# puzzlepaint/surfelmeshing

Hardware: NVIDIA H100
Metric: RGB-D frames/s at 640x480 (depth pre-processing + Integrate()) (higher is better)
Workload: dtype f32

## Files before the change

surfelmeshing_b200/csrc/api.cu:

```cuda

#include <algorithm>
#include <atomic>
#include <chrono>
#include <cstdio>
#include <cstdlib>
#include <cstring>
#include <limits>
#include <mutex>
#include <string>
#include <vector>

#include "sm_handle.cuh"

namespace smb {

namespace {
thread_local std::string g_last_error;
std::atomic<unsigned long long> g_launches{0};
}

int SetError(int code, const char* message) {
  g_last_error = message ? message : "";
  return code;
}

int CheckLaunch(const char* what) {
  const cudaError_t e = cudaGetLastError();
  if (e == cudaSuccess) return SM_OK;
  g_last_error = std::string(what) + ": " + cudaGetErrorString(e);
  return SM_ERR_CUDA;
}

namespace {
struct ProfileRecord { cudaEvent_t start, stop; int id; };
std::mutex g_profile_mutex;
bool g_profile_enabled = false;
std::vector<ProfileRecord> g_profile_records;
std::vector<cudaEvent_t> g_event_pool;

cudaEvent_t TakeEvent() {
  if (!g_event_pool.empty()) { cudaEvent_t e = g_event_pool.back(); g_event_pool.pop_back(); return e; }
  cudaEvent_t e = nullptr;
  cudaEventCreate(&e);
  return e;
}
}

bool ProfilingEnabled() { return g_profile_enabled; }

void CountLaunches(unsigned long long n) { g_launches.fetch_add(n, std::memory_order_relaxed); }
unsigned long long LaunchCount() { return g_launches.load(); }

void LaunchOnStream(cudaStream_t stream, const KernelLaunch& k, bool dependent) {
  LaunchScope scope(stream, static_cast<KernelId>(k.kernel_id));
  cudaLaunchConfig_t cfg = {};
  cfg.gridDim = k.grid;
  cfg.blockDim = k.block;
  cfg.dynamicSmemBytes = k.smem;
  cfg.stream = stream;
  cudaLaunchAttribute attr[1];
  attr[0].id = cudaLaunchAttributeProgrammaticStreamSerialization;
  attr[0].val.programmaticStreamSerializationAllowed = 1;
  cfg.attrs = attr;
  const int mode = PdlMode();
  cfg.numAttrs = (mode == 2 || (mode == 1 && dependent)) ? 1 : 0;
  cudaLaunchKernelExC(&cfg, k.func, const_cast<void**>(k.args));
}

namespace {
u32 ModInverse(u32 x, u32 m) {
  long long t = 0, new_t = 1, r = m, new_r = x % m;
  while (new_r != 0) {
    const long long q = r / new_r;
    long long tmp = t - q * new_t; t = new_t; new_t = tmp;
    tmp = r - q * new_r; r = new_r; new_r = tmp;
  }
  if (t < 0) t += m;
  return static_cast<u32>(t);
}
}

int SetTieBreakWave(TieBreakConfig* cfg, u32 wave, u32 capacity) {
  u32 lane_shift = cfg->lane_request;
  if (wave != 0) {
    const unsigned long long top = (static_cast<unsigned long long>(capacity) / wave + 2) * 2ull * wave;
    if (wave < 2 || top >= 0xFFFFFFFFull) return SetError(SM_ERR_INVALID_ARGUMENT, "tiebreak_wave out of range for this surfel cap");
    if (lane_shift > 10) return SetError(SM_ERR_INVALID_ARGUMENT, "tiebreak_lanes must be a power of two <= 1024");
    if (wave % (1u << lane_shift) != 0 || (wave >> lane_shift) < 2) lane_shift = 0;
    const u32 groups = wave >> lane_shift;
    const unsigned long long prime = 2654435761ull;
    cfg->mul = static_cast<u32>(prime % groups);
    if (cfg->mul == 0) cfg->mul = 1;
    cfg->mul_inv = ModInverse(cfg->mul, groups);
  }
  cfg->wave = wave;
  cfg->lane_shift = lane_shift;
  return SM_OK;
}

TieBreak MakeTieBreak(const TieBreakConfig& cfg, u32 frame_index) {
  TieBreak t{};
  t.wave = cfg.wave;
  if (cfg.wave == 0) return t;
  t.lane_shift = cfg.lane_shift;
  t.wave_offset = cfg.wave_offset;
  t.groups = cfg.wave >> cfg.lane_shift;
  t.mul = cfg.mul;
  t.mul_inv = cfg.mul_inv;
  t.wave_reciprocal = ~0ull / cfg.wave;
  t.group_reciprocal = ~0ull / t.groups;
  t.add = tb_hash(frame_index * 0x9E3779B9u + 0x7F4A7C15u) % t.groups;
  t.salt = tb_hash(frame_index ^ 0x85EBCA6Bu);
  auto threshold = [](double fraction) {
    const double scaled = fraction * 4294967296.0;
    return scaled <= 0 ? 0u : (scaled >= 4294967295.0 ? 0xFFFFFFFFu : static_cast<u32>(scaled));
  };
  t.early_threshold = threshold(cfg.early_fraction);
  t.index_order_threshold = threshold(cfg.index_order_fraction);
  const double later = cfg.early_fraction_later >= 0 ? cfg.early_fraction_later : cfg.early_fraction;
  t.early_threshold_later = threshold(later);
  t.early_threshold_second = threshold(cfg.early_fraction_second >= 0 ? cfg.early_fraction_second : later);
  t.index_order_threshold_later = threshold(cfg.index_order_fraction_later >= 0 ? cfg.index_order_fraction_later : cfg.index_order_fraction);
  return t;
}

int ScaleGrid(int blocks) {
  static const int percent = [] { const char* e = std::getenv("SM_B200_GRID_PERCENT"); return e ? std::atoi(e) : 100; }();
  const int scaled = static_cast<int>(static_cast<long long>(blocks) * percent / 100);
  return scaled > 0 ? scaled : 1;
}

int PdlMode() {
  static const int mode = [] {
    const char* e = std::getenv("SM_B200_PDL");
    return (e && e[0] >= '0' && e[0] <= '2') ? e[0] - '0' : 1;
  }();
  return mode;
}

const char* KernelName(int id) {
  static const char* names[KID_COUNT] = {
      "k_clear", "k_bilateral_outlier", "k_bilateral_generic", "k_outlier", "k_erode_normals_radii", "k_erode",
      "k_normals", "k_radii", "k_project", "k_associate", "k_merge", "k_blend", "k_integrate", "k_update_neighbors",
      "k_new_surfel_scan", "k_create_surfels", "k_reg_accumulate", "k_reg_step", "k_reg_copy_only",
      "k_export_vertices", "k_median_densify", "k_delta_select", "k_viz_buffers", "k_project_tail",
      "k_downscale_depth_median", "k_downscale_color"};
  return (id >= 0 && id < KID_COUNT) ? names[id] : "?";
}

LaunchScope::LaunchScope(cudaStream_t stream, KernelId id) : stream_(stream), slot_(-1) {
  g_launches.fetch_add(1, std::memory_order_relaxed);
  if (g_profile_enabled) {
    std::lock_guard<std::mutex> lock(g_profile_mutex);
    ProfileRecord r{TakeEvent(), TakeEvent(), static_cast<int>(id)};
    cudaEventRecord(r.start, stream_);
    slot_ = static_cast<int>(g_profile_records.size());
    g_profile_records.push_back(r);
  }
}

LaunchScope::~LaunchScope() {
  if (slot_ >= 0) {
    std::lock_guard<std::mutex> lock(g_profile_mutex);
    cudaEventRecord(g_profile_records[slot_].stop, stream_);
  }
}

}

using namespace smb;

#define SM_CUDA(call)                                                                        \
  do {                                                                                       \
    const cudaError_t e_ = (call);                                                           \
    if (e_ != cudaSuccess) {                                                                 \
      g_last_error = std::string(#call) + ": " + cudaGetErrorString(e_);                     \
      return SM_ERR_CUDA;                                                                    \
    }                                                                                        \
  } while (0)

namespace smb {

int FetchCounters(sm_reconstruction* r, cudaStream_t stream) {
  SM_CUDA(cudaMemcpyAsync(r->host_counters, r->d.counters, sizeof(Counters), cudaMemcpyDeviceToHost, stream));
  SM_CUDA(cudaStreamSynchronize(stream));
  if (r->host_counters->capacity_overflow) {
    return SetError(SM_ERR_CAPACITY, "surfel cap exceeded: new surfels of at least one frame were dropped "
                                     "(the reference writes out of bounds here)");
  }
  return SM_OK;
}

FrameParams MakeFrameParams(const sm_reconstruction* r, u32 frame_index, int count_slot, const sm_integrate_params& p,
                            u16* depth, size_t depth_pitch, const u16* depth_pre, size_t depth_pre_pitch,
                            const float* normals, size_t normals_pitch, const float* radius, size_t radius_pitch,
                            const uint8_t* color, size_t color_pitch, const float* global_T_local,
                            const float* local_T_global) {
  FrameParams f;
  f.frame_index = frame_index;
  f.count_slot = count_slot;
  f.skip = 0;
  f.op_epoch = r->op_epoch;
  f.tb = MakeTieBreak(r->tiebreak, frame_index);
  f.active_window = p.surfel_integration_active_window_size;
  f.fx = r->fx; f.fy = r->fy; f.cx = r->cx; f.cy = r->cy;
  f.fx_inv = 1.0f / r->fx;
  f.fy_inv = 1.0f / r->fy;
  const float cx_pixel_center = r->cx - 0.5f;
  const float cy_pixel_center = r->cy - 0.5f;
  f.cx_inv = -cx_pixel_center / r->fx;
  f.cy_inv = -cy_pixel_center / r->fy;
  f.sensor_noise_factor = p.sensor_noise_factor;
  f.cos_normal_compatibility_threshold = cosf(M_PI / 180.0f * p.normal_compatibility_threshold_deg);
  f.max_surfel_confidence = p.max_surfel_confidence;
  f.inv_depth_scaling = 1.0f / p.depth_scaling;
  f.depth_scaling = 1.0f / f.inv_depth_scaling;
  f.radius_factor_squared =
      p.radius_factor_for_regularization_neighbors * p.radius_factor_for_regularization_neighbors;
  f.blend_radius = p.measurement_blending_radius;
  f.local_T_global = MakeMat3x4(local_T_global);
  f.global_T_local = MakeMat3x4(global_T_local);
  f.depth = depth; f.depth_pitch = depth_pitch;
  f.depth_pre = depth_pre; f.depth_pre_pitch = depth_pre_pitch;
  f.normals = reinterpret_cast<const float2*>(normals); f.normals_pitch = normals_pitch;
  f.radius = radius; f.radius_pitch = radius_pitch;
  f.color = reinterpret_cast<const uchar3*>(color); f.color_pitch = color_pitch;
  return f;
}

int IntegrateImpl(sm_reconstruction* r, cudaStream_t stream, u32 frame_index, const sm_integrate_params& p,
                  u16* depth, size_t depth_pitch, const float* normals, size_t normals_pitch, const float* radius,
                  size_t radius_pitch, const uint8_t* color, size_t color_pitch, const float* global_T_local,
                  const float* local_T_global) {
  r->last_stream = stream;
  RecordOperation(r, static_cast<int>(frame_index - static_cast<u32>(p.regularization_frame_window_size)));
  const u16* depth_pre = depth;
  size_t depth_pre_pitch = depth_pitch;
  if (p.do_blending) {
    SM_CUDA(cudaMemcpy2DAsync(r->blend_src, r->blend_src_pitch, depth, depth_pitch, r->d.width * sizeof(u16),
                              r->d.height, cudaMemcpyDeviceToDevice, stream));
    depth_pre = r->blend_src;
    depth_pre_pitch = r->blend_src_pitch;
  }
  const FrameParams f = MakeFrameParams(r, frame_index, r->count_slot, p, depth, depth_pitch, depth_pre, depth_pre_pitch,
                                        normals, normals_pitch, radius, radius_pitch, color, color_pitch,
                                        global_T_local, local_T_global);
  r->last_tiebreak = f.tb;
  int status = IntegrateFrame(stream, r->d, f, p.do_blending != 0, r->rasters_cleared, r->plan, &r->events);
  r->rasters_cleared = false;
  if (status != SM_OK) return status;
  NoteIntegratedFrame(r->d, frame_index);
  const int old_slot = r->count_slot;
  r->count_slot = (r->count_slot + 1) % kCountSlots;
  if (r->events.enabled) cudaEventRecord(r->events.ev[12], stream);
  const int iterations = p.regularization_iterations_per_integration_iteration;
  if (iterations == 0) {
    status = RegularizeSurfels(stream, r->d,  true, frame_index,
                               p.radius_factor_for_regularization_neighbors, p.regularizer_weight,
                               p.regularization_frame_window_size, r->count_slot, old_slot, r->plan);
  } else {
    for (int i = 0; i < iterations && status == SM_OK; ++i) {
      status = RegularizeSurfels(stream, r->d,  false, frame_index,
                                 p.radius_factor_for_regularization_neighbors, p.regularizer_weight,
                                 p.regularization_frame_window_size, r->count_slot, i == 0 ? old_slot : -1, r->plan);
    }
  }
  if (r->events.enabled) cudaEventRecord(r->events.ev[13], stream);
  return status;
}

}

namespace {

int CreateImpl(sm_reconstruction* r, uint64_t max_surfel_count, int32_t width, int32_t height, float fx, float fy,
               float cx, float cy) {
  SM_CUDA(cudaGetDevice(&r->device));
  cudaDeviceProp prop;
  SM_CUDA(cudaGetDeviceProperties(&prop, r->device));
  r->sm_count = prop.multiProcessorCount;
  r->plan.sm_count = r->sm_count;
  {
    const char* e = std::getenv("SM_B200_CARVEOUT");
    const int percent = e ? std::atoi(e) : 47;
    int status = ConfigurePreprocessKernels(percent);
    if (status == SM_OK) status = ConfigureIntegrateKernels(percent, &r->plan);
    if (status == SM_OK) status = ConfigureRegularizeKernels(percent, &r->plan);
    if (status != SM_OK) return status;
  }
  r->fx = fx; r->fy = fy; r->cx = cx; r->cy = cy;
  DeviceState& d = r->d;
  d.width = width; d.height = height;
  d.capacity = static_cast<u32>(max_surfel_count);
  const size_t padded = (max_surfel_count + kSegment - 1) / kSegment * kSegment;
  d.stride = padded;
  const size_t P = static_cast<size_t>(width) * height;
  const size_t scan_tiles = (P + kSegment - 1) / kSegment;
  SM_CUDA(cudaMalloc(&d.surfels, sizeof(float) * SM_ROW_COUNT * d.stride));
  SM_CUDA(cudaMalloc(&d.gradient, sizeof(float4) * d.stride));
  SM_CUDA(cudaMalloc(&r->smooth_alt, sizeof(float) * 3 * d.stride));
  d.smooth = d.surfels + static_cast<size_t>(SM_ROW_SMOOTH_X) * d.stride;
  d.smooth_next = r->smooth_alt;
  SM_CUDA(cudaMemset(d.gradient, 0, sizeof(float4) * d.stride));
  for (int i = 0; i < kSets; ++i) {
    SM_CUDA(cudaMalloc(&r->assoc_set[i], sizeof(PixelAssoc) * P));
    SM_CUDA(cudaMalloc(&r->first_depth_set[i], sizeof(float) * P));
    SM_CUDA(cudaMalloc(&r->supported_set[i], P));
    SM_CUDA(cudaMalloc(&r->vis_set[i], sizeof(VisEntry) * padded));
    SM_CUDA(cudaMalloc(&r->seg_count_set[i], sizeof(u32) * (padded / kSegment)));
    SM_CUDA(cudaMalloc(&r->merge_flag_set[i], padded));
    SM_CUDA(cudaMalloc(&r->upd_list_set[i], sizeof(uint2) * padded));
    SM_CUDA(cudaMalloc(&r->upd_count_set[i], sizeof(u32)));
  }
  d.assoc = r->assoc_set[0]; d.first_depth = r->first_depth_set[0]; d.supported = r->supported_set[0];
  d.vis = r->vis_set[0]; d.seg_count = r->seg_count_set[0]; d.merge_flag = r->merge_flag_set[0];
  d.upd_list = r->upd_list_set[0]; d.upd_count = r->upd_count_set[0];
  d.reg_t_prev = 0;
  d.reg_full_sweep = 1;
  SM_CUDA(cudaMalloc(&d.new_list, sizeof(u32) * P));
  SM_CUDA(cudaMalloc(&d.new_flag, P));
  SM_CUDA(cudaMalloc(&d.new_index, sizeof(u32) * P));
  SM_CUDA(cudaMalloc(&d.scan_state, sizeof(unsigned long long) * scan_tiles));
  SM_CUDA(cudaMalloc(&d.counters, sizeof(Counters)));
  SM_CUDA(cudaMemset(d.counters, 0, sizeof(Counters)));
  d.timeline = nullptr;
  d.timeline_frames = 0;
  SM_CUDA(cudaMemset(d.new_flag, 0, P));
  SM_CUDA(cudaMemset(d.new_index, 0, sizeof(u32) * P));
  SM_CUDA(cudaMemset(d.scan_state, 0, sizeof(unsigned long long) * scan_tiles));
  SM_CUDA(cudaMallocHost(&r->host_counters, sizeof(Counters)));
  std::memset(r->host_counters, 0, sizeof(Counters));
  SM_CUDA(cudaMallocPitch(reinterpret_cast<void**>(&r->scratch_B), &r->scratch_B_pitch, width * sizeof(u16), height));
  SM_CUDA(cudaMallocPitch(reinterpret_cast<void**>(&r->blend_src), &r->blend_src_pitch, width * sizeof(u16), height));
  {
    const char* e = std::getenv("SM_B200_TAIL_FILL");
    const bool want_tma = !(e && std::string(e) == "vector");
    if (want_tma) {
      const int status = MakeDepthTensorMap(&r->scratch_B_map, r->scratch_B, r->scratch_B_pitch, width, height);
      if (status != SM_OK) return status;
      r->scratch_B_map_valid = true;
    }
  }
  for (int i = 0; i < 14; ++i) SM_CUDA(cudaEventCreate(&r->events.ev[i]));
  r->events.enabled = false;
  {
    u32 wave = kDefaultTieBreakWave, lanes = 1u << kDefaultTieBreakLaneShift;
    double early = kDefaultTieBreakEarlyFraction, index_order = kDefaultTieBreakIndexOrderFraction;
    u32 offset = kDefaultTieBreakWaveOffset;
    if (const char* e = std::getenv("SM_B200_TIEBREAK")) {
      unsigned w = 0, l = 0, o = 0; double q = 0, b = 0;
      const int got = std::sscanf(e, "%u,%lf,%lf,%u,%u", &w, &q, &b, &l, &o);
      if (got >= 2) { wave = w; early = q; }
      if (got >= 3) index_order = b;
      if (got >= 4) lanes = l;
      if (got >= 5) offset = o ? 1u : 0u;
    }
    r->tiebreak.wave_offset = offset;
    u32 lane_shift = 0;
    while ((1u << lane_shift) < lanes && lane_shift < 10) ++lane_shift;
    if (wave != 0 && (static_cast<unsigned long long>(d.capacity) / wave + 2) * 2ull * wave >= 0xFFFFFFFFull) wave = 0;
    r->tiebreak.lane_request = lane_shift;
    const int status = SetTieBreakWave(&r->tiebreak, wave, d.capacity);
    if (status != SM_OK) return status;
    r->tiebreak.early_fraction = early;
    r->tiebreak.index_order_fraction = index_order;
    r->tiebreak.early_fraction_later = kDefaultTieBreakEarlyFractionLater;
    r->tiebreak.index_order_fraction_later = kDefaultTieBreakIndexOrderFractionLater;
    r->tiebreak.early_fraction_second = kDefaultTieBreakEarlyFractionSecond;
  }
  const int status = ClearAssociationRasters(nullptr, d);
  if (status != SM_OK) return status;
  SM_CUDA(cudaDeviceSynchronize());
  return SM_OK;
}

}

extern "C" {

void sm_default_integrate_params(sm_integrate_params* p) {
  p->depth_scaling = 5000;
  p->sensor_noise_factor = 0.05f;
  p->max_surfel_confidence = 5.0f;
  p->regularizer_weight = 10.0f;
  p->regularization_frame_window_size = 30;
  p->do_blending = 1;
  p->measurement_blending_radius = 12;
  p->regularization_iterations_per_integration_iteration = 1;
  p->radius_factor_for_regularization_neighbors = 2;
  p->normal_compatibility_threshold_deg = 40;
  p->surfel_integration_active_window_size = std::numeric_limits<int>::max();
}

void sm_default_preprocess_params(sm_preprocess_params* p) {
  p->depth_scaling = 5000;
  p->max_depth = 3.0f;
  p->depth_valid_region_radius = 333;
  p->bilateral_filter_sigma_xy = 3;
  p->bilateral_filter_radius_factor = 2.0f;
  p->bilateral_filter_sigma_depth_factor = 0.05;
  p->outlier_filtering_frame_count = 8;
  p->outlier_filtering_required_inliers = -1;
  p->outlier_filtering_depth_tolerance_factor = 0.02f;
  p->depth_erosion_radius = 2;
  p->observation_angle_threshold_deg = 85;
  p->point_radius_extension_factor = 1.5f;
  p->point_radius_clamp_factor = std::numeric_limits<float>::infinity();
}

const char* sm_last_error(void) { return g_last_error.c_str(); }
const char* sm_version(void) { return "surfel_b200 0.1 (sm_90a)"; }
uint64_t sm_kernel_launch_count(void) { return g_launches.load(); }

int sm_profile_kernels(int32_t enable) {
  std::lock_guard<std::mutex> lock(g_profile_mutex);
  g_profile_enabled = enable != 0;
  return SM_OK;
}

int32_t sm_profile_kernel_count(void) { return KID_COUNT; }
const char* sm_profile_kernel_name(int32_t id) { return KernelName(id); }

int sm_profile_report(double* total_ms, uint64_t* launches, int32_t n) {
  SM_CUDA(cudaDeviceSynchronize());
  std::lock_guard<std::mutex> lock(g_profile_mutex);
  for (int i = 0; i < n; ++i) { total_ms[i] = 0; launches[i] = 0; }
  for (const ProfileRecord& r : g_profile_records) {
    float ms = 0;
    if (cudaEventElapsedTime(&ms, r.start, r.stop) == cudaSuccess && r.id < n) {
      total_ms[r.id] += ms;
      launches[r.id] += 1;
    }
    g_event_pool.push_back(r.start);
    g_event_pool.push_back(r.stop);
  }
  g_profile_records.clear();
  return SM_OK;
}

int sm_create(sm_reconstruction** out, uint64_t max_surfel_count, int32_t width, int32_t height, float fx, float fy,
              float cx, float cy) {
  if (out) *out = nullptr;
  if (!out || width <= 0 || height <= 0 || max_surfel_count == 0 || max_surfel_count > 0x7FFFFFFFull - kSegment) {
    return SetError(SM_ERR_INVALID_ARGUMENT, "sm_create: bad argument");
  }
  sm_reconstruction* r = new sm_reconstruction();
  const int status = CreateImpl(r, max_surfel_count, width, height, fx, fy, cx, cy);
  if (status != SM_OK) {
    const std::string message = g_last_error;
    sm_destroy(r);
    g_last_error = message;
    return status;
  }
  *out = r;
  return SM_OK;
}

int sm_destroy(sm_reconstruction* r) {
  if (!r) return SM_OK;
  cudaDeviceSynchronize();
  cudaGetLastError();
  DestroyFrameGraph(r->graph);
  DeviceState& d = r->d;
  cudaFree(d.surfels); cudaFree(d.gradient); cudaFree(r->smooth_alt); cudaFree(d.new_list);
  for (int i = 0; i < kSets; ++i) {
    cudaFree(r->vis_set[i]); cudaFree(r->seg_count_set[i]); cudaFree(r->merge_flag_set[i]);
    cudaFree(r->upd_list_set[i]); cudaFree(r->upd_count_set[i]);
    cudaFree(r->assoc_set[i]); cudaFree(r->first_depth_set[i]); cudaFree(r->supported_set[i]);
    cudaFree(r->run_depth[i]); cudaFree(r->run_depth_pre[i]); cudaFree(r->run_normals[i]); cudaFree(r->run_radius[i]);
  }
  cudaFree(d.new_flag); cudaFree(d.new_index); cudaFree(d.scan_state); cudaFree(d.counters);
  cudaFree(d.timeline);
  if (r->host_counters) cudaFreeHost(r->host_counters);
  cudaFree(r->scratch_B);
  cudaFree(r->blend_src);
  cudaFree(r->median_stage[0]); cudaFree(r->median_stage[1]);
  cudaFree(r->pyramid_depth_stage); cudaFree(r->pyramid_color_stage);
  FreeTransferBuffers(r);
  for (int i = 0; i < 2; ++i) {
    if (r->pipe.ev_create[i]) cudaEventDestroy(r->pipe.ev_create[i]);
    if (r->pipe.ev_update[i]) cudaEventDestroy(r->pipe.ev_update[i]);
    if (r->pre_done[i]) cudaEventDestroy(r->pre_done[i]);
    if (r->int_done[i]) cudaEventDestroy(r->int_done[i]);
  }
  for (cudaStream_t st : {r->pre_stream, r->pipe.crit, r->pipe.front, r->pipe.side, r->upload_stream, r->graph_stream})
    if (st) cudaStreamDestroy(st);
  for (cudaEvent_t e : {r->pipe.ev_assoc, r->pipe.ev_merge, r->pipe.ev_blend, r->pipe.ev_integrate, r->pipe.ev_reg,
                        r->entry_event, r->upload_done, r->graph_exit})
    if (e) cudaEventDestroy(e);
  for (cudaEvent_t e : r->iteration_done) if (e) cudaEventDestroy(e);
  for (u16* b : r->ring_depth) cudaFree(b);
  for (uchar3* b : r->ring_color) cudaFree(b);
  for (int i = 0; i < 14; ++i) if (r->events.ev[i]) cudaEventDestroy(r->events.ev[i]);
  delete r;
  cudaGetLastError();
  return SM_OK;
}

int sm_reset(sm_reconstruction* r, void* stream) {
  SM_CUDA(cudaMemsetAsync(r->d.counters, 0, sizeof(Counters), static_cast<cudaStream_t>(stream)));
  r->count_slot = 0;
  r->rasters_cleared = false;
  r->last_stream = static_cast<cudaStream_t>(stream);
  ++r->state_generation;
  r->op_history.clear();
  return SM_OK;
}

int sm_preprocess(sm_reconstruction* r, void* stream, const sm_preprocess_params* p, const uint16_t* raw_depth,
                  size_t raw_pitch, const uint16_t* const* other_depths, const size_t* other_pitches,
                  const float* others_TR_reference, uint16_t* out_depth, size_t out_depth_pitch, float* out_normals,
                  size_t out_normals_pitch, float* out_radius, size_t out_radius_pitch) {
  const int status = PreprocessFused(static_cast<cudaStream_t>(stream), *p, r->d.width, r->d.height, r->fx, r->fy,
                                     r->cx, r->cy, raw_depth, raw_pitch, other_depths, other_pitches,
                                     others_TR_reference, r->scratch_B, r->scratch_B_pitch, out_depth,
                                     out_depth_pitch, reinterpret_cast<float2*>(out_normals), out_normals_pitch,
                                     out_radius, out_radius_pitch, r->d.assoc, r->d.first_depth, r->d.supported, nullptr, 0,
                                     nullptr, nullptr, r->ScratchBMap());
  if (status == SM_OK) r->rasters_cleared = true;
  return status;
}

int sm_bilateral_filter_and_depth_cutoff(void* stream, float sigma_xy, float sigma_value_factor,
                                         uint16_t value_to_ignore, float radius_factor, uint16_t max_depth,
                                         float depth_valid_region_radius, int32_t width, int32_t height,
                                         const uint16_t* in_depth, size_t in_pitch, uint16_t* out_depth,
                                         size_t out_pitch) {
  return StageBilateral(static_cast<cudaStream_t>(stream), sigma_xy, sigma_value_factor, value_to_ignore,
                        radius_factor, max_depth, depth_valid_region_radius, width, height, in_depth, in_pitch,
                        out_depth, out_pitch);
}

int sm_outlier_depth_map_fusion(void* stream, int32_t other_count, int32_t required_count, float tolerance, float fx,
                                float fy, float cx, float cy, int32_t width, int32_t height, const uint16_t* in_depth,
                                size_t in_pitch, const uint16_t* const* other_depths, const size_t* other_pitches,
                                const float* others_TR_reference, uint16_t* out_depth, size_t out_pitch) {
  return StageOutlier(static_cast<cudaStream_t>(stream), other_count, required_count, tolerance, fx, fy, cx, cy,
                      width, height, in_depth, in_pitch, other_depths, other_pitches, others_TR_reference, out_depth,
                      out_pitch);
}

int sm_median_filter_and_densify_depth_map(void* stream, int32_t iterations, int32_t width, int32_t height,
                                           const uint16_t* in_depth, size_t in_pitch, uint16_t* out_depth,
                                           size_t out_pitch, uint16_t* scratch, size_t scratch_pitch) {
  return StageMedianDensify(static_cast<cudaStream_t>(stream), iterations, width, height, in_depth, in_pitch, out_depth,
                            out_pitch, scratch, scratch_pitch);
}

int sm_downscale_using_median_while_excluding(void* stream, uint16_t value_to_ignore, int32_t in_width,
                                              int32_t in_height, const uint16_t* in, size_t in_pitch,
                                              int32_t out_width, int32_t out_height, uint16_t* out,
                                              size_t out_pitch) {
  return StageDownscaleMedian(static_cast<cudaStream_t>(stream), value_to_ignore, in_width, in_height, in, in_pitch,
                              out_width, out_height, out, out_pitch);
}

int sm_color_image_pyramid(void* stream, int32_t levels, int32_t width, int32_t height, const uint8_t* in,
                           size_t in_pitch, uint8_t* out, size_t out_pitch) {
  return StageColorPyramid(static_cast<cudaStream_t>(stream), levels, width, height, in, in_pitch, out, out_pitch);
}

int sm_erode_depth_map(void* stream, int32_t radius, int32_t width, int32_t height, const uint16_t* in_depth,
                       size_t in_pitch, uint16_t* out_depth, size_t out_pitch) {
  return StageErode(static_cast<cudaStream_t>(stream), radius, width, height, in_depth, in_pitch, out_depth,
                    out_pitch);
}

int sm_compute_normals_and_drop_bad_pixels(void* stream, float observation_angle_threshold_deg, float depth_scaling,
                                           float fx, float fy, float cx, float cy, int32_t width, int32_t height,
                                           const uint16_t* in_depth, size_t in_pitch, uint16_t* out_depth,
                                           size_t out_pitch, float* out_normals, size_t normals_pitch) {
  return StageNormals(static_cast<cudaStream_t>(stream), observation_angle_threshold_deg, depth_scaling, fx, fy, cx,
                      cy, width, height, in_depth, in_pitch, out_depth, out_pitch,
                      reinterpret_cast<float2*>(out_normals), normals_pitch);
}

int sm_compute_point_radii_and_remove_isolated_pixels(void* stream, float point_radius_extension_factor,
                                                      float point_radius_clamp_factor, float depth_scaling, float fx,
                                                      float fy, float cx, float cy, int32_t width, int32_t height,
                                                      const uint16_t* in_depth, size_t in_pitch, float* out_radius,
                                                      size_t radius_pitch, uint16_t* out_depth, size_t out_pitch) {
  return StageRadii(static_cast<cudaStream_t>(stream), point_radius_extension_factor, point_radius_clamp_factor,
                    depth_scaling, fx, fy, cx, cy, width, height, in_depth, in_pitch, out_radius, radius_pitch,
                    out_depth, out_pitch);
}

int sm_integrate(sm_reconstruction* r, void* stream, uint32_t frame_index, const sm_integrate_params* p,
                 uint16_t* depth, size_t depth_pitch, const float* normals, size_t normals_pitch, const float* radius,
                 size_t radius_pitch, const uint8_t* color, size_t color_pitch, const float global_T_local[12],
                 const float local_T_global[12]) {
  return IntegrateImpl(r, static_cast<cudaStream_t>(stream), frame_index, *p, depth, depth_pitch, normals,
                       normals_pitch, radius, radius_pitch, color, color_pitch, global_T_local, local_T_global);
}

int sm_regularize(sm_reconstruction* r, void* stream, uint32_t frame_index, float regularizer_weight,
                  float radius_factor_for_regularization_neighbors, int32_t regularization_frame_window_size) {
  r->last_stream = static_cast<cudaStream_t>(stream);
  RecordOperation(r, static_cast<int>(frame_index - static_cast<u32>(regularization_frame_window_size)));
  return RegularizeSurfels(static_cast<cudaStream_t>(stream), r->d,  false, frame_index,
                           radius_factor_for_regularization_neighbors, regularizer_weight,
                           regularization_frame_window_size, r->count_slot, -1, r->plan);
}

int sm_surfel_count(sm_reconstruction* r, uint32_t* out) {
  const int status = FetchCounters(r, r->last_stream);
  *out = r->host_counters->surfel_count[r->count_slot] - r->host_counters->merge_count;
  return status;
}

int sm_surfels_size(sm_reconstruction* r, uint32_t* out) {
  const int status = FetchCounters(r, r->last_stream);
  *out = r->host_counters->surfel_count[r->count_slot];
  return status;
}

int sm_transfer_all_to_cpu(sm_reconstruction* r, void* stream_v, uint32_t , float* x, float* y,
                           float* z, float* radius_squared, float* nx, float* ny, float* nz,
                           uint32_t* last_update_stamp, uint64_t* out_count) {
  cudaStream_t stream = static_cast<cudaStream_t>(stream_v);
  const int status = FetchCounters(r, stream);
  const u32 n = r->host_counters->surfel_count[r->count_slot];
  if (out_count) *out_count = n;
  if (n == 0) return status;
  const size_t bytes = sizeof(float) * n;
  const float* s = r->d.surfels;
  const size_t st = r->d.stride;
  SM_CUDA(cudaMemcpyAsync(x, r->d.smooth + 0 * st, bytes, cudaMemcpyDeviceToHost, stream));
  SM_CUDA(cudaMemcpyAsync(y, r->d.smooth + 1 * st, bytes, cudaMemcpyDeviceToHost, stream));
  SM_CUDA(cudaMemcpyAsync(z, r->d.smooth + 2 * st, bytes, cudaMemcpyDeviceToHost, stream));
  SM_CUDA(cudaMemcpyAsync(radius_squared, s + SM_ROW_RADIUS_SQUARED * st, bytes, cudaMemcpyDeviceToHost, stream));
  SM_CUDA(cudaMemcpyAsync(nx, s + SM_ROW_NORMAL_X * st, bytes, cudaMemcpyDeviceToHost, stream));
  SM_CUDA(cudaMemcpyAsync(ny, s + SM_ROW_NORMAL_Y * st, bytes, cudaMemcpyDeviceToHost, stream));
  SM_CUDA(cudaMemcpyAsync(nz, s + SM_ROW_NORMAL_Z * st, bytes, cudaMemcpyDeviceToHost, stream));
  SM_CUDA(cudaMemcpyAsync(last_update_stamp, s + SM_ROW_LAST_UPDATE_STAMP * st, bytes, cudaMemcpyDeviceToHost, stream));
  return status;
}

int sm_transfer_delta_to_cpu(sm_reconstruction* r, void* stream, uint32_t frame_index, sm_transfer_token* token,
                             float* x, float* y, float* z, float* radius_squared, float* nx, float* ny, float* nz,
                             uint32_t* last_update_stamp, sm_transfer_stats* stats) {
  if (!r || !token) return SetError(SM_ERR_INVALID_ARGUMENT, "sm_transfer_delta_to_cpu: null argument");
  return TransferDelta(r, static_cast<cudaStream_t>(stream), frame_index, token, x, y, z, radius_squared, nx, ny, nz,
                       last_update_stamp, stats);
}

int sm_update_visualization_buffers(sm_reconstruction* r, void* stream, const sm_visualization_params* p,
                                    float* vertex_buffer, uint32_t* neighbor_index_buffer, float* normal_vertex_buffer) {
  if (!r || !p) return SetError(SM_ERR_INVALID_ARGUMENT, "sm_update_visualization_buffers: null argument");
  return UpdateVisualizationBuffers(r, static_cast<cudaStream_t>(stream), *p, vertex_buffer, neighbor_index_buffer,
                                    normal_vertex_buffer);
}

int sm_export_vertices(sm_reconstruction* r, void* stream, float* position_buffer, uint8_t* color_buffer) {
  return ExportVertices(static_cast<cudaStream_t>(stream), r->d, r->count_slot, r->sm_count, position_buffer,
                        color_buffer);
}

int sm_get_timings(sm_reconstruction* r, float out_ms[7]) {
  if (!r->events.enabled) return SetError(SM_ERR_INVALID_ARGUMENT, "timings are not enabled (sm_enable_timings)");
  SM_CUDA(cudaEventSynchronize(r->events.ev[13]));
  for (int i = 0; i < 7; ++i) SM_CUDA(cudaEventElapsedTime(&out_ms[i], r->events.ev[2 * i], r->events.ev[2 * i + 1]));
  return SM_OK;
}

int sm_enable_timings(sm_reconstruction* r, int32_t enable) {
  r->events.enabled = enable != 0;
  return SM_OK;
}

int sm_dump_state(sm_reconstruction* r, void* stream_v, float* host_rows, uint64_t host_row_stride_elems,
                  uint32_t* surfels_size, uint32_t* merge_count) {
  cudaStream_t stream = static_cast<cudaStream_t>(stream_v);
  const int status = FetchCounters(r, stream);
  const u32 n = r->host_counters->surfel_count[r->count_slot];
  if (surfels_size) *surfels_size = n;
  if (merge_count) *merge_count = r->host_counters->merge_count;
  if (host_rows && n > host_row_stride_elems) return SetError(SM_ERR_INVALID_ARGUMENT, "sm_dump_state: host rows shorter than surfels_size()");
  if (host_rows && n > 0) {
    SM_CUDA(cudaMemcpy2DAsync(host_rows, host_row_stride_elems * sizeof(float), r->d.surfels,
                              r->d.stride * sizeof(float), n * sizeof(float), SM_ROW_COUNT, cudaMemcpyDeviceToHost,
                              stream));
    SM_CUDA(cudaMemcpy2DAsync(host_rows + SM_ROW_SMOOTH_X * host_row_stride_elems, host_row_stride_elems * sizeof(float),
                              r->d.smooth, r->d.stride * sizeof(float), n * sizeof(float), 3, cudaMemcpyDeviceToHost,
                              stream));
    SM_CUDA(cudaStreamSynchronize(stream));
  }
  return status;
}

int sm_load_state(sm_reconstruction* r, void* stream_v, const float* host_rows, uint64_t host_row_stride_elems,
                  uint32_t surfels_size, uint32_t merge_count) {
  cudaStream_t stream = static_cast<cudaStream_t>(stream_v);
  if (surfels_size > r->d.capacity) return SetError(SM_ERR_CAPACITY, "sm_load_state: state larger than the surfel cap");
  r->d.smooth = r->d.surfels + static_cast<size_t>(SM_ROW_SMOOTH_X) * r->d.stride;
  r->d.smooth_next = r->smooth_alt;
  r->d.reg_full_sweep = 1;
  if (surfels_size > 0) {
    SM_CUDA(cudaMemcpy2DAsync(r->d.surfels, r->d.stride * sizeof(float), host_rows,
                              host_row_stride_elems * sizeof(float), surfels_size * sizeof(float), SM_ROW_COUNT,
                              cudaMemcpyHostToDevice, stream));
    SM_CUDA(cudaMemsetAsync(r->d.gradient, 0, surfels_size * sizeof(float4), stream));
    const int zero_rows[4] = {SM_ROW_GRADIENT_X, SM_ROW_GRADIENT_Y, SM_ROW_GRADIENT_Z, SM_ROW_GRADIENT_COUNT};
    for (int row : zero_rows) {
      SM_CUDA(cudaMemsetAsync(r->d.surfels + row * r->d.stride, 0, surfels_size * sizeof(float), stream));
    }
    SM_CUDA(cudaMemsetAsync(r->d.surfels + kRowMergeEpoch * r->d.stride, 0, surfels_size * sizeof(float), stream));
    const int status = RebuildMetaRow(stream, r->d, surfels_size, r->sm_count);
    if (status != SM_OK) return status;
  }
  Counters c{};
  for (int i = 0; i < kCountSlots; ++i) c.surfel_count[i] = surfels_size;
  c.merge_count = merge_count;
  *r->host_counters = c;
  SM_CUDA(cudaMemcpyAsync(r->d.counters, r->host_counters, sizeof(Counters), cudaMemcpyHostToDevice, stream));
  SM_CUDA(cudaStreamSynchronize(stream));
  r->count_slot = 0;
  r->last_stream = stream;
  ++r->state_generation;
  r->op_history.clear();
  return SM_OK;
}

int sm_download_rasters(sm_reconstruction* r, void* stream_v, uint32_t* supporting_surfels,
                        uint32_t* supporting_surfel_counts, float* supporting_surfel_depth_sums,
                        uint32_t* conflicting_surfels, float* first_surfel_depth, uint8_t* new_surfel_flag_vector,
                        uint32_t* new_surfel_indices) {
  cudaStream_t stream = static_cast<cudaStream_t>(stream_v);
  const size_t P = static_cast<size_t>(r->d.width) * r->d.height;
  std::vector<PixelAssoc> assoc(P);
  SM_CUDA(cudaMemcpyAsync(assoc.data(), r->d.assoc, sizeof(PixelAssoc) * P, cudaMemcpyDeviceToHost, stream));
  if (first_surfel_depth)
    SM_CUDA(cudaMemcpyAsync(first_surfel_depth, r->d.first_depth, sizeof(float) * P, cudaMemcpyDeviceToHost, stream));
  if (new_surfel_flag_vector)
    SM_CUDA(cudaMemcpyAsync(new_surfel_flag_vector, r->d.new_flag, P, cudaMemcpyDeviceToHost, stream));
  if (new_surfel_indices)
    SM_CUDA(cudaMemcpyAsync(new_surfel_indices, r->d.new_index, sizeof(u32) * P, cudaMemcpyDeviceToHost, stream));
  SM_CUDA(cudaStreamSynchronize(stream));
  for (size_t i = 0; i < P; ++i) {
    if (supporting_surfels) supporting_surfels[i] = supporting_index(r->last_tiebreak, assoc[i].x, static_cast<u32>(i));
    if (conflicting_surfels) conflicting_surfels[i] = assoc[i].y;
    if (supporting_surfel_counts) supporting_surfel_counts[i] = assoc[i].z;
    if (supporting_surfel_depth_sums) std::memcpy(&supporting_surfel_depth_sums[i], &assoc[i].w, sizeof(float));
  }
  return SM_OK;
}

int sm_frame_counters(sm_reconstruction* r, void* stream_v, uint64_t out[4]) {
  cudaStream_t stream = static_cast<cudaStream_t>(stream_v);
  const int status = FetchCounters(r, stream);
  const u32 n_after = r->host_counters->surfel_count[r->count_slot];
  const u32 n_swept = n_after - r->host_counters->new_surfel_count;
  const size_t segments = (static_cast<size_t>(n_swept) + kSegment - 1) / kSegment;
  std::vector<u32> seg(segments);
  if (segments) SM_CUDA(cudaMemcpy(seg.data(), r->d.seg_count, sizeof(u32) * segments, cudaMemcpyDeviceToHost));
  uint64_t visible = 0;
  for (u32 c : seg) visible += c;
  const size_t P = static_cast<size_t>(r->d.width) * r->d.height;
  std::vector<PixelAssoc> assoc(P);
  SM_CUDA(cudaMemcpy(assoc.data(), r->d.assoc, sizeof(PixelAssoc) * P, cudaMemcpyDeviceToHost));
  uint64_t support = 0;
  for (const PixelAssoc& a : assoc) support += a.z;
  out[0] = n_swept; out[1] = visible; out[2] = support; out[3] = r->host_counters->new_surfel_count;
  return status;
}

int sm_timeline_enable(sm_reconstruction* r, int32_t frames) {
  if (r == nullptr || frames < 0) return SetError(SM_ERR_INVALID_ARGUMENT, "sm_timeline_enable: bad arguments");
  SM_CUDA(cudaDeviceSynchronize());
  if (r->d.timeline) {
    cudaFree(r->d.timeline);
    r->d.timeline = nullptr;
    r->d.timeline_frames = 0;
  }
  if (frames == 0) return SM_OK;
  const size_t slots = static_cast<size_t>(frames) * KID_COUNT;
  SM_CUDA(cudaMalloc(&r->d.timeline, slots * 2 * sizeof(unsigned long long)));
  std::vector<unsigned long long> init(slots * 2);
  for (size_t i = 0; i < slots; ++i) { init[2 * i] = ~0ull; init[2 * i + 1] = 0ull; }
  SM_CUDA(cudaMemcpy(r->d.timeline, init.data(), init.size() * sizeof(unsigned long long), cudaMemcpyHostToDevice));
  r->d.timeline_frames = static_cast<u32>(frames);
  return SM_OK;
}

int sm_timeline_read(sm_reconstruction* r, uint64_t* out, int32_t frames) {
  if (r == nullptr || out == nullptr) return SetError(SM_ERR_INVALID_ARGUMENT, "sm_timeline_read: bad arguments");
  if (r->d.timeline == nullptr || frames != static_cast<int32_t>(r->d.timeline_frames))
    return SetError(SM_ERR_INVALID_ARGUMENT, "sm_timeline_read: timeline not enabled with this frame count");
  SM_CUDA(cudaDeviceSynchronize());
  SM_CUDA(cudaMemcpy(out, r->d.timeline, static_cast<size_t>(frames) * KID_COUNT * 2 * sizeof(uint64_t), cudaMemcpyDeviceToHost));
  return SM_OK;
}

int sm_stream_run(sm_reconstruction* r, void* stream_v, const sm_stream_desc* s, const sm_preprocess_params* pp,
                  const sm_integrate_params* ip, int32_t first_frame, int32_t last_frame, sm_stream_stats* stats) {
  if (!r || !s || !pp || !ip) return SetError(SM_ERR_INVALID_ARGUMENT, "sm_stream_run: null argument");
  return StreamRun(r, static_cast<cudaStream_t>(stream_v), s, pp, ip, first_frame, last_frame, stats);
}

int sm_configure(sm_reconstruction* r, const char* key, double value) {
  if (!r || !key) return SetError(SM_ERR_INVALID_ARGUMENT, "sm_configure: null argument");
  const std::string k(key);
  if (k == "tiebreak_wave") {
    if (value < 0 || value > 2147483647.0) return SetError(SM_ERR_INVALID_ARGUMENT, "tiebreak_wave out of range");
    return SetTieBreakWave(&r->tiebreak, static_cast<u32>(value), r->d.capacity);
  }
  if (k == "tiebreak_early_fraction_later" || k == "tiebreak_index_order_fraction_later" || k == "tiebreak_early_fraction_second") {
    if (!(value <= 1.0)) return SetError(SM_ERR_INVALID_ARGUMENT, "tiebreak_*_later / _second must be <= 1 (negative: inherit)");
    (k == "tiebreak_early_fraction_later" ? r->tiebreak.early_fraction_later
     : k == "tiebreak_early_fraction_second" ? r->tiebreak.early_fraction_second : r->tiebreak.index_order_fraction_later) = value;
    return SM_OK;
  }
  if (k == "tiebreak_wave_offset") {
    r->tiebreak.wave_offset = value != 0.0 ? 1u : 0u;
    return SM_OK;
  }
  if (k == "tiebreak_lanes") {
    const u32 lanes = static_cast<u32>(value);
    if (value < 1 || value > 1024 || (lanes & (lanes - 1)) != 0) return SetError(SM_ERR_INVALID_ARGUMENT, "tiebreak_lanes must be a power of two in [1, 1024]");
    u32 shift = 0;
    while ((1u << shift) < lanes) ++shift;
    r->tiebreak.lane_request = shift;
    return SetTieBreakWave(&r->tiebreak, r->tiebreak.wave, r->d.capacity);
  }
  if (k == "tiebreak_early_fraction") {
    if (!(value >= 0.0 && value <= 1.0)) return SetError(SM_ERR_INVALID_ARGUMENT, "tiebreak_early_fraction must be in [0, 1]");
    r->tiebreak.early_fraction = value;
    return SM_OK;
  }
  if (k == "tiebreak_index_order_fraction") {
    if (!(value >= 0.0 && value <= 1.0)) return SetError(SM_ERR_INVALID_ARGUMENT, "tiebreak_index_order_fraction must be in [0, 1]");
    r->tiebreak.index_order_fraction = value;
    return SM_OK;
  }
  if (k == "median_filter_and_densify_iterations") {
    if (value < 0 || value > 16 || value != static_cast<int>(value)) return SetError(SM_ERR_INVALID_ARGUMENT, "median_filter_and_densify_iterations must be an integer in [0, 16]");
    r->median_iterations = static_cast<int>(value);
    return SM_OK;
  }
  if (k == "pyramid_level") {
    if (value < 0 || value > 4 || value != static_cast<int>(value)) return SetError(SM_ERR_INVALID_ARGUMENT, "pyramid_level must be an integer in [0, 4]");
    r->pyramid_level = static_cast<int>(value);
    return SM_OK;
  }
  return SetError(SM_ERR_INVALID_ARGUMENT, "sm_configure: unknown key");
}

}
```

surfelmeshing_b200/csrc/integrate.cu:

```cuda

#include <algorithm>
#include <cstdio>
#include <cstdlib>

#include <cooperative_groups.h>

#include "sm_kernels.cuh"

namespace cg = cooperative_groups;

namespace smb {

namespace {

#define SM_S(row, i) d.surfels[static_cast<size_t>(row) * d.stride + (i)]
#define SM_SU(row, i) reinterpret_cast<u32*>(d.surfels)[static_cast<size_t>(row) * d.stride + (i)]
#define SM_SMOOTH(axis, i) d.smooth[static_cast<size_t>(axis) * d.stride + (i)]
#define SM_SMOOTH_NEXT(axis, i) d.smooth_next[static_cast<size_t>(axis) * d.stride + (i)]

constexpr int kBlock = 256;

__device__ __forceinline__ bool is_active(u32 last_update_stamp, u32 frame_index, int window) {
  return static_cast<int>(last_update_stamp) > static_cast<int>(frame_index - static_cast<u32>(window));
}

struct Projection {
  float u, v;
  int px, py;
  bool in_image;
};

__device__ __forceinline__ Projection project(const FrameParams& f, int width, int height, float x, float y, float z) {
  Projection p;
  const float inv_z = frcp(z);
  p.u = ffma(fmul(x, inv_z), f.fx, f.cx);
  p.v = ffma(fmul(y, inv_z), f.fy, f.cy);
  p.px = f2i_trunc(p.u);
  p.py = f2i_trunc(p.v);
  p.in_image = !(p.u < 0.f || p.v < 0.f || p.px < 0 || p.py < 0 || p.px >= width || p.py >= height);
  return p;
}

__device__ __forceinline__ bool secondary_pixel(const Projection& p, int width, int height, int* ox, int* oy) {
  const float x_frac = fsub(p.u, i2f(p.px));
  const float y_frac = fsub(p.v, i2f(p.py));
  if (x_frac < y_frac) {
    if (x_frac < fadd(-y_frac, 1.0f)) {
      if (p.px > 1) { *ox = p.px - 1; *oy = p.py; return true; }
      return false;
    }
    if (p.py < height - 1) { *ox = p.px; *oy = p.py + 1; return true; }
    return false;
  }
  if (x_frac < fadd(-y_frac, 1.0f)) {
    if (p.py > 0) { *ox = p.px; *oy = p.py - 1; return true; }
    return false;
  }
  if (p.px < width - 1) { *ox = p.px + 1; *oy = p.py; return true; }
  return false;
}

__device__ __forceinline__ float normal_z_abs(float nx, float ny) {
  return fsqrt_approx(fmaxf(0.f, ffma(-ny, ny, ffma(-nx, nx, 1.0f))));
}

__device__ __forceinline__ float facing_dot(const FrameParams& f, float x, float y, float z, float nx, float ny,
                                            float nz, float3* local_normal) {
  const float rs = frsqrt_approx(squared_norm(x, y, z));
  *local_normal = rotate_vec(f.local_T_global, nx, ny, nz);
  return fmul(rs, ffma(z, local_normal->z, ffma(x, local_normal->x, fmul(y, local_normal->y))));
}

template <typename Body>
__device__ __forceinline__ void for_each_visible(const DeviceState& d, const u32* surfel_count, Body&& body) {
  constexpr u32 kItemsPerSegment = kSegment / kBlock;
  const u32 max_items = ((d.capacity + kSegment - 1) / kSegment) * kItemsPerSegment;
  const u32 n = *surfel_count;
  u32 item = blockIdx.x;
  u32 cnt = 0;
  VisEntry e = make_uint4(0u, 0u, 0u, 0u);
  if (item < max_items) {
    cnt = d.seg_count[item / kItemsPerSegment];
    e = d.vis[static_cast<size_t>(item) * kBlock + threadIdx.x];
  }
  const u32 items = ((n + kSegment - 1) / kSegment) * kItemsPerSegment;
  while (item < items) {
    const u32 next = item + gridDim.x;
    u32 cnt_next = 0;
    VisEntry e_next = e;
    if (next < items) {
      cnt_next = d.seg_count[next / kItemsPerSegment];
      e_next = d.vis[static_cast<size_t>(next) * kBlock + threadIdx.x];
    }
    const u32 k = (item % kItemsPerSegment) * kBlock + threadIdx.x;
    if (k < cnt) body(static_cast<size_t>(item) * kBlock + threadIdx.x, e);
    item = next;
    cnt = cnt_next;
    e = e_next;
  }
}

__global__ void __launch_bounds__(kBlock) k_clear(DeviceState d) {
  pdl_prologue();
  const int n = d.width * d.height;
  for (int i = blockIdx.x * blockDim.x + threadIdx.x; i < n; i += gridDim.x * blockDim.x) {
    d.assoc[i] = make_uint4(kInvalidIndex, kInvalidIndex, 0u, 0u);
    d.first_depth[i] = __int_as_float(0x7f800000);
    d.supported[i] = 0;
  }
}

constexpr int kProjectBlock = 512;

enum { kProjectAll = 0, kProjectMain = 1, kProjectTail = 2 };

__global__ void __launch_bounds__(kProjectBlock) k_project(DeviceState d, FrameParams f, int part) {
  pdl_prologue();
  if (f.skip) return;
  const TimelineScope timeline_scope(d, f.frame_index, part == kProjectTail ? KID_PROJECT_TAIL : KID_PROJECT);
  __shared__ u32 warp_totals[kProjectBlock / 32];
  const int lane = threadIdx.x & 31, warp = threadIdx.x >> 5;
  const u32 first_seg_if_all = blockIdx.x;

  if (blockIdx.x == 0 && part != kProjectMain) {
    const int tiles = (d.width * d.height + kSegment - 1) / kSegment;
    for (int t = threadIdx.x; t < tiles; t += blockDim.x) d.scan_state[t] = 0ull;
    if (threadIdx.x == 0) { d.counters->scan_ticket = 0; *d.upd_count = 0; }
  }

  struct SlotRows { float2 X, Y, Z; uint2 T; };
  auto fetch = [&](u32 seg) {
    SlotRows r;
    const size_t base = static_cast<size_t>(seg) * kSegment + threadIdx.x * 2;
    r.X = *reinterpret_cast<const float2*>(&SM_S(SM_ROW_X, base));
    r.Y = *reinterpret_cast<const float2*>(&SM_S(SM_ROW_Y, base));
    r.Z = *reinterpret_cast<const float2*>(&SM_S(SM_ROW_Z, base));
    r.T = *reinterpret_cast<const uint2*>(&SM_SU(SM_ROW_LAST_UPDATE_STAMP, base));
    return r;
  };
  SlotRows rows = {};
  if (part != kProjectTail && (static_cast<size_t>(first_seg_if_all) + 1) * kSegment <= d.stride) rows = fetch(first_seg_if_all);
  const u32 n_before = part == kProjectAll ? 0u : d.counters->surfel_count[(f.count_slot + kCountSlots - 1) % kCountSlots];
  const u32 seg_begin = part == kProjectTail ? n_before / kSegment : 0u;
  const u32 n = part == kProjectMain ? (n_before / kSegment) * kSegment
                                     : d.counters->surfel_count[f.count_slot];
  if (part == kProjectTail && static_cast<u64>(seg_begin + blockIdx.x) * kSegment < n) rows = fetch(seg_begin + blockIdx.x);
  for (u32 seg = seg_begin + blockIdx.x; static_cast<u64>(seg) * kSegment < n; seg += gridDim.x) {
    const u32 base = seg * kSegment + threadIdx.x * 2;
    const SlotRows cur = rows;
    if (static_cast<u64>(seg + gridDim.x) * kSegment < n) rows = fetch(seg + gridDim.x);
    VisEntry e[2];
    bool visible[2] = {false, false};
    u32 cnt = 0;
    if (base < n) {
      const float xs[2] = {cur.X.x, cur.X.y}, ys[2] = {cur.Y.x, cur.Y.y}, zs[2] = {cur.Z.x, cur.Z.y};
      const u32 ts[2] = {cur.T.x, cur.T.y};
#pragma unroll
      for (int j = 0; j < 2; ++j) {
        const u32 i = base + j;
        if (i >= n) break;
        const float z = transform_row(f.local_T_global.r2, xs[j], ys[j], zs[j]);
        if (!(z > 0.f)) continue;
        const float x = transform_row(f.local_T_global.r0, xs[j], ys[j], zs[j]);
        const float y = transform_row(f.local_T_global.r1, xs[j], ys[j], zs[j]);
        const Projection p = project(f, d.width, d.height, x, y, z);
        if (!p.in_image) continue;
        const bool active = is_active(ts[j], f.frame_index, f.active_window);
        e[j] = make_uint4(i | (active ? kActiveBit : 0u), __float_as_uint(x), __float_as_uint(y), __float_as_uint(z));
        visible[j] = true;
        ++cnt;
        if (active) {
// ... 510 lines not shown
  }
#endif
}


struct SurfelState {
  float x, y, z, confidence, radius_squared, nx, ny, nz;
  float smooth_x, smooth_y, smooth_z;
  u32 color, creation_stamp, last_update_stamp;
  bool replaced, dirty, stamped;
};

struct PixelMeasurement {
  float measurement_depth, first, radius_squared;
  float2 normal;
  u32 conflicting, count;
  u32 r, g, b;
};

__device__ __forceinline__ PixelMeasurement load_pixel_measurement(const DeviceState& d, const FrameParams& f, int x,
                                                                   int y) {
  PixelMeasurement m;
  const int p = y * d.width + x;
  m.measurement_depth = fmul(u2f(row_ptr(f.depth, f.depth_pitch, y)[x]), f.inv_depth_scaling);
  m.first = d.first_depth[p];
  const PixelAssoc a = d.assoc[p];
  m.conflicting = a.y;
  m.count = a.z;
  m.normal = row_ptr(f.normals, f.normals_pitch, y)[x];
  m.radius_squared = row_ptr(f.radius, f.radius_pitch, y)[x];
  const uchar3 c = row_ptr(f.color, f.color_pitch, y)[x];
  m.r = c.x; m.g = c.y; m.b = c.z;
  return m;
}

__device__ __forceinline__ void integrate_or_conflict(const FrameParams& f, const PixelMeasurement& m, int x, int y,
                                                      u32 idx, float cx_, float cy_, float cz_, SurfelState& s) {
  if (!(m.measurement_depth > 0.f)) return;
  bool integrate = true, conflicting = false;
  if (m.first < fmul(m.measurement_depth, fadd(-f.sensor_noise_factor, 1.0f))) {
    if (m.first == cz_ && m.conflicting == idx) conflicting = true;
    integrate = false;
  }
  if (!integrate && !conflicting) return;
  if (cz_ > fmul(fadd(f.sensor_noise_factor, 1.0f), m.measurement_depth)) integrate = false;
  if (!integrate && !conflicting) return;

  const float lx = fmul(m.measurement_depth, ffma(i2f(x), f.fx_inv, f.cx_inv));
  const float ly = fmul(m.measurement_depth, ffma(i2f(y), f.fy_inv, f.cy_inv));
  const float3 g = transform_point(f.global_T_local, lx, ly, m.measurement_depth);
  const float3 gn = rotate_vec(f.global_T_local, m.normal.x, m.normal.y, -normal_z_abs(m.normal.x, m.normal.y));

  if (conflicting) {
    const float confidence = fadd(s.confidence, -1.0f);
    if (confidence <= 0.f) {
      s.x = g.x; s.y = g.y; s.z = g.z;
      s.smooth_x = g.x; s.smooth_y = g.y; s.smooth_z = g.z;
      s.nx = gn.x; s.ny = gn.y; s.nz = gn.z;
      s.color = m.r | (m.g << 8) | (m.b << 16) | (1u << 24);
      s.radius_squared = m.radius_squared;
      s.confidence = 1.0f;
      s.creation_stamp = f.frame_index;
      s.stamped = true;
      s.replaced = true;
    } else {
      s.confidence = confidence;
    }
    s.dirty = true;
  }
  if (!integrate) return;

  float3 ln;
  if (facing_dot(f, cx_, cy_, cz_, s.nx, s.ny, s.nz, &ln) > 0.f) return;
  if (m.measurement_depth < cz_) {
    if (ffma(gn.z, s.nz, ffma(gn.x, s.nx, fmul(gn.y, s.ny))) < f.cos_normal_compatibility_threshold) return;
  }
  if (s.radius_squared < 0.f) return;

  const float weight = frcp(u2f(max(1u, m.count)));
  if (s.creation_stamp < f.frame_index) {
    const float confidence = s.confidence;
    const float cw = fadd(weight, confidence);
    s.confidence = (cw < f.max_surfel_confidence) ? cw : f.max_surfel_confidence;
    const float normalization_factor = frcp(cw);
    s.x = fmul(normalization_factor, ffma(g.x, weight, fmul(confidence, s.x)));
    s.y = fmul(normalization_factor, ffma(g.y, weight, fmul(confidence, s.y)));
    s.z = fmul(normalization_factor, ffma(g.z, weight, fmul(confidence, s.z)));
    const float nx = ffma(gn.x, weight, fmul(confidence, s.nx));
    const float ny = ffma(gn.y, weight, fmul(confidence, s.ny));
    const float nz = ffma(gn.z, weight, fmul(confidence, s.nz));
    const float normal_normalization = frsqrt_approx(ffma(nz, nz, ffma(nx, nx, fmul(ny, ny))));
    s.nx = fmul(nx, normal_normalization);
    s.ny = fmul(ny, normal_normalization);
    s.nz = fmul(nz, normal_normalization);
    s.radius_squared = fminf(s.radius_squared, m.radius_squared);
    const u32 old_color = s.color;
    const u32 r = f2u_trunc(ffma(normalization_factor, ffma(u2f(m.r), weight, fmul(confidence, u2f(old_color & 0xFFu))), 0.5f));
    const u32 gr = f2u_trunc(ffma(normalization_factor, ffma(u2f(m.g), weight, fmul(confidence, u2f((old_color >> 8) & 0xFFu))), 0.5f));
    const u32 b = f2u_trunc(ffma(normalization_factor, ffma(u2f(m.b), weight, fmul(confidence, u2f((old_color >> 16) & 0xFFu))), 0.5f));
    s.color = (r & 0xFFu) | ((gr & 0xFFu) << 8) | ((b & 0xFFu) << 16);
    s.stamped = true;
    s.dirty = true;
  }
}

#ifndef SM_INTEGRATE_LEVELS
#define SM_INTEGRATE_LEVELS 2
#endif

__device__ __forceinline__ bool pixel_can_touch(const FrameParams& f, float measurement_depth, float first, u32 conflicting,
                                                u32 idx, float cz_) {
  if (!(measurement_depth > 0.f)) return false;
  if (first < fmul(measurement_depth, fadd(-f.sensor_noise_factor, 1.0f))) return first == cz_ && conflicting == idx;
  return !(cz_ > fmul(fadd(f.sensor_noise_factor, 1.0f), measurement_depth));
}

__device__ __forceinline__ bool integrate_entry(const DeviceState& d, const FrameParams& f, size_t pos, const VisEntry& e,
                                                int* ux, int* uy) {
    const u32 idx = e.x & ~kActiveBit;
    const float x = __uint_as_float(e.y), y = __uint_as_float(e.z), z = __uint_as_float(e.w);
    const Projection p = project(f, d.width, d.height, x, y, z);
    int ox = p.px, oy = p.py;
    const bool has2 = secondary_pixel(p, d.width, d.height, &ox, &oy);
    const u8 merged = d.merge_flag[pos];
    SurfelState s;
    PixelMeasurement m0, m1;
#if SM_INTEGRATE_LEVELS == 1
    m0 = load_pixel_measurement(d, f, p.px, p.py);
    m1 = load_pixel_measurement(d, f, ox, oy);
    s.x = SM_S(SM_ROW_X, idx); s.y = SM_S(SM_ROW_Y, idx); s.z = SM_S(SM_ROW_Z, idx);
    s.confidence = SM_S(SM_ROW_CONFIDENCE, idx);
    s.radius_squared = SM_S(SM_ROW_RADIUS_SQUARED, idx);
    s.nx = SM_S(SM_ROW_NORMAL_X, idx); s.ny = SM_S(SM_ROW_NORMAL_Y, idx); s.nz = SM_S(SM_ROW_NORMAL_Z, idx);
    s.color = SM_SU(SM_ROW_COLOR, idx);
    s.creation_stamp = SM_SU(SM_ROW_CREATION_STAMP, idx);
#else
    const int p0 = p.py * d.width + p.px, p1 = oy * d.width + ox;
    m0.measurement_depth = fmul(u2f(row_ptr(f.depth, f.depth_pitch, p.py)[p.px]), f.inv_depth_scaling);
    m1.measurement_depth = fmul(u2f(row_ptr(f.depth, f.depth_pitch, oy)[ox]), f.inv_depth_scaling);
    m0.first = d.first_depth[p0];
    m1.first = d.first_depth[p1];
    const PixelAssoc a0 = d.assoc[p0], a1 = d.assoc[p1];
    m0.conflicting = a0.y; m0.count = a0.z;
    m1.conflicting = a1.y; m1.count = a1.z;
    s.radius_squared = SM_S(SM_ROW_RADIUS_SQUARED, idx);
#endif
    s.last_update_stamp = 0;
    s.smooth_x = s.smooth_y = s.smooth_z = 0.f;
    s.replaced = false; s.dirty = false; s.stamped = false;
    if (merged) {
      SM_SU(SM_ROW_LAST_UPDATE_STAMP, idx) = 0;
      SM_S(SM_ROW_RADIUS_SQUARED, idx) = -1.0f;
      reinterpret_cast<u8*>(&SM_SU(SM_ROW_COLOR, idx))[3] = 1;
      SM_SU(kRowMeta, idx) = kMetaDetachBit;
      SM_SU(kRowMergeEpoch, idx) = f.op_epoch;
      SM_SMOOTH_NEXT(0, idx) = SM_SMOOTH(0, idx); SM_SMOOTH_NEXT(1, idx) = SM_SMOOTH(1, idx);
      SM_SMOOTH_NEXT(2, idx) = SM_SMOOTH(2, idx);
      return false;
    }
    if (!(e.x & kActiveBit)) return false;
    if (s.radius_squared < 0.f) return false;
#if SM_INTEGRATE_LEVELS != 1
    const bool touch0 = pixel_can_touch(f, m0.measurement_depth, m0.first, m0.conflicting, idx, z);
    const bool touch1 = has2 && pixel_can_touch(f, m1.measurement_depth, m1.first, m1.conflicting, idx, z);
    if (touch0 || touch1) {
      const int qx0 = touch0 ? p.px : ox, qy0 = touch0 ? p.py : oy;
      const int qx1 = touch1 ? ox : qx0, qy1 = touch1 ? oy : qy0;
      m0.normal = row_ptr(f.normals, f.normals_pitch, qy0)[qx0];
      m1.normal = row_ptr(f.normals, f.normals_pitch, qy1)[qx1];
      m0.radius_squared = row_ptr(f.radius, f.radius_pitch, qy0)[qx0];
      m1.radius_squared = row_ptr(f.radius, f.radius_pitch, qy1)[qx1];
      const uchar3 c0 = row_ptr(f.color, f.color_pitch, qy0)[qx0];
      const uchar3 c1 = row_ptr(f.color, f.color_pitch, qy1)[qx1];
      m0.r = c0.x; m0.g = c0.y; m0.b = c0.z;
      m1.r = c1.x; m1.g = c1.y; m1.b = c1.z;
      s.x = SM_S(SM_ROW_X, idx); s.y = SM_S(SM_ROW_Y, idx); s.z = SM_S(SM_ROW_Z, idx);
      s.confidence = SM_S(SM_ROW_CONFIDENCE, idx);
      s.nx = SM_S(SM_ROW_NORMAL_X, idx); s.ny = SM_S(SM_ROW_NORMAL_Y, idx); s.nz = SM_S(SM_ROW_NORMAL_Z, idx);
      s.color = SM_SU(SM_ROW_COLOR, idx);
      s.creation_stamp = SM_SU(SM_ROW_CREATION_STAMP, idx);
      if (touch0) integrate_or_conflict(f, m0, p.px, p.py, idx, x, y, z, s);
      if (touch1) integrate_or_conflict(f, m1, ox, oy, idx, x, y, z, s);
    }
#else
    integrate_or_conflict(f, m0, p.px, p.py, idx, x, y, z, s);
    if (has2) integrate_or_conflict(f, m1, ox, oy, idx, x, y, z, s);
#endif
    if (s.dirty) {
      SM_S(SM_ROW_X, idx) = s.x; SM_S(SM_ROW_Y, idx) = s.y; SM_S(SM_ROW_Z, idx) = s.z;
      SM_S(SM_ROW_CONFIDENCE, idx) = s.confidence;
      SM_S(SM_ROW_RADIUS_SQUARED, idx) = s.radius_squared;
      SM_S(SM_ROW_NORMAL_X, idx) = s.nx; SM_S(SM_ROW_NORMAL_Y, idx) = s.ny; SM_S(SM_ROW_NORMAL_Z, idx) = s.nz;
      SM_SU(SM_ROW_COLOR, idx) = s.color;
      if (s.stamped) {
        SM_SU(SM_ROW_LAST_UPDATE_STAMP, idx) = f.frame_index;
        SM_SU(kRowMeta, idx) = f.frame_index | (((s.color >> 24) & 1u) ? kMetaDetachBit : 0u);
      }
      if (s.replaced) {
        SM_SMOOTH(0, idx) = s.smooth_x; SM_SMOOTH(1, idx) = s.smooth_y; SM_SMOOTH(2, idx) = s.smooth_z;
        SM_SMOOTH_NEXT(0, idx) = s.smooth_x; SM_SMOOTH_NEXT(1, idx) = s.smooth_y; SM_SMOOTH_NEXT(2, idx) = s.smooth_z;
        SM_SU(SM_ROW_CREATION_STAMP, idx) = f.frame_index;
#pragma unroll
        for (int i = 0; i < 4; ++i) SM_SU(SM_ROW_NEIGHBOR0 + i, idx) = kInvalidIndex;
      }
    }

    if (s.stamped && !is_active(f.frame_index, f.frame_index, f.active_window)) return false;
    if (s.radius_squared < 0.f) return false;
    float cz_ = z;
    int px = p.px, py = p.py;
    if (s.dirty) {
      cz_ = transform_row(f.local_T_global.r2, s.x, s.y, s.z);
      if (!(cz_ > 0.f)) return false;
      const float cx_ = transform_row(f.local_T_global.r0, s.x, s.y, s.z);
      const float cy_ = transform_row(f.local_T_global.r1, s.x, s.y, s.z);
      const float inv_z = frcp(cz_);
      px = f2i_trunc(ffma(fmul(cx_, inv_z), f.fx, f.cx));
      py = f2i_trunc(ffma(fmul(cy_, inv_z), f.fy, f.cy));
    }
    constexpr int kBorder = 1;
    if (px < kBorder || py < kBorder || px >= d.width - kBorder || py >= d.height - kBorder) return false;
    float measurement_depth = m0.measurement_depth;
    if (px != p.px || py != p.py) {
      measurement_depth = fmul(u2f(row_ptr(f.depth, f.depth_pitch, py)[px]), f.inv_depth_scaling);
    }
    if (cz_ > fmul(measurement_depth, fadd(f.sensor_noise_factor, 1.0f))) return false;
    *ux = px;
    *uy = py;
    return true;
}

__global__ void __launch_bounds__(kBlock, 4) k_integrate(DeviceState d, FrameParams f) {
  pdl_prologue();
  if (f.skip) return;
  const TimelineScope timeline_scope(d, f.frame_index, KID_INTEGRATE);
  for_each_visible(d, &d.counters->surfel_count[f.count_slot], [&](size_t pos, const VisEntry& e) {
    int ux, uy;
    if (!integrate_entry(d, f, pos, e, &ux, &uy)) return;
    const cg::coalesced_group g = cg::coalesced_threads();
    u32 base = 0;
    if (g.thread_rank() == 0) base = atomicAdd(d.upd_count, g.size());
    base = g.shfl(base, 0) + g.thread_rank();
    d.upd_list[base] = make_uint2(e.x & ~kActiveBit, static_cast<u32>(ux) | (static_cast<u32>(uy) << 16));
  });
}

__device__ __forceinline__ void update_neighbors_survivor(const DeviceState& d, const FrameParams& f, u32 idx, int x, int y) {
  const int kDirectionsX[4] = {-1, 1, 0, 0};
  const int kDirectionsY[4] = {0, 0, -1, 1};
  const float gx = SM_S(SM_ROW_X, idx), gy = SM_S(SM_ROW_Y, idx), gz = SM_S(SM_ROW_Z, idx);
  const float nx = SM_S(SM_ROW_NORMAL_X, idx), ny = SM_S(SM_ROW_NORMAL_Y, idx), nz = SM_S(SM_ROW_NORMAL_Z, idx);
  const float radius_squared = SM_S(SM_ROW_RADIUS_SQUARED, idx);
  u32 neighbor_surfel_indices[4];
#pragma unroll
  for (int m = 0; m < 4; ++m) neighbor_surfel_indices[m] = SM_SU(SM_ROW_NEIGHBOR0 + m, idx);
  const float observation_radius_squared = row_ptr(f.radius, f.radius_pitch, y)[x];
  u32 candidate[4];
#pragma unroll
  for (int direction = 0; direction < 4; ++direction) {
    const int candidate_pixel = (y + kDirectionsY[direction]) * d.width + x + kDirectionsX[direction];
    candidate[direction] = supporting_index(f.tb, d.assoc[candidate_pixel].x, static_cast<u32>(candidate_pixel));
  }
  const float cz_ = transform_row(f.local_T_global.r2, gx, gy, gz);
  const float cx_ = transform_row(f.local_T_global.r0, gx, gy, gz);
  const float cy_ = transform_row(f.local_T_global.r1, gx, gy, gz);
  float3 ln;
  if (facing_dot(f, cx_, cy_, cz_, nx, ny, nz, &ln) > 0.f) return;
  if (fmul(observation_radius_squared, frcp(radius_squared)) > 2.25f) return;
  bool any_new = false;
#pragma unroll
  for (int direction = 0; direction < 4; ++direction) {
    const u32 q = candidate[direction];
    if (q == kInvalidIndex || q == idx) { candidate[direction] = kInvalidIndex; continue; }
    any_new |= q != neighbor_surfel_indices[0] && q != neighbor_surfel_indices[1] &&
               q != neighbor_surfel_indices[2] && q != neighbor_surfel_indices[3];
  }
  if (!any_new) return;

  float neighbor_distances_squared[4];
#pragma unroll
  for (int m = 0; m < 4; ++m) {
    const u32 q = neighbor_surfel_indices[m];
    if (q == kInvalidIndex) {
      neighbor_distances_squared[m] = __int_as_float(0x7f800000);
    } else {
      neighbor_distances_squared[m] = squared_norm(fsub(gx, SM_S(SM_ROW_X, q)), fsub(gy, SM_S(SM_ROW_Y, q)),
                                                   fsub(gz, SM_S(SM_ROW_Z, q)));
    }
  }
  const float max_distance_squared = fmul(radius_squared, f.radius_factor_squared);
  float cand_distance[4], cand_dot[4];
#pragma unroll
  for (int direction = 0; direction < 4; ++direction) {
    const u32 q = candidate[direction];
    if (q == kInvalidIndex) continue;
    cand_distance[direction] = squared_norm(fsub(SM_S(SM_ROW_X, q), gx), fsub(SM_S(SM_ROW_Y, q), gy),
                                            fsub(SM_S(SM_ROW_Z, q), gz));
    cand_dot[direction] = dot3(nx, ny, nz, SM_S(SM_ROW_NORMAL_X, q), SM_S(SM_ROW_NORMAL_Y, q), SM_S(SM_ROW_NORMAL_Z, q));
  }
  bool changed = false;
#pragma unroll
  for (int direction = 0; direction < 4; ++direction) {
    const u32 q = candidate[direction];
    if (q == kInvalidIndex) continue;
    const float distance_squared = cand_distance[direction];
    if (distance_squared > max_distance_squared) continue;
    if (cand_dot[direction] <= 0.f) continue;
    int best_n = -1;
    float best_distance_squared = -1.f;
#pragma unroll
    for (int m = 0; m < 4; ++m) {
      if (q == neighbor_surfel_indices[m]) { best_n = -1; break; }
      if (neighbor_distances_squared[m] > best_distance_squared) {
        best_n = m;
        best_distance_squared = neighbor_distances_squared[m];
      }
    }
    if (best_n >= 0 && distance_squared < best_distance_squared) {
#pragma unroll
      for (int m = 0; m < 4; ++m) {
        if (m == best_n) { neighbor_surfel_indices[m] = q; neighbor_distances_squared[m] = distance_squared; }
      }
      changed = true;
    }
  }
  if (changed) {
#pragma unroll
    for (int m = 0; m < 4; ++m) SM_SU(SM_ROW_NEIGHBOR0 + m, idx) = neighbor_surfel_indices[m];
  }
}

__global__ void __launch_bounds__(kBlock) k_update_neighbors(DeviceState d, FrameParams f) {
  pdl_prologue();
  if (f.skip) return;
  const TimelineScope timeline_scope(d, f.frame_index, KID_UPDATE_NEIGHBORS);
  const u32 n = *d.upd_count;
  for (u32 k = blockIdx.x * blockDim.x + threadIdx.x; k < n; k += gridDim.x * blockDim.x) {
    const uint2 w = d.upd_list[k];
    update_neighbors_survivor(d, f, w.x, static_cast<int>(w.y & 0xFFFFu), static_cast<int>(w.y >> 16));
  }
}

__device__ __forceinline__ unsigned long long load_scan_state(unsigned long long* p) { return atomicAdd(p, 0ull); }

__global__ void __launch_bounds__(kBlock) k_new_surfel_scan(DeviceState d, FrameParams f) {
  pdl_prologue();
  if (f.skip) return;
  const TimelineScope timeline_scope(d, f.frame_index, KID_NEW_SURFEL_SCAN);
  __shared__ u32 s_tile, s_prefix;
  __shared__ u32 warp_totals[kBlock / 32];
  const int total_pixels = d.width * d.height;
  const int tiles = (total_pixels + kSegment - 1) / kSegment;
  if (threadIdx.x == 0) s_tile = atomicAdd(&d.counters->scan_ticket, 1u);
  __syncthreads();
  const u32 tile = s_tile;
  if (tile >= static_cast<u32>(tiles)) return;

  const int base = tile * kSegment + threadIdx.x * 4;
  u32 flags[4];
  u32 cnt = 0;
#pragma unroll
  for (int j = 0; j < 4; ++j) {
    const int seq = base + j;
    u32 flag = 0;
    if (seq < total_pixels) {
      const int y = seq / d.width, x = seq - y * d.width;
      constexpr int kBorder = 1;
      if (x >= kBorder && y >= kBorder && x < d.width - kBorder && y < d.height - kBorder &&
          row_ptr(f.depth, f.depth_pitch, y)[x] > 0 && !d.supported[seq]) {
        flag = (d.assoc[seq].y == kInvalidIndex) ? 1u : 0u;
      }
    }
    flags[j] = flag;
    cnt += flag;
  }
  const int lane = threadIdx.x & 31, warp = threadIdx.x >> 5;
  u32 incl = cnt;
#pragma unroll
  for (int o = 1; o < 32; o <<= 1) {
    const u32 t = __shfl_up_sync(0xffffffffu, incl, o);
    if (lane >= o) incl += t;
  }
  if (lane == 31) warp_totals[warp] = incl;
  __syncthreads();
  u32 warp_base = 0, block_total = 0;
#pragma unroll
  for (int w = 0; w < kBlock / 32; ++w) {
    const u32 t = warp_totals[w];
    if (w < warp) warp_base += t;
    block_total += t;
  }
  if (warp == 0) {
    if (lane == 0) atomicExch(&d.scan_state[tile], ((tile == 0 ? 2ull : 1ull) << 32) | block_total);
    u32 exclusive = 0;
    int window_end = static_cast<int>(tile) - 1;
    while (window_end >= 0) {
      const int t = window_end - lane;
      unsigned long long v = 2ull << 32;
      if (t >= 0) {
        do { v = load_scan_state(&d.scan_state[t]); } while ((v >> 32) == 0ull);
      }
      const unsigned inclusive_mask = __ballot_sync(0xffffffffu, (v >> 32) == 2ull);
      const int first_inclusive = __ffs(inclusive_mask) - 1;
      const u32 contribution = (first_inclusive < 0 || lane <= first_inclusive) ? static_cast<u32>(v) : 0u;
      exclusive += __reduce_add_sync(0xffffffffu, contribution);
      if (first_inclusive >= 0) break;
      window_end -= 32;
    }
    if (lane == 0) {
      if (tile != 0) atomicExch(&d.scan_state[tile], (2ull << 32) | (exclusive + block_total));
      s_prefix = exclusive;
      if (tile == static_cast<u32>(tiles) - 1) {
        const u32 n_old = d.counters->surfel_count[f.count_slot];
        u32 new_count = exclusive + block_total;
        if (static_cast<u64>(n_old) + new_count > d.capacity) {
          d.counters->capacity_overflow = 1;
          new_count = 0;
        }
        d.counters->new_surfel_count = new_count;
        d.counters->surfel_count[(f.count_slot + 1) % kCountSlots] = n_old + new_count;
      }
    }
  }
  __syncthreads();
  u32 running = s_prefix + warp_base + (incl - cnt);
#pragma unroll
  for (int j = 0; j < 4; ++j) {
    const int seq = base + j;
    if (seq < total_pixels) {
      d.new_flag[seq] = static_cast<u8>(flags[j]);
      d.new_index[seq] = running;
      if (flags[j]) d.new_list[running] = seq;
    }
    running += flags[j];
  }
}

__global__ void __launch_bounds__(kBlock) k_create_surfels(DeviceState d, FrameParams f) {
  pdl_prologue();
  if (f.skip) return;
  const TimelineScope timeline_scope(d, f.frame_index, KID_CREATE_SURFELS);
  const u32 new_count = d.counters->new_surfel_count;
  const u32 surfel_count = d.counters->surfel_count[f.count_slot];
  for (u32 k = blockIdx.x * blockDim.x + threadIdx.x; k < new_count; k += gridDim.x * blockDim.x) {
    const int seq = d.new_list[k];
    const int y = seq / d.width, x = seq - y * d.width;
    const u32 idx = surfel_count + k;
    const float depth = fmul(u2f(row_ptr(f.depth, f.depth_pitch, y)[x]), f.inv_depth_scaling);
    const float2 nm = row_ptr(f.normals, f.normals_pitch, y)[x];
    const uchar3 color = row_ptr(f.color, f.color_pitch, y)[x];
    const float radius_squared = row_ptr(f.radius, f.radius_pitch, y)[x];
    const int kDirectionsX[4] = {-1, 1, 0, 0};
    const int kDirectionsY[4] = {0, 0, -1, 1};
    u32 neighbor_index[4], neighbor_new_index[4];
    u8 neighbor_is_new[4];
    u16 neighbor_depth[4];
#pragma unroll
    for (int direction = 0; direction < 4; ++direction) {
      const int nx_ = x + kDirectionsX[direction], ny_ = y + kDirectionsY[direction];
      const int nseq = ny_ * d.width + nx_;
      neighbor_index[direction] = supporting_index(f.tb, d.assoc[nseq].x, static_cast<u32>(nseq));
      neighbor_is_new[direction] = d.new_flag[nseq];
      neighbor_new_index[direction] = d.new_index[nseq];
      neighbor_depth[direction] = row_ptr(f.depth, f.depth_pitch, ny_)[nx_];
    }
    const float lx = fmul(depth, ffma(i2f(x), f.fx_inv, f.cx_inv));
    const float ly = fmul(depth, ffma(u2f(y), f.fy_inv, f.cy_inv));
    const float3 g = transform_point(f.global_T_local, lx, ly, depth);
    const float3 gn = rotate_vec(f.global_T_local, nm.x, nm.y, -normal_z_abs(nm.x, nm.y));
    const float max_distance_squared = fmul(radius_squared, f.radius_factor_squared);
    float ndist[4], nsx[4], nsy[4], nsz[4];
#pragma unroll
    for (int direction = 0; direction < 4; ++direction) {
      const u32 q = neighbor_index[direction];
      if (q == kInvalidIndex) continue;
      ndist[direction] = squared_norm(fsub(SM_S(SM_ROW_X, q), g.x), fsub(SM_S(SM_ROW_Y, q), g.y), fsub(SM_S(SM_ROW_Z, q), g.z));
      nsx[direction] = SM_SMOOTH(0, q);
      nsy[direction] = SM_SMOOTH(1, q);
      nsz[direction] = SM_SMOOTH(2, q);
    }
    float sum_x = 0.f, sum_y = 0.f, sum_z = 0.f;
    int existing_neighbor_count_plus_1 = 1;
#pragma unroll
    for (int direction = 0; direction < 4; ++direction) {
      u32 q = neighbor_index[direction];
      if (q != kInvalidIndex) {
        if (ndist[direction] > max_distance_squared) {
          q = kInvalidIndex;
        } else {
          sum_x = fadd(sum_x, nsx[direction]);
          sum_y = fadd(sum_y, nsy[direction]);
          sum_z = fadd(sum_z, nsz[direction]);
          ++existing_neighbor_count_plus_1;
        }
      } else if (neighbor_is_new[direction] == 1) {
        const float diff = ffma(-u2f(neighbor_depth[direction]), f.inv_depth_scaling, depth);
        if (!(fmul(diff, diff) > max_distance_squared)) q = surfel_count + neighbor_new_index[direction];
      }
      SM_SU(SM_ROW_NEIGHBOR0 + direction, idx) = q;
    }
    SM_S(SM_ROW_X, idx) = g.x; SM_S(SM_ROW_Y, idx) = g.y; SM_S(SM_ROW_Z, idx) = g.z;
    SM_S(SM_ROW_NORMAL_X, idx) = gn.x; SM_S(SM_ROW_NORMAL_Y, idx) = gn.y; SM_S(SM_ROW_NORMAL_Z, idx) = gn.z;
    SM_SU(SM_ROW_COLOR, idx) = color.x | (color.y << 8) | (color.z << 16);
    SM_S(SM_ROW_CONFIDENCE, idx) = 1.0f;
    SM_SU(SM_ROW_CREATION_STAMP, idx) = f.frame_index;
    SM_SU(SM_ROW_LAST_UPDATE_STAMP, idx) = f.frame_index;
    SM_SU(kRowMeta, idx) = f.frame_index;
    SM_S(SM_ROW_RADIUS_SQUARED, idx) = radius_squared;
    SM_S(SM_ROW_GRADIENT_X, idx) = 0.f; SM_S(SM_ROW_GRADIENT_Y, idx) = 0.f; SM_S(SM_ROW_GRADIENT_Z, idx) = 0.f;
    SM_S(SM_ROW_GRADIENT_COUNT, idx) = 0.f;
    d.gradient[idx] = make_float4(0.f, 0.f, 0.f, 0.f);
    const float rcp_count = frcp(i2f(existing_neighbor_count_plus_1));
    const float sx = fmul(fadd(g.x, sum_x), rcp_count);
    const float sy = fmul(fadd(g.y, sum_y), rcp_count);
    const float sz = fmul(fadd(g.z, sum_z), rcp_count);
    SM_SMOOTH(0, idx) = sx; SM_SMOOTH(1, idx) = sy; SM_SMOOTH(2, idx) = sz;
    SM_SMOOTH_NEXT(0, idx) = sx; SM_SMOOTH_NEXT(1, idx) = sy; SM_SMOOTH_NEXT(2, idx) = sz;
  }
}

__global__ void __launch_bounds__(kBlock) k_export_vertices(DeviceState d, int count_slot, float* position_buffer,
                                                            u8* color_buffer) {
  pdl_prologue();
  const u32 n = d.counters->surfel_count[count_slot];
  for (u32 i = blockIdx.x * blockDim.x + threadIdx.x; i < n; i += gridDim.x * blockDim.x) {
    const bool merged = SM_S(SM_ROW_RADIUS_SQUARED, i) < 0.f;
    const float nan = __int_as_float(0x7fffffff);
    position_buffer[3 * i + 0] = merged ? nan : SM_SMOOTH(0, i);
    position_buffer[3 * i + 1] = merged ? nan : SM_SMOOTH(1, i);
    position_buffer[3 * i + 2] = merged ? nan : SM_SMOOTH(2, i);
    const u32 c = SM_SU(SM_ROW_COLOR, i);
    color_buffer[3 * i + 0] = c & 0xFF;
    color_buffer[3 * i + 1] = (c >> 8) & 0xFF;
    color_buffer[3 * i + 2] = (c >> 16) & 0xFF;
  }
}

}

namespace {
size_t BlendSmemBytes(int radius) {
  const size_t rw = kBlendTileW + 2 * blend_halo_x(radius), rh = kBlendTileH + 2 * blend_halo_y(radius);
  const size_t rn16 = (rw * rh + 15) & ~static_cast<size_t>(15);
  const size_t mask_words = rh * ((rw + 31) / 32);
  return rn16 * 14 + mask_words * 11 * 4 + 16;
}
constexpr size_t kBlendSmemLimit = 224 * 1024;

#define SM_EV(call)                                                              \
  do {                                                                           \
    const cudaError_t e_ = (call);                                               \
    if (e_ != cudaSuccess) return SetError(SM_ERR_CUDA, cudaGetErrorString(e_)); \
  } while (0)
}

int DescribeFrameKernel(FrameKernel which, const LaunchPlan& plan, const DeviceState& d, const FrameParams& f,
                        KernelLaunch* out) {
  static_assert(sizeof(DeviceState) + sizeof(FrameParams) + 32 <= sizeof(out->storage), "KernelLaunch::storage too small");
  const int scan_tiles = (d.width * d.height + kSegment - 1) / kSegment;
  switch (which) {
    case FK_PROJECT:
    case FK_PROJECT_MAIN:
      out->Reset(reinterpret_cast<const void*>(k_project), dim3(plan.project), dim3(kProjectBlock), 0, KID_PROJECT);
      break;
    case FK_PROJECT_TAIL:
      out->Reset(reinterpret_cast<const void*>(k_project), dim3(plan.sm_count), dim3(kProjectBlock), 0, KID_PROJECT_TAIL);
      break;
    case FK_ASSOCIATE:
      out->Reset(reinterpret_cast<const void*>(k_associate), dim3(plan.associate), dim3(kBlock), 0, KID_ASSOCIATE);
      break;
    case FK_MERGE:
      out->Reset(reinterpret_cast<const void*>(k_merge), dim3(plan.merge), dim3(kBlock), 0, KID_MERGE);
      break;
    case FK_BLEND: {
      const size_t smem = BlendSmemBytes(f.blend_radius);
      if (f.blend_radius < 1 || f.blend_radius > kMaxBlendRadius || smem > kBlendSmemLimit)
        return SetError(SM_ERR_INVALID_ARGUMENT, "measurement_blending_radius too large for one tile region per SM");
      const dim3 pixel_tiles((d.width + kBlendTileW - 1) / kBlendTileW, (d.height + kBlendTileH - 1) / kBlendTileH);
      out->Reset(reinterpret_cast<const void*>(k_blend), pixel_tiles, dim3(kBlendBlock), smem, KID_BLEND);
      break;
    }
    case FK_INTEGRATE:
      out->Reset(reinterpret_cast<const void*>(k_integrate), dim3(plan.integrate), dim3(kBlock), 0, KID_INTEGRATE);
      break;
    case FK_UPDATE_NEIGHBORS:
      out->Reset(reinterpret_cast<const void*>(k_update_neighbors), dim3(plan.update_neighbors), dim3(kBlock), 0,
                 KID_UPDATE_NEIGHBORS);
      break;
    case FK_SCAN:
      out->Reset(reinterpret_cast<const void*>(k_new_surfel_scan), dim3(scan_tiles), dim3(kBlock), 0, KID_NEW_SURFEL_SCAN);
      break;
    case FK_CREATE:
      out->Reset(reinterpret_cast<const void*>(k_create_surfels), dim3(plan.sm_count * 2), dim3(kBlock), 0, KID_CREATE_SURFELS);
      break;
    default:
      return SetError(SM_ERR_INVALID_ARGUMENT, "DescribeFrameKernel");
  }
  out->Arg(d);
  out->Arg(f);
  if (which == FK_PROJECT) out->Arg(static_cast<int>(kProjectAll));
  if (which == FK_PROJECT_MAIN) out->Arg(static_cast<int>(kProjectMain));
  if (which == FK_PROJECT_TAIL) out->Arg(static_cast<int>(kProjectTail));
  return SM_OK;
}

namespace {
int LaunchFrameKernel(cudaStream_t stream, FrameKernel which, const LaunchPlan& plan, const DeviceState& d,
                      const FrameParams& f, bool dependent) {
  KernelLaunch k;
  const int status = DescribeFrameKernel(which, plan, d, f, &k);
  if (status != SM_OK) return status;
  LaunchOnStream(stream, k, dependent);
  return SM_OK;
}
}

int ClearAssociationRasters(cudaStream_t stream, const DeviceState& d) {
  const int blocks = (d.width * d.height + kBlock * 4 - 1) / (kBlock * 4);
  { LaunchScope scope(stream, KID_CLEAR); LaunchKernel(k_clear, dim3(blocks), dim3(kBlock), 0, stream, d); }
  return CheckLaunch("clear");
}

int IntegrateFrame(cudaStream_t stream, const DeviceState& d, const FrameParams& f, bool do_blending,
                   bool rasters_already_cleared, const LaunchPlan& plan, const IntegrateEvents* events) {
  const bool timed = events && events->enabled;
  auto record = [&](int i) { if (timed) cudaEventRecord(events->ev[i], stream); };
  int status = SM_OK;
  auto launch = [&](FrameKernel which, bool dependent) {
    if (status == SM_OK) status = LaunchFrameKernel(stream, which, plan, d, f, dependent);
  };
  record(0);
  if (!rasters_already_cleared) {
    status = ClearAssociationRasters(stream, d);
    if (status != SM_OK) return status;
  }
  launch(FK_PROJECT, false);
  launch(FK_ASSOCIATE, true);
  record(1); record(2);
  launch(FK_MERGE, false);
  record(3); record(4);
  if (do_blending) launch(FK_BLEND, true);
  record(5); record(6);
  launch(FK_INTEGRATE, false);
  record(7); record(8);
  launch(FK_UPDATE_NEIGHBORS, false);
  record(9); record(10);
  launch(FK_SCAN, false);
  launch(FK_CREATE, false);
  record(11);
  if (status != SM_OK) return status;
  return CheckLaunch("integrate");
}

int IntegrateFramePipelined(cudaStream_t stream, PipelineCtx* pc, int set, DeviceState& d, const FrameParams& f,
                            bool do_blending, const RegularizeArgs& reg, const LaunchPlan& plan) {
  cudaStream_t crit = pc->crit, side = pc->side;
  int status = SM_OK;
  auto launch = [&](cudaStream_t s, FrameKernel which, bool dependent) {
    if (status == SM_OK) status = LaunchFrameKernel(s, which, plan, d, f, dependent);
  };
  if (pc->have_frame) SM_EV(cudaStreamWaitEvent(stream, pc->ev_create[set ^ 1], 0));
  launch(stream, FK_PROJECT, false);
  launch(stream, FK_ASSOCIATE, true);
  SM_EV(cudaEventRecord(pc->ev_assoc, stream));
  SM_EV(cudaStreamWaitEvent(side, pc->ev_assoc, 0));
  launch(side, FK_MERGE, false);
  SM_EV(cudaEventRecord(pc->ev_merge, side));
  if (do_blending) launch(stream, FK_BLEND, true);
  SM_EV(cudaEventRecord(pc->ev_blend, stream));
  SM_EV(cudaStreamWaitEvent(side, pc->ev_blend, 0));
  launch(side, FK_SCAN, false);
  SM_EV(cudaStreamWaitEvent(crit, pc->ev_blend, 0));
  SM_EV(cudaStreamWaitEvent(crit, pc->ev_merge, 0));
  launch(crit, FK_INTEGRATE, false);
  SM_EV(cudaEventRecord(pc->ev_integrate, crit));
  launch(crit, FK_UPDATE_NEIGHBORS, true);
  SM_EV(cudaEventRecord(pc->ev_update[set], crit));
  SM_EV(cudaStreamWaitEvent(side, pc->ev_integrate, 0));
  launch(side, FK_CREATE, false);
  SM_EV(cudaEventRecord(pc->ev_create[set], side));
  SM_EV(cudaStreamWaitEvent(crit, pc->ev_create[set], 0));
  if (status != SM_OK) return status;
  status = CheckLaunch("integrate (pipelined)");
// ... 72 lines not shown
```

surfelmeshing_b200/csrc/knn.cu:

```cuda

#include <algorithm>
#include <climits>
#include <cmath>
#include <cstring>
#include <string>

#include "sm_handle.cuh"
#include "sm_math.cuh"

struct sm_knn_index {
  int device = 0;
  int sm_count = 0;
  smb::u32 capacity = 0;
  smb::u32 table_size = 0;
  smb::u32* bucket_start = nullptr;
  smb::u32* bucket_cursor = nullptr;
  smb::u32* scan_sums = nullptr;
  smb::u32* point_bucket = nullptr;
  float4* records = nullptr;
  smb::u32 point_count = 0;
  float cell_size = 0.f;
  float inverse_cell_size = 0.f;
  bool built = false;
  smb::u32 batch_points = 0;
// ... 400 lines not shown
              k->bucket_cursor, k->point_bucket, k->records};
  const u32 scan_n = k->table_size + 1;
  const u32 tiles = (scan_n + kScanTile - 1) / kScanTile;
  if (n > 0) {
    const int blocks = static_cast<int>(std::min<u32>((n + kBuildBlock - 1) / kBuildBlock, 8u * k->sm_count));
    k_knn_count<<<blocks, kBuildBlock, 0, stream>>>(a);
    k_knn_scan_tiles<<<tiles, kScanBlock, 0, stream>>>(k->bucket_start, scan_n, k->scan_sums);
    k_knn_scan_sums<<<1, kScanBlock, 0, stream>>>(k->scan_sums, tiles);
    k_knn_scan_add<<<tiles, kScanBlock, 0, stream>>>(k->bucket_start, scan_n, k->scan_sums);
    k_knn_scatter<<<blocks, kBuildBlock, 0, stream>>>(a);
  }
  SM_CUDA(cudaGetLastError());
  k->built = true;
  return SM_OK;
}

int KnnQuery(sm_knn_index* k, cudaStream_t stream, u32 query_count, const float* qx, const float* qy, const float* qz,
             const float* radius_squared, float radius_scale, const u8* state, int include_completed, int include_free,
             int max_result_count, float* out_distance_squared, u32* out_index, int* out_count) {
  if (!k->built) return SetError(SM_ERR_INVALID_ARGUMENT, "sm_knn_query: the index has not been built");
  if (max_result_count < 1 || max_result_count > kMaxResults) {
    return SetError(SM_ERR_INVALID_ARGUMENT, "sm_knn_query: max_result_count must be in [1, 64]");
  }
  if (query_count == 0) return SM_OK;
  QueryArgs a{query_count, qx, qy, qz, radius_squared, radius_scale, state, include_completed, include_free, max_result_count,
              k->inverse_cell_size, k->table_size - 1, k->bucket_start, k->records, out_distance_squared, out_index,
              out_count};
  const u32 needed = (query_count + kQueryBlock / 32 - 1) / (kQueryBlock / 32);
  const int blocks = static_cast<int>(std::min<u32>(needed, 16u * k->sm_count));
  k_knn_query<<<blocks, kQueryBlock, 0, stream>>>(a);
  SM_CUDA(cudaGetLastError());
  return SM_OK;
}

int KnnBatchHost(sm_knn_index* k, cudaStream_t stream, u32 n, const float* x, const float* y, const float* z,
                 const float* radius_squared, float radius_factor_squared, float cell_size, int max_result_count,
                 float* out_distance_squared, u32* out_index, int* out_count) {
  if (n > k->capacity) return SetError(SM_ERR_INVALID_ARGUMENT, "sm_knn_batch_host: more points than the index was created for");
  if (max_result_count < 1 || max_result_count > kMaxResults) {
    return SetError(SM_ERR_INVALID_ARGUMENT, "sm_knn_batch_host: max_result_count must be in [1, 64]");
  }
  if (!(radius_factor_squared > 0.f)) return SetError(SM_ERR_INVALID_ARGUMENT, "sm_knn_batch_host: radius_factor_squared must be positive");
  if (n == 0) return SM_OK;
  if (!(cell_size > 0.f)) {
    float largest = 0.f;
    for (u32 i = 0; i < n; ++i) largest = std::max(largest, radius_squared[i]);
    if (!(largest > 0.f)) largest = 1.f;
    cell_size = 2.f * std::sqrt(largest * radius_factor_squared);
  }
  if (k->batch_points < n || k->batch_k < max_result_count) {
    SM_CUDA(cudaStreamSynchronize(stream));
    cudaFree(k->batch_rows); cudaFree(k->batch_distance_squared); cudaFree(k->batch_index); cudaFree(k->batch_count);
    k->batch_rows = nullptr; k->batch_distance_squared = nullptr; k->batch_index = nullptr; k->batch_count = nullptr;
    k->batch_points = 0;
    const size_t points = std::min<size_t>(k->capacity, std::max<size_t>(n, 1u << 16));
    const size_t width = static_cast<size_t>(std::max(max_result_count, k->batch_k));
    SM_CUDA(cudaMalloc(&k->batch_rows, sizeof(float) * 4 * points));
    SM_CUDA(cudaMalloc(&k->batch_distance_squared, sizeof(float) * width * points));
    SM_CUDA(cudaMalloc(&k->batch_index, sizeof(u32) * width * points));
    SM_CUDA(cudaMalloc(&k->batch_count, sizeof(int) * points));
    k->batch_points = static_cast<u32>(points);
    k->batch_k = static_cast<int>(width);
  }
  const size_t stride = k->batch_points;
  float* dx = k->batch_rows;
  float* dy = dx + stride;
  float* dz = dy + stride;
  float* dr = dz + stride;
  const size_t bytes = sizeof(float) * n;
  SM_CUDA(cudaMemcpyAsync(dx, x, bytes, cudaMemcpyHostToDevice, stream));
  SM_CUDA(cudaMemcpyAsync(dy, y, bytes, cudaMemcpyHostToDevice, stream));
  SM_CUDA(cudaMemcpyAsync(dz, z, bytes, cudaMemcpyHostToDevice, stream));
  SM_CUDA(cudaMemcpyAsync(dr, radius_squared, bytes, cudaMemcpyHostToDevice, stream));
  int status = KnnBuild(k, stream, n, dx, dy, dz, dr, nullptr, cell_size);
  if (status != SM_OK) return status;
  status = KnnQuery(k, stream, n, dx, dy, dz, dr, radius_factor_squared, nullptr, 1, 1, max_result_count,
                    k->batch_distance_squared, k->batch_index, k->batch_count);
  if (status != SM_OK) return status;
  constexpr u32 kChunk = 1u << 16;
  const size_t chunk_bytes = static_cast<size_t>(kChunk) * (kMaxResults * 8 + 4);
  for (int i = 0; i < 2; ++i) {
    if (!k->bounce[i]) SM_CUDA(cudaMallocHost(&k->bounce[i], chunk_bytes));
    if (!k->bounce_ready[i]) SM_CUDA(cudaEventCreateWithFlags(&k->bounce_ready[i], cudaEventDisableTiming));
  }
  const u32 chunks = (n + kChunk - 1) / kChunk;
  auto enqueue = [&](u32 c) -> int {
    const u32 first = c * kChunk, count = std::min(kChunk, n - first);
    const size_t row = static_cast<size_t>(count) * max_result_count;
    char* b = static_cast<char*>(k->bounce[c & 1]);
    SM_CUDA(cudaMemcpyAsync(b, k->batch_distance_squared + static_cast<size_t>(first) * max_result_count, sizeof(float) * row,
                            cudaMemcpyDeviceToHost, stream));
    SM_CUDA(cudaMemcpyAsync(b + sizeof(float) * row, k->batch_index + static_cast<size_t>(first) * max_result_count,
                            sizeof(u32) * row, cudaMemcpyDeviceToHost, stream));
    SM_CUDA(cudaMemcpyAsync(b + 2 * sizeof(float) * row, k->batch_count + first, sizeof(int) * count, cudaMemcpyDeviceToHost, stream));
    SM_CUDA(cudaEventRecord(k->bounce_ready[c & 1], stream));
    return SM_OK;
  };
  status = enqueue(0);
  if (status != SM_OK) return status;
  for (u32 c = 0; c < chunks; ++c) {
    if (c + 1 < chunks) {
      status = enqueue(c + 1);
      if (status != SM_OK) return status;
    }
    SM_CUDA(cudaEventSynchronize(k->bounce_ready[c & 1]));
    const u32 first = c * kChunk, count = std::min(kChunk, n - first);
    const size_t row = static_cast<size_t>(count) * max_result_count;
    const char* b = static_cast<const char*>(k->bounce[c & 1]);
    std::memcpy(out_distance_squared + static_cast<size_t>(first) * max_result_count, b, sizeof(float) * row);
    std::memcpy(out_index + static_cast<size_t>(first) * max_result_count, b + sizeof(float) * row, sizeof(u32) * row);
    std::memcpy(out_count + first, b + 2 * sizeof(float) * row, sizeof(int) * count);
  }
  SM_CUDA(cudaStreamSynchronize(stream));
  return SM_OK;
}

}

extern "C" {

int sm_knn_create(sm_knn_index** out, uint32_t max_points) {
  if (!out || max_points == 0 || max_points > (1u << 26)) {
    return smb::SetError(SM_ERR_INVALID_ARGUMENT, "sm_knn_create: need out and 1 <= max_points <= 2^26");
  }
  sm_knn_index* k = new sm_knn_index;
  const int status = smb::CreateIndex(k, max_points);
  if (status != SM_OK) {
    smb::FreeIndex(k);
    return status;
  }
  *out = k;
  return SM_OK;
}

void sm_knn_destroy(sm_knn_index* k) {
  if (k) smb::FreeIndex(k);
}

int sm_knn_build(sm_knn_index* k, void* stream, uint32_t point_count, const float* x, const float* y, const float* z,
                 const float* radius_squared, const uint8_t* state, float cell_size) {
  if (!k || (point_count && (!x || !y || !z))) return smb::SetError(SM_ERR_INVALID_ARGUMENT, "sm_knn_build: null argument");
  return smb::KnnBuild(k, static_cast<cudaStream_t>(stream), point_count, x, y, z, radius_squared, state, cell_size);
}

int sm_knn_build_from_reconstruction(sm_knn_index* k, sm_reconstruction* r, void* stream_v, float cell_size,
                                     uint32_t* out_point_count) {
  if (!k || !r) return smb::SetError(SM_ERR_INVALID_ARGUMENT, "sm_knn_build_from_reconstruction: null argument");
  cudaStream_t stream = static_cast<cudaStream_t>(stream_v);
  uint32_t n = 0;
  const int status = sm_surfels_size(r, &n);
  if (status != SM_OK) return status;
  if (out_point_count) *out_point_count = n;
  const size_t st = r->d.stride;
  return smb::KnnBuild(k, stream, n, r->d.smooth, r->d.smooth + st, r->d.smooth + 2 * st,
                       r->d.surfels + SM_ROW_RADIUS_SQUARED * st, nullptr, cell_size);
}

int sm_knn_query(sm_knn_index* k, void* stream, uint32_t query_count, const float* qx, const float* qy, const float* qz,
                 const float* radius_squared, const uint8_t* state, int32_t include_completed, int32_t include_free,
                 int32_t max_result_count, float* out_distance_squared, uint32_t* out_index, int32_t* out_count) {
  if (!k || (query_count && (!qx || !qy || !qz || !radius_squared || !out_distance_squared || !out_index || !out_count))) {
    return smb::SetError(SM_ERR_INVALID_ARGUMENT, "sm_knn_query: null argument");
  }
  return smb::KnnQuery(k, static_cast<cudaStream_t>(stream), query_count, qx, qy, qz, radius_squared, 1.0f, state,
                       include_completed, include_free, max_result_count, out_distance_squared, out_index, out_count);
}

int sm_knn_batch_host(sm_knn_index* k, void* stream, uint32_t point_count, const float* x, const float* y, const float* z,
                      const float* radius_squared, float radius_factor_squared, float cell_size, int32_t max_result_count,
                      float* out_distance_squared, uint32_t* out_index, int32_t* out_count) {
  if (!k || (point_count && (!x || !y || !z || !radius_squared || !out_distance_squared || !out_index || !out_count))) {
    return smb::SetError(SM_ERR_INVALID_ARGUMENT, "sm_knn_batch_host: null argument");
  }
  return smb::KnnBatchHost(k, static_cast<cudaStream_t>(stream), point_count, x, y, z, radius_squared, radius_factor_squared,
                           cell_size, max_result_count, out_distance_squared, out_index, out_count);
}

}
```

surfelmeshing_b200/csrc/pipeline.cu:

```cuda

#include <chrono>
#include <cstdio>
#include <cstdlib>
#include <string>

#include "sm_handle.cuh"

namespace smb {

namespace {

#define SM_CUDA(call)                                                                                   \
  do {                                                                                                  \
    const cudaError_t e_ = (call);                                                                      \
    if (e_ != cudaSuccess) return SetError(SM_ERR_CUDA, (std::string(#call) + ": " + cudaGetErrorString(e_)).c_str()); \
  } while (0)

constexpr int kDepthRing = 16;
constexpr int kColorRing = 6;
constexpr int kIterationEvents = 32;

int EnvInt(const char* name, int fallback) {
  const char* e = std::getenv(name);
  return (e && e[0]) ? std::atoi(e) : fallback;
// ... 259 lines not shown
      size_t color_pitch;
      const uint8_t* color = c.Color(frame, &color_pitch);
      status = IntegrateImpl(r, stream, static_cast<u32>(frame), *c.ip, r->run_depth[set], r->run_depth_pitch,
                             reinterpret_cast<const float*>(r->run_normals[set]), r->run_normals_pitch,
                             r->run_radius[set], r->run_radius_pitch, color, color_pitch,
                             c.s->global_T_frame + 12 * frame, c.s->frame_T_global + 12 * frame);
      if (status != SM_OK) return status;
      SM_CUDA(cudaEventRecord(r->int_done[set], stream));
    }
    ++*integrated;
  }
  if (pipelined && r->pipe.have_frame) SM_CUDA(cudaStreamWaitEvent(stream, r->pipe.ev_reg, 0));
  return SM_OK;
}

}

struct FrameGraph {
  cudaGraph_t graph = nullptr;
  cudaGraphExec_t exec = nullptr;
  std::vector<cudaGraphNode_t> nodes;
  std::vector<const void*> funcs;
  int blending = -1, reg_launches = -1, pdl = -1, prio = -1, order = -1;
  size_t blend_smem = 0;
  dim3 scan_grid;
};

void DestroyFrameGraph(FrameGraph* g) {
  if (!g) return;
  if (g->exec) cudaGraphExecDestroy(g->exec);
  if (g->graph) cudaGraphDestroy(g->graph);
  delete g;
}

namespace {

struct StepLayout {
  int integrate, scan, update, create, reg0, reg_count, project, project_tail , associate,
      merge, blend , bilateral, tail, count;
};

StepLayout MakeLayout(bool blending, int reg_launches, bool split_project) {
  StepLayout l;
  int n = 0;
  l.integrate = n++; l.scan = n++; l.update = n++; l.create = n++;
  l.reg0 = n; l.reg_count = reg_launches; n += reg_launches;
  l.project = n++;
  l.project_tail = split_project ? n++ : -1;
  l.associate = n++; l.merge = n++;
  l.blend = blending ? n++ : -1;
  l.bilateral = n++; l.tail = n++;
  l.count = n;
  return l;
}

cudaKernelNodeParams NodeParams(const KernelLaunch& k) {
  cudaKernelNodeParams p = {};
  p.func = const_cast<void*>(k.func);
  p.gridDim = k.grid;
  p.blockDim = k.block;
  p.sharedMemBytes = static_cast<unsigned>(k.smem);
  p.kernelParams = const_cast<void**>(k.args);
  p.extra = nullptr;
  return p;
}

constexpr int kDefaultGraphOrder = 0;

int BuildFrameGraph(FrameGraph* g, const StepLayout& l, const std::vector<KernelLaunch>& launches, int pdl) {
  SM_CUDA(cudaGraphCreate(&g->graph, 0));
  g->nodes.assign(l.count, nullptr);
  g->funcs.assign(l.count, nullptr);
  for (int i = 0; i < l.count; ++i) {
    const cudaKernelNodeParams p = NodeParams(launches[i]);
    SM_CUDA(cudaGraphAddKernelNode(&g->nodes[i], g->graph, nullptr, 0, &p));
    g->funcs[i] = launches[i].func;
  }
  if (const int prio = EnvInt("SM_B200_GRAPH_PRIO", 0)) {
    int least = 0, greatest = 0;
    SM_CUDA(cudaDeviceGetStreamPriorityRange(&least, &greatest));
    auto set_priority = [&](int node, int priority) -> int {
      if (node < 0) return SM_OK;
      cudaKernelNodeAttrValue v = {};
      v.priority = priority;
      SM_CUDA(cudaGraphKernelNodeSetAttribute(g->nodes[node], cudaKernelNodeAttributePriority, &v));
      return SM_OK;
    };
    const int mid = (least + greatest) / 2;
    for (int i = 0; i < l.count; ++i) { const int st = set_priority(i, prio >= 2 ? mid : least); if (st != SM_OK) return st; }
    for (int node : {l.integrate, l.create, l.project, l.project_tail, l.associate, l.blend}) { const int st = set_priority(node, greatest); if (st != SM_OK) return st; }
    if (prio >= 2) for (int node : {l.bilateral, l.tail}) { const int st = set_priority(node, least); if (st != SM_OK) return st; }
  }
  std::vector<cudaGraphNode_t> from, to;
  std::vector<cudaGraphEdgeData> data;
  auto edge = [&](int a, int b, bool programmatic) {
    from.push_back(g->nodes[a]);
    to.push_back(g->nodes[b]);
    cudaGraphEdgeData e = {};
    if (pdl == 2 || (pdl == 1 && programmatic)) {
      e.from_port = cudaGraphKernelNodePortProgrammatic;
      e.type = cudaGraphDependencyTypeProgrammatic;
    }
    data.push_back(e);
  };
  edge(l.integrate, l.update, true);
  edge(l.integrate, l.create, false);
  edge(l.scan, l.create, false);
  if (l.reg_count > 0) {
    edge(l.update, l.reg0, false);
    edge(l.create, l.reg0, false);
    for (int i = 1; i < l.reg_count; ++i) edge(l.reg0 + i - 1, l.reg0 + i, true);
  }
  if (l.project_tail >= 0) {
    edge(l.integrate, l.project, false);
    edge(l.create, l.project_tail, false);
    edge(l.project, l.associate, false);
    edge(l.project_tail, l.associate, false);
  } else {
    edge(l.create, l.project, false);
    edge(l.project, l.associate, true);
  }
  edge(l.associate, l.merge, false);
  if (l.blend >= 0) edge(l.associate, l.blend, true);
  edge(l.bilateral, l.tail, true);
  const int order = EnvInt("SM_B200_GRAPH_ORDER", kDefaultGraphOrder);
  if (order & 1) edge(l.create, l.update, false);
  if ((order & 2) && l.reg_count > 0) edge(l.associate, l.reg0, false);
  if ((order & 4) && l.reg_count > 0) edge(l.merge, l.reg0, false);
  if (order & 8) edge(l.project_tail >= 0 ? l.project_tail : l.project, l.update, false);
  SM_CUDA(cudaGraphAddDependencies_v2(g->graph, from.data(), to.data(), data.data(), from.size()));
  SM_CUDA(cudaGraphInstantiate(&g->exec, g->graph, 0));
  return SM_OK;
}

int RunGraph(RunContext& c, cudaStream_t stream, uint32_t* integrated) {
  sm_reconstruction* r = c.r;
  const int W = c.W, H = c.H, half = c.half;
  const bool blending = c.ip->do_blending != 0;
  const int iterations = c.ip->regularization_iterations_per_integration_iteration;
  const bool disable_denoising = iterations == 0;
  const int reg_launches = disable_denoising ? 1 : 2 * iterations;
  const bool split_project = EnvInt("SM_B200_SPLIT_PROJECT", 0) != 0;
  const StepLayout l = MakeLayout(blending, reg_launches, split_project);
  const int pdl = EnvInt("SM_B200_GRAPH_PDL", 0);
  std::vector<KernelLaunch> launches(l.count);

  cudaStream_t gs = r->graph_stream;
  SM_CUDA(cudaEventRecord(r->entry_event, stream));
  SM_CUDA(cudaStreamWaitEvent(gs, r->entry_event, 0));
  if (c.depth_ring) SM_CUDA(cudaStreamWaitEvent(r->upload_stream, r->entry_event, 0));
  int uploaded_until = c.first - half - 1;
  const int it0 = c.first - 2;

  float* smooth = r->d.smooth;
  float* smooth_next = r->d.smooth_next;

  auto active = [&](int frame) { return frame >= c.first && frame < c.last; };
  auto clamp_frame = [&](int frame) { return frame < c.first ? c.first : (frame >= c.last ? c.last - 1 : frame); };

  for (int it = it0; it < c.last; ++it) {
    const int crit = it, front = it + 1, pre = it + 2;
    if (c.depth_ring && active(pre)) {
      for (int f = uploaded_until + 1; f <= pre + half; ++f) {
        const int last_reader_step = f - kDepthRing + half - 2;
        if (last_reader_step >= it0) SM_CUDA(cudaStreamWaitEvent(r->upload_stream, r->iteration_done[(last_reader_step - it0) % kIterationEvents], 0));
        const int st = c.EnqueueRawFrame(f);
        if (st != SM_OK) return st;
      }
      uploaded_until = pre + half;
      if (c.color_ring) {
        const int last_color_step = pre - kColorRing;
        if (last_color_step >= it0) SM_CUDA(cudaStreamWaitEvent(r->upload_stream, r->iteration_done[(last_color_step - it0) % kIterationEvents], 0));
        const int st = c.EnqueueColorFrame(pre);
        if (st != SM_OK) return st;
      }
      SM_CUDA(cudaEventRecord(r->upload_done, r->upload_stream));
      SM_CUDA(cudaStreamWaitEvent(gs, r->upload_done, 0));
    }

    int status = SM_OK;
    {
      const int frame = clamp_frame(crit), set = frame % kSets;
      DeviceState d = c.SetState(set);
      d.smooth = smooth; d.smooth_next = smooth_next;
      if (active(crit)) RecordOperation(r, static_cast<int>(static_cast<u32>(frame) - static_cast<u32>(c.ip->regularization_frame_window_size)));
      FrameParams f = c.Params(frame, set);
      f.skip = active(crit) ? 0 : 1;
      if (active(crit)) r->last_tiebreak = f.tb;
      const FrameKernel kernels[4] = {FK_INTEGRATE, FK_SCAN, FK_UPDATE_NEIGHBORS, FK_CREATE};
      const int slots[4] = {l.integrate, l.scan, l.update, l.create};
      for (int i = 0; i < 4; ++i) {
        status = DescribeFrameKernel(kernels[i], r->plan, d, f, &launches[slots[i]]);
        if (status != SM_OK) return status;
      }
      const int old_slot = f.count_slot, new_slot = (f.count_slot + 1) % kCountSlots;
      if (active(crit)) NoteIntegratedFrame(d, static_cast<u32>(frame));
      for (int i = 0; i < (disable_denoising ? 1 : iterations); ++i) {
        KernelLaunch* first = &launches[l.reg0 + (disable_denoising ? 0 : 2 * i)];
        KernelLaunch* second = disable_denoising ? nullptr : first + 1;
        DescribeRegularize(first, second, !active(crit), r->plan, d, disable_denoising, static_cast<u32>(frame),
                           c.ip->radius_factor_for_regularization_neighbors, c.ip->regularizer_weight,
                           c.ip->regularization_frame_window_size, new_slot, i == 0 ? old_slot : -1);
        if (!disable_denoising && active(crit)) {
          float* const filled = smooth_next;
          smooth_next = smooth;
          smooth = filled;
          d.smooth = smooth; d.smooth_next = smooth_next;
          NoteRegStep(d, static_cast<u32>(frame), c.ip->regularization_frame_window_size);
        }
      }
      r->d.reg_t_prev = d.reg_t_prev;
      r->d.reg_full_sweep = d.reg_full_sweep;
      if (active(crit)) ++*integrated;
    }
    {
      const int frame = clamp_frame(front), set = frame % kSets;
      const DeviceState d = c.SetState(set);
      FrameParams f = c.Params(frame, set);
      f.skip = active(front) ? 0 : 1;
      const FrameKernel kernels[5] = {split_project ? FK_PROJECT_MAIN : FK_PROJECT, FK_PROJECT_TAIL, FK_ASSOCIATE, FK_MERGE, FK_BLEND};
      const int slots[5] = {l.project, l.project_tail, l.associate, l.merge, l.blend};
      for (int i = 0; i < 5; ++i) {
        if (slots[i] < 0) continue;
        status = DescribeFrameKernel(kernels[i], r->plan, d, f, &launches[slots[i]]);
        if (status != SM_OK) return status;
      }
    }
    {
      const int frame = clamp_frame(pre), set = frame % kSets;
      const u16* others[8];
      size_t other_pitches[8];
      c.Others(frame, others, other_pitches);
      size_t raw_pitch;
      const u16* raw = c.Raw(frame, &raw_pitch);
      status = DescribePreprocess(&launches[l.bilateral], &launches[l.tail], !active(pre), *c.pp, W, H, r->fx, r->fy,
                                  r->cx, r->cy, raw, raw_pitch, others, other_pitches,
                                  c.s->others_TR_reference + static_cast<size_t>(frame) * c.K * 12, r->scratch_B,
                                  r->scratch_B_pitch, r->run_depth[set], r->run_depth_pitch, r->run_normals[set],
                                  r->run_normals_pitch, r->run_radius[set], r->run_radius_pitch, r->assoc_set[set],
                                  r->first_depth_set[set], r->supported_set[set], r->run_depth_pre[set],
                                  r->run_depth_pitch, TimelineSlot(r->d, static_cast<u32>(frame), KID_BILATERAL_OUTLIER),
                                  TimelineSlot(r->d, static_cast<u32>(frame), KID_ERODE_NORMALS_RADII), r->ScratchBMap());
      if (status != SM_OK) return status;
    }

    FrameGraph* g = r->graph;
    const int prio = EnvInt("SM_B200_GRAPH_PRIO", 0);
    const int order = EnvInt("SM_B200_GRAPH_ORDER", kDefaultGraphOrder);
    bool rebuild = g == nullptr || g->blending != (blending ? 1 : 0) || g->reg_launches != reg_launches || g->pdl != pdl ||
                   g->prio != prio || g->order != order || static_cast<int>(g->nodes.size()) != l.count;
    if (!rebuild) {
      for (int i = 0; i < l.count && !rebuild; ++i) rebuild = g->funcs[i] != launches[i].func;
      if (l.blend >= 0) rebuild = rebuild || g->blend_smem != launches[l.blend].smem;
    }
    if (rebuild) {
      if (g) { SM_CUDA(cudaStreamSynchronize(gs)); DestroyFrameGraph(g); r->graph = nullptr; }
      g = new FrameGraph();
      r->graph = g;
      g->blending = blending ? 1 : 0; g->reg_launches = reg_launches; g->pdl = pdl; g->prio = prio; g->order = order;
      g->blend_smem = l.blend >= 0 ? launches[l.blend].smem : 0;
      status = BuildFrameGraph(g, l, launches, pdl);
      if (status != SM_OK) return status;
    } else {
      for (int i = 0; i < l.count; ++i) {
        const cudaKernelNodeParams p = NodeParams(launches[i]);
        SM_CUDA(cudaGraphExecKernelNodeSetParams(g->exec, g->nodes[i], &p));
      }
    }
    SM_CUDA(cudaGraphLaunch(g->exec, gs));
    CountLaunches(static_cast<unsigned long long>(l.count));
    if (c.depth_ring) SM_CUDA(cudaEventRecord(r->iteration_done[(it - it0) % kIterationEvents], gs));
  }
  r->d.smooth = smooth;
  r->d.smooth_next = smooth_next;
  {
    const DeviceState last_set = c.SetState((c.last - 1) % kSets);
    r->d.assoc = last_set.assoc; r->d.first_depth = last_set.first_depth; r->d.supported = last_set.supported;
    r->d.vis = last_set.vis; r->d.seg_count = last_set.seg_count; r->d.merge_flag = last_set.merge_flag;
    r->d.upd_list = last_set.upd_list; r->d.upd_count = last_set.upd_count;
  }
  r->count_slot = c.CountSlot(c.last);
  SM_CUDA(cudaEventRecord(r->graph_exit, gs));
  SM_CUDA(cudaStreamWaitEvent(stream, r->graph_exit, 0));
  return SM_OK;
}

}

int StreamRun(sm_reconstruction* r, cudaStream_t stream, const sm_stream_desc* s, const sm_preprocess_params* pp,
              const sm_integrate_params* ip, int first_frame, int last_frame, sm_stream_stats* stats) {
  RunContext c;
  c.r = r; c.s = s; c.pp = pp; c.ip = ip;
  c.W = r->d.width; c.H = r->d.height;
  c.pyramid = r->pyramid_level;
  if (c.pyramid > 0) {
    if (r->median_iterations > 0) {
      return SetError(SM_ERR_INVALID_ARGUMENT, "pyramid_level > 0 cannot be combined with median_filter_and_densify_iterations > 0");
    }
    const int step = 1 << c.pyramid;
    if (s->width <= 0 || s->height <= 0 || s->width % step != 0 || s->height % step != 0 ||
        (s->width >> c.pyramid) != c.W || (s->height >> c.pyramid) != c.H) {
      return SetError(SM_ERR_INVALID_ARGUMENT, "stream size must be the handle's size times 2^pyramid_level");
    }
  } else if (s->width != c.W || s->height != c.H) {
    return SetError(SM_ERR_INVALID_ARGUMENT, "stream size mismatch");
  }
  c.source_W = s->width; c.source_H = s->height;
  c.source_elems = static_cast<size_t>(c.source_W) * c.source_H;
  c.K = pp->outlier_filtering_frame_count;
  c.half = c.K / 2;
  if (c.K < 2 || c.K > 8 || first_frame < c.half || last_frame > s->frame_count - c.half || first_frame > last_frame) {
    return SetError(SM_ERR_INVALID_ARGUMENT,
                    "frame range needs outlier_filtering_frame_count/2 frames on both sides (main.cc:987-992)");
  }
  c.first = first_frame; c.last = last_frame;
  c.frame_elems = static_cast<size_t>(c.W) * c.H;
  c.on_host = s->frames_on_host != 0;
  c.depth_ring = c.on_host || r->median_iterations > 0 || c.pyramid > 0;
  c.color_ring = c.on_host || c.pyramid > 0;
  c.base_slot = r->count_slot;
  int status = EnsureRunBuffers(r, c.on_host, c.depth_ring, c.color_ring, c.source_W, c.source_H);
  if (status != SM_OK) return status;
  const unsigned long long launches_before = LaunchCount();
  const auto host_t0 = std::chrono::steady_clock::now();
  r->last_stream = stream;

  const bool serial = r->events.enabled || ProfilingEnabled();
  const int radius = static_cast<int>(pp->bilateral_filter_radius_factor * pp->bilateral_filter_sigma_xy + 0.5f);
  const bool use_graph = !serial && EnvInt("SM_B200_GRAPH", 1) != 0 && radius == 6 && first_frame < last_frame;
  uint32_t integrated = 0;
  if (use_graph) {
    status = RunGraph(c, stream, &integrated);
    if (status != SM_OK) cudaStreamSynchronize(r->graph_stream);
  } else {
    status = RunStreams(c, stream, !serial, &integrated);
    if (status != SM_OK) cudaDeviceSynchronize();
  }
  if (status != SM_OK) return status;
  const double host_enqueue_ms = std::chrono::duration<double, std::milli>(std::chrono::steady_clock::now() - host_t0).count();
  status = FetchCounters(r, stream);
  if (stats) {
    stats->frames_integrated = integrated;
    stats->surfels_size = r->host_counters->surfel_count[r->count_slot];
    stats->surfel_count = stats->surfels_size - r->host_counters->merge_count;
    stats->kernel_launches = LaunchCount() - launches_before;
    stats->h2d_bytes = c.h2d;
    stats->d2h_bytes = sizeof(Counters);
    stats->host_enqueue_ms = host_enqueue_ms;
  }
  return status;
}

}
```

surfelmeshing_b200/csrc/regularize.cu:

```cuda

#include <algorithm>
#include <cstdlib>

#include "sm_kernels.cuh"

namespace smb {

namespace {

#define SM_S(row, i) d.surfels[static_cast<size_t>(row) * d.stride + (i)]
#define SM_SU(row, i) reinterpret_cast<u32*>(d.surfels)[static_cast<size_t>(row) * d.stride + (i)]
#define SM_SMOOTH(axis, i) d.smooth[static_cast<size_t>(axis) * d.stride + (i)]
#define SM_SMOOTH_NEXT(axis, i) d.smooth_next[static_cast<size_t>(axis) * d.stride + (i)]

constexpr int kBlock = 256;
#ifndef SM_REG_ACCUMULATE_MIN_BLOCKS
#define SM_REG_ACCUMULATE_MIN_BLOCKS 1
#endif
#ifndef SM_REG_STEP_MIN_BLOCKS
#define SM_REG_STEP_MIN_BLOCKS 1
#endif

struct RegParams {
  u32 frame_index;
  int window;
  float radius_factor_squared;
  float regularizer_weight;
  int count_slot;
  int remove_below_slot;
  int skip;
  int t_prev;
  int full_sweep;
};

__device__ __forceinline__ bool outside_window(u32 stamp, const RegParams& p) {
  return static_cast<int>(stamp) < static_cast<int>(p.frame_index - static_cast<u32>(p.window));
}

__global__ void __launch_bounds__(kBlock, SM_REG_ACCUMULATE_MIN_BLOCKS) k_reg_accumulate(DeviceState d, RegParams p) {
  pdl_prologue();
  if (p.skip) return;
  const TimelineScope timeline_scope(d, p.frame_index, KID_REG_ACCUMULATE);
  const u32 n = d.counters->surfel_count[p.count_slot];
  const u32 n_remove = p.remove_below_slot >= 0 ? d.counters->surfel_count[p.remove_below_slot] : 0u;
  const u32 step = gridDim.x * blockDim.x;
  u32 i = blockIdx.x * blockDim.x + threadIdx.x;
  u32 nbr_ahead[4] = {kInvalidIndex, kInvalidIndex, kInvalidIndex, kInvalidIndex};
  if (i < d.stride) {
#pragma unroll
    for (int k = 0; k < 4; ++k) nbr_ahead[k] = SM_SU(SM_ROW_NEIGHBOR0 + k, i);
  }
  for (; i < n; i += step) {
    u32 nbr[4];
#pragma unroll
    for (int k = 0; k < 4; ++k) nbr[k] = nbr_ahead[k];
    if (i + step < n) {
#pragma unroll
      for (int k = 0; k < 4; ++k) nbr_ahead[k] = SM_SU(SM_ROW_NEIGHBOR0 + k, i + step);
    }
    if ((nbr[0] & nbr[1] & nbr[2] & nbr[3]) == kInvalidIndex) continue;

    u32 meta[4];
#pragma unroll
    for (int k = 0; k < 4; ++k) {
      const u32 q = nbr[k] != kInvalidIndex ? nbr[k] : i;
      meta[k] = SM_SU(kRowMeta, q);
    }
    const float sx = SM_SMOOTH(0, i), sy = SM_SMOOTH(1, i), sz = SM_SMOOTH(2, i);
    const float nx = SM_S(SM_ROW_NORMAL_X, i), ny = SM_S(SM_ROW_NORMAL_Y, i), nz = SM_S(SM_ROW_NORMAL_Z, i);
    const float radius_squared = SM_S(SM_ROW_RADIUS_SQUARED, i);

    bool use[4];
    int neighbor_count = 0;
#pragma unroll
    for (int k = 0; k < 4; ++k) {
      if (i < n_remove && nbr[k] != kInvalidIndex && (meta[k] & kMetaDetachBit)) {
        nbr[k] = kInvalidIndex;
        SM_SU(SM_ROW_NEIGHBOR0 + k, i) = kInvalidIndex;
      }
      use[k] = nbr[k] != kInvalidIndex && !outside_window(meta[k] & ~kMetaDetachBit, p);
      neighbor_count += use[k] ? 1 : 0;
    }
    if (neighbor_count == 0) continue;

    float qx[4], qy[4], qz[4];
#pragma unroll
    for (int k = 0; k < 4; ++k) {
      const u32 q = use[k] ? nbr[k] : i;
      qx[k] = SM_SMOOTH(0, q);
      qy[k] = SM_SMOOTH(1, q);
      qz[k] = SM_SMOOTH(2, q);
    }
    const float max_distance_squared = fmul(radius_squared, p.radius_factor_squared);
    const float rcp_count = frcp(i2f(neighbor_count));
    const float factor = fmul(fadd(p.regularizer_weight, p.regularizer_weight), rcp_count);
    const float weight_term = fmul(rcp_count, p.regularizer_weight);
#pragma unroll
    for (int k = 0; k < 4; ++k) {
      if (!use[k]) continue;
      const u32 q = nbr[k];
      const float dx = fsub(qx[k], sx);
      const float dy = fsub(qy[k], sy);
      const float dz = fsub(qz[k], sz);
      const float f = fmul(factor, ffma(nz, dz, ffma(nx, dx, fmul(ny, dy))));
      atomicAdd(&d.gradient[q], make_float4(fmul(nx, f), fmul(ny, f), fmul(nz, f), weight_term));
      if (squared_norm(dx, dy, dz) > max_distance_squared) SM_SU(SM_ROW_NEIGHBOR0 + k, i) = kInvalidIndex;
    }
  }
}

__global__ void __launch_bounds__(kBlock, SM_REG_STEP_MIN_BLOCKS) k_reg_step(DeviceState d, RegParams p) {
  pdl_prologue();
  if (p.skip) return;
  const TimelineScope timeline_scope(d, p.frame_index, KID_REG_STEP);
  const u32 n = d.counters->surfel_count[p.count_slot];
  const u32 step = gridDim.x * blockDim.x;
  u32 i = blockIdx.x * blockDim.x + threadIdx.x;
  u32 stamp_ahead = 0;
  if (i < d.stride) stamp_ahead = SM_SU(SM_ROW_LAST_UPDATE_STAMP, i);
  for (; i < n; i += step) {
    const u32 stamp = stamp_ahead;
    if (i + step < n) stamp_ahead = SM_SU(SM_ROW_LAST_UPDATE_STAMP, i + step);
    if (outside_window(stamp, p)) {
      if (p.full_sweep || static_cast<int>(stamp) >= p.t_prev) {
        SM_SMOOTH_NEXT(0, i) = SM_SMOOTH(0, i); SM_SMOOTH_NEXT(1, i) = SM_SMOOTH(1, i); SM_SMOOTH_NEXT(2, i) = SM_SMOOTH(2, i);
      }
      continue;
    }
    u32 nbr[4];
#pragma unroll
    for (int k = 0; k < 4; ++k) nbr[k] = SM_SU(SM_ROW_NEIGHBOR0 + k, i);
    const float sx = SM_SMOOTH(0, i), sy = SM_SMOOTH(1, i), sz = SM_SMOOTH(2, i);
    const float nx = SM_S(SM_ROW_NORMAL_X, i), ny = SM_S(SM_ROW_NORMAL_Y, i), nz = SM_S(SM_ROW_NORMAL_Z, i);
    const float4 accumulated = d.gradient[i];
    float gx = ffma(fsub(sx, SM_S(SM_ROW_X, i)), 2.0f, accumulated.x);
    float gy = ffma(fsub(sy, SM_S(SM_ROW_Y, i)), 2.0f, accumulated.y);
    float gz = ffma(fsub(sz, SM_S(SM_ROW_Z, i)), 2.0f, accumulated.z);
    int neighbor_count = 0;
    float rx = 0.f, ry = 0.f, rz = 0.f;
    float qx[4], qy[4], qz[4];
#pragma unroll
    for (int k = 0; k < 4; ++k) {
      const u32 q = nbr[k] != kInvalidIndex ? nbr[k] : i;
      qx[k] = SM_SMOOTH(0, q);
      qy[k] = SM_SMOOTH(1, q);
      qz[k] = SM_SMOOTH(2, q);
    }
#pragma unroll
    for (int k = 0; k < 4; ++k) {
      if (nbr[k] == kInvalidIndex) continue;
      ++neighbor_count;
      const float dx = fsub(qx[k], sx);
      const float dy = fsub(qy[k], sy);
      const float dz = fsub(qz[k], sz);
      const float normal_dot_difference = ffma(nz, dz, ffma(nx, dx, fmul(ny, dy)));
      rx = ffma(-nx, normal_dot_difference, rx);
      ry = ffma(-ny, normal_dot_difference, ry);
      rz = ffma(-nz, normal_dot_difference, rz);
    }
    if (neighbor_count > 0) {
      const float factor = fmul(fadd(p.regularizer_weight, p.regularizer_weight), frcp(i2f(neighbor_count)));
      gx = ffma(factor, rx, gx);
      gy = ffma(factor, ry, gy);
      gz = ffma(factor, rz, gz);
    }
    const float gradient_length = fsqrt_approx(ffma(gz, gz, ffma(gx, gx, fmul(gy, gy))));
    const float residual_terms_weight_sum = fadd(fadd(p.regularizer_weight, 1.0f), accumulated.w);
    float step_factor = fmul(frcp(residual_terms_weight_sum), 0.5f);
    const float max_step_length = fsqrt_approx(SM_S(SM_ROW_RADIUS_SQUARED, i));
    const float step_length = fmul(step_factor, gradient_length);
    if (step_length > max_step_length) step_factor = fmul(step_factor, fmul(max_step_length, frcp(step_length)));
    SM_SMOOTH_NEXT(0, i) = ffma(step_factor, -gx, sx);
    SM_SMOOTH_NEXT(1, i) = ffma(step_factor, -gy, sy);
    SM_SMOOTH_NEXT(2, i) = ffma(step_factor, -gz, sz);
    d.gradient[i] = make_float4(0.f, 0.f, 0.f, 0.f);
  }
}

__global__ void __launch_bounds__(kBlock) k_reg_copy_only(DeviceState d, RegParams p) {
  pdl_prologue();
  if (p.skip) return;
  const TimelineScope timeline_scope(d, p.frame_index, KID_REG_COPY_ONLY);
  const u32 n = d.counters->surfel_count[p.count_slot];
  const u32 n_remove = p.remove_below_slot >= 0 ? d.counters->surfel_count[p.remove_below_slot] : 0u;
  for (u32 i = blockIdx.x * blockDim.x + threadIdx.x; i < n; i += gridDim.x * blockDim.x) {
    if (i < n_remove) {
#pragma unroll
      for (int k = 0; k < 4; ++k) {
        const u32 q = SM_SU(SM_ROW_NEIGHBOR0 + k, i);
        if (q != kInvalidIndex && (SM_SU(SM_ROW_COLOR, q) >> 24) == 1u) SM_SU(SM_ROW_NEIGHBOR0 + k, i) = kInvalidIndex;
      }
    }
    if (outside_window(SM_SU(SM_ROW_LAST_UPDATE_STAMP, i), p)) continue;
    const float x = SM_S(SM_ROW_X, i), y = SM_S(SM_ROW_Y, i), z = SM_S(SM_ROW_Z, i);
    SM_SMOOTH(0, i) = x; SM_SMOOTH(1, i) = y; SM_SMOOTH(2, i) = z;
    SM_SMOOTH_NEXT(0, i) = x; SM_SMOOTH_NEXT(1, i) = y; SM_SMOOTH_NEXT(2, i) = z;
  }
}

}

namespace {
__global__ void __launch_bounds__(kBlock) k_rebuild_meta(DeviceState d, u32 count) {
  for (u32 i = blockIdx.x * blockDim.x + threadIdx.x; i < count; i += gridDim.x * blockDim.x) {
    const u32 flag = (SM_SU(SM_ROW_COLOR, i) >> 24) == 1u ? kMetaDetachBit : 0u;
    SM_SU(kRowMeta, i) = (SM_SU(SM_ROW_LAST_UPDATE_STAMP, i) & ~kMetaDetachBit) | flag;
  }
}
}

int RebuildMetaRow(cudaStream_t stream, const DeviceState& d, u32 count, int sm_count) {
  if (count == 0) return SM_OK;
  k_rebuild_meta<<<sm_count * 4, kBlock, 0, stream>>>(d, count);
  return CheckLaunch("rebuild meta row");
}

int DescribeRegularize(KernelLaunch* first, KernelLaunch* second, bool skip, const LaunchPlan& plan,
                       const DeviceState& d, bool disable_denoising, u32 frame_index,
                       float radius_factor_for_regularization_neighbors, float regularizer_weight,
                       int regularization_frame_window_size, int count_slot, int remove_replaced_below_slot) {
  RegParams p;
  p.frame_index = frame_index;
  p.window = regularization_frame_window_size;
  p.radius_factor_squared =
      radius_factor_for_regularization_neighbors * radius_factor_for_regularization_neighbors;
  p.regularizer_weight = regularizer_weight;
  p.count_slot = count_slot;
  p.remove_below_slot = remove_replaced_below_slot;
  p.skip = skip ? 1 : 0;
  p.t_prev = d.reg_t_prev;
  p.full_sweep = d.reg_full_sweep;
  static_assert(sizeof(DeviceState) + sizeof(RegParams) + 32 <= sizeof(first->storage), "KernelLaunch::storage too small");
  if (disable_denoising) {
    first->Reset(reinterpret_cast<const void*>(k_reg_copy_only), dim3(plan.reg_copy), dim3(kBlock), 0, KID_REG_COPY_ONLY);
    first->Arg(d);
    first->Arg(p);
    return 1;
  }
  first->Reset(reinterpret_cast<const void*>(k_reg_accumulate), dim3(plan.reg_accumulate), dim3(kBlock), 0, KID_REG_ACCUMULATE);
  first->Arg(d);
  first->Arg(p);
  second->Reset(reinterpret_cast<const void*>(k_reg_step), dim3(plan.reg_step), dim3(kBlock), 0, KID_REG_STEP);
  second->Arg(d);
  second->Arg(p);
  return 2;
}

int RegularizeSurfels(cudaStream_t stream, DeviceState& d, bool disable_denoising, u32 frame_index,
                      float radius_factor_for_regularization_neighbors, float regularizer_weight,
                      int regularization_frame_window_size, int count_slot, int remove_replaced_below_slot,
                      const LaunchPlan& plan) {
  KernelLaunch first, second;
  const int n = DescribeRegularize(&first, &second, false, plan, d, disable_denoising, frame_index,
                                   radius_factor_for_regularization_neighbors, regularizer_weight,
                                   regularization_frame_window_size, count_slot, remove_replaced_below_slot);
  LaunchOnStream(stream, first, false);
  if (n == 1) return CheckLaunch("regularize (copy only)");
  LaunchOnStream(stream, second, true);
  float* const filled = d.smooth_next;
  d.smooth_next = d.smooth;
  d.smooth = filled;
  NoteRegStep(d, frame_index, regularization_frame_window_size);
  return CheckLaunch("regularize");
}

int ConfigureRegularizeKernels(int carveout_percent, LaunchPlan* plan) {
  if (carveout_percent >= 0) {
    cudaFuncSetAttribute(k_reg_accumulate, cudaFuncAttributePreferredSharedMemoryCarveout, carveout_percent);
    cudaFuncSetAttribute(k_reg_step, cudaFuncAttributePreferredSharedMemoryCarveout, carveout_percent);
    cudaFuncSetAttribute(k_reg_copy_only, cudaFuncAttributePreferredSharedMemoryCarveout, carveout_percent);
    cudaGetLastError();
  }
  const char* e = std::getenv("SM_B200_RESIDENT_GRIDS");
  auto resident = [&](auto kernel) {
    int per_sm = 0;
    if ((e && e[0] == '0') || cudaOccupancyMaxActiveBlocksPerMultiprocessor(&per_sm, kernel, kBlock, 0) != cudaSuccess || per_sm < 1) {
      cudaGetLastError();
      per_sm = 8;
    }
    return ScaleGrid(plan->sm_count * per_sm);
  };
  plan->reg_accumulate = resident(k_reg_accumulate);
  plan->reg_step = resident(k_reg_step);
  plan->reg_copy = resident(k_reg_copy_only);
  if (const char* pe = std::getenv("SM_B200_OFFCHAIN_GRID_PERCENT")) {
    const int percent = std::atoi(pe);
    if (percent > 0 && percent < 100) {
      plan->reg_accumulate = std::max(plan->sm_count, plan->reg_accumulate * percent / 100);
      plan->reg_step = std::max(plan->sm_count, plan->reg_step * percent / 100);
    }
  }
  return SM_OK;
}

}
```

surfelmeshing_b200/csrc/sm_handle.cuh:

```cuda
#pragma once

#include <vector>

#include "sm_kernels.cuh"

namespace smb {

constexpr int kSets = 3;

struct TieBreakConfig {
  u32 wave;
  double early_fraction;
  double index_order_fraction;
  double early_fraction_later, index_order_fraction_later;
  double early_fraction_second;
  u32 wave_offset;
  u32 lane_request;
  u32 lane_shift;
  u32 mul, mul_inv;
};
constexpr u32 kDefaultTieBreakWave = 264 * 1024;
constexpr u32 kDefaultTieBreakLaneShift = 5;
constexpr u32 kDefaultTieBreakWaveOffset = 0;
constexpr double kDefaultTieBreakEarlyFraction = 0.015;
constexpr double kDefaultTieBreakIndexOrderFraction = 0.25;
constexpr double kDefaultTieBreakEarlyFractionLater = 0.04;
constexpr double kDefaultTieBreakIndexOrderFractionLater = 0.45;
constexpr double kDefaultTieBreakEarlyFractionSecond = 0.02;
TieBreak MakeTieBreak(const TieBreakConfig& cfg, u32 frame_index);
int SetTieBreakWave(TieBreakConfig* cfg, u32 wave, u32 capacity);

struct FrameGraph;
void DestroyFrameGraph(FrameGraph* g);

}

struct sm_reconstruction {
  smb::DeviceState d{};
  int device = 0;
  int sm_count = 0;
  smb::LaunchPlan plan{};
  float fx = 0, fy = 0, cx = 0, cy = 0;
  int count_slot = 0;
  bool rasters_cleared = false;
  smb::IntegrateEvents events{};
  smb::TieBreakConfig tiebreak{};
  smb::TieBreak last_tiebreak{};
  smb::Counters* host_counters = nullptr;
  cudaStream_t last_stream = nullptr;
  smb::u16* scratch_B = nullptr; size_t scratch_B_pitch = 0;
  smb::TensorMapStorage scratch_B_map{};
  bool scratch_B_map_valid = false;
  const smb::TensorMapStorage* ScratchBMap() const { return scratch_B_map_valid ? &scratch_B_map : nullptr; }
  smb::u16* blend_src = nullptr; size_t blend_src_pitch = 0;
  smb::PixelAssoc* assoc_set[smb::kSets] = {};
  float* first_depth_set[smb::kSets] = {};
  smb::u8* supported_set[smb::kSets] = {};
  smb::VisEntry* vis_set[smb::kSets] = {};
  smb::u32* seg_count_set[smb::kSets] = {};
  smb::u8* merge_flag_set[smb::kSets] = {};
  uint2* upd_list_set[smb::kSets] = {};
  smb::u32* upd_count_set[smb::kSets] = {};
  smb::u16* run_depth[smb::kSets] = {}; size_t run_depth_pitch = 0;
  float2* run_normals[smb::kSets] = {}; size_t run_normals_pitch = 0;
  float* run_radius[smb::kSets] = {}; size_t run_radius_pitch = 0;
  smb::u16* run_depth_pre[smb::kSets] = {};
  float* smooth_alt = nullptr;
  smb::PipelineCtx pipe{};
  cudaStream_t pre_stream = nullptr;
  cudaEvent_t pre_done[2] = {nullptr, nullptr}, int_done[2] = {nullptr, nullptr}, entry_event = nullptr;
  std::vector<smb::u16*> ring_depth; size_t ring_depth_pitch = 0;
  std::vector<uchar3*> ring_color; size_t ring_color_pitch = 0;
  cudaStream_t upload_stream = nullptr;
  cudaEvent_t upload_done = nullptr;
  int median_iterations = 0;
  smb::u16* median_stage[2] = {nullptr, nullptr}; size_t median_stage_pitch = 0;
  int pyramid_level = 0;
  smb::u16* pyramid_depth_stage = nullptr; size_t pyramid_depth_stage_pitch = 0;
  smb::u8* pyramid_color_stage = nullptr; size_t pyramid_color_stage_pitch = 0;
  int pyramid_stage_width = 0, pyramid_stage_height = 0;
  std::vector<cudaEvent_t> iteration_done;
  smb::u32 op_epoch = 0;
  uint64_t state_generation = 1;
  struct Operation { smb::u32 epoch; int stamp_threshold; };
  std::vector<Operation> op_history;
  smb::u32* delta_index = nullptr; float* delta_values = nullptr; smb::u32* delta_cursor = nullptr;
  smb::u32 delta_capacity = 0;
  smb::u32* delta_host = nullptr; size_t delta_host_capacity = 0;
  cudaStream_t graph_stream = nullptr;
  cudaEvent_t graph_exit = nullptr;
  smb::FrameGraph* graph = nullptr;
};

namespace smb {
int FetchCounters(sm_reconstruction* r, cudaStream_t stream);
FrameParams MakeFrameParams(const sm_reconstruction* r, u32 frame_index, int count_slot, const sm_integrate_params& p,
                            u16* depth, size_t depth_pitch, const u16* depth_pre, size_t depth_pre_pitch,
                            const float* normals, size_t normals_pitch, const float* radius, size_t radius_pitch,
                            const uint8_t* color, size_t color_pitch, const float* global_T_local,
                            const float* local_T_global);
int IntegrateImpl(sm_reconstruction* r, cudaStream_t stream, u32 frame_index, const sm_integrate_params& p, u16* depth,
                  size_t depth_pitch, const float* normals, size_t normals_pitch, const float* radius,
                  size_t radius_pitch, const uint8_t* color, size_t color_pitch, const float* global_T_local,
                  const float* local_T_global);
void CountLaunches(unsigned long long n);
unsigned long long LaunchCount();
void RecordOperation(sm_reconstruction* r, int stamp_threshold);
void FreeTransferBuffers(sm_reconstruction* r);
int TransferDelta(sm_reconstruction* r, cudaStream_t stream, uint32_t frame_index, sm_transfer_token* token, float* x,
                  float* y, float* z, float* radius_squared, float* nx, float* ny, float* nz,
                  uint32_t* last_update_stamp, sm_transfer_stats* stats);
int UpdateVisualizationBuffers(sm_reconstruction* r, cudaStream_t stream, const sm_visualization_params& p, float* vertex,
                               uint32_t* neighbor_index, float* normal_vertex);
int StreamRun(sm_reconstruction* r, cudaStream_t stream, const sm_stream_desc* s, const sm_preprocess_params* pp,
              const sm_integrate_params* ip, int first_frame, int last_frame, sm_stream_stats* stats);
}
```

surfelmeshing_b200/csrc/sm_kernels.cuh:

```cuda
#pragma once

#include <cuda_runtime.h>
#include <math.h>
#include <stddef.h>
#include <stdint.h>
#include <string.h>

#include "../../include/surfel_b200.h"
#include "sm_math.cuh"

namespace smb {

int SetError(int code, const char* message);
int CheckLaunch(const char* what);

enum KernelId {
  KID_CLEAR = 0, KID_BILATERAL_OUTLIER, KID_BILATERAL_GENERIC, KID_OUTLIER, KID_ERODE_NORMALS_RADII, KID_ERODE,
  KID_NORMALS, KID_RADII, KID_PROJECT, KID_ASSOCIATE, KID_MERGE, KID_BLEND, KID_INTEGRATE, KID_UPDATE_NEIGHBORS,
  KID_NEW_SURFEL_SCAN, KID_CREATE_SURFELS, KID_REG_ACCUMULATE, KID_REG_STEP, KID_REG_COPY_ONLY,
  KID_EXPORT_VERTICES, KID_MEDIAN_DENSIFY, KID_DELTA_SELECT, KID_VIZ_BUFFERS, KID_PROJECT_TAIL, KID_DOWNSCALE_DEPTH,
  KID_DOWNSCALE_COLOR, KID_COUNT
};
const char* KernelName(int id);
bool ProfilingEnabled();
class LaunchScope {
 public:
  LaunchScope(cudaStream_t stream, KernelId id);
  ~LaunchScope();
 private:
  cudaStream_t stream_;
  int slot_;
};

inline Mat3x4 MakeMat3x4(const float* m) {
  Mat3x4 r;
  r.r0 = make_float4(m[0], m[1], m[2], m[3]);
  r.r1 = make_float4(m[4], m[5], m[6], m[7]);
  r.r2 = make_float4(m[8], m[9], m[10], m[11]);
  return r;
}


constexpr u32 kInvalidIndex = 0xFFFFFFFFu;

constexpr int kRowMergeEpoch = SM_ROW_ACCUM_X;
constexpr int kRowMeta = SM_ROW_ACCUM_Y;
constexpr u32 kMetaDetachBit = 0x80000000u;
constexpr int kSegment = 1024;
constexpr u32 kActiveBit = 0x80000000u;

constexpr u32 kSecondaryBit = 0x80000000u;
struct TieBreak {
  u32 wave;
  u32 lane_shift;
  u32 groups;
  u32 mul, mul_inv;
  u32 add;
  u32 salt;
  u32 early_threshold;
  u32 index_order_threshold;
  u32 early_threshold_second;
  u32 early_threshold_later, index_order_threshold_later;
  u32 wave_offset;
  u64 wave_reciprocal;
  u64 group_reciprocal;
};
__host__ __device__ __forceinline__ u64 tb_divide(u64 x, u32 d, u64 reciprocal, u32* remainder) {
#if defined(__CUDA_ARCH__)
  u64 q = __umul64hi(x, reciprocal);
#else
  u64 q = static_cast<u64>((static_cast<unsigned __int128>(x) * reciprocal) >> 64);
#endif
  u64 r = x - q * d;
  while (r >= d) { r -= d; ++q; }
  *remainder = static_cast<u32>(r);
  return q;
}
__host__ __device__ __forceinline__ u32 tb_hash(u32 x) {
  x ^= x >> 16; x *= 0x7feb352du; x ^= x >> 15; x *= 0x846ca68bu; x ^= x >> 16;
  return x;
}
__host__ __device__ __forceinline__ bool tb_index_order(const TieBreak& t, u32 pixel, u32 wave_index) {
  return tb_hash(pixel ^ ~t.salt) < (wave_index == 0 ? t.index_order_threshold : t.index_order_threshold_later);
}
__host__ __device__ __forceinline__ u32 tb_phase(const TieBreak& t, u32 pixel) {
  if (!t.wave_offset) return 0u;
  u32 g;
  tb_divide(tb_hash(pixel ^ t.salt ^ 0x5bd1e995u), t.groups, t.group_reciprocal, &g);
  return g << t.lane_shift;
}
__host__ __device__ __forceinline__ u32 tb_encode(const TieBreak& t, u32 idx, bool secondary, u32 pixel) {
  if (t.wave == 0) return idx | (secondary ? kSecondaryBit : 0u);
  u32 r, rp;
  const u32 w = static_cast<u32>(tb_divide(static_cast<u64>(idx) + tb_phase(t, pixel), t.wave, t.wave_reciprocal, &r));
  if (tb_index_order(t, pixel, w)) {
    rp = r;
  } else {
    u32 gp;
    tb_divide(static_cast<u64>(r >> t.lane_shift) * t.mul + t.add, t.groups, t.group_reciprocal, &gp);
    rp = (gp << t.lane_shift) | (r & ((1u << t.lane_shift) - 1u));
  }
  const bool late = secondary && !(tb_hash(idx ^ t.salt) <
                                   (w == 0 ? t.early_threshold : (w == 1 ? t.early_threshold_second : t.early_threshold_later)));
  return w * (2u * t.wave) + (late ? t.wave : 0u) + rp;
}
__host__ __device__ __forceinline__ u32 supporting_index(const TieBreak& t, u32 key, u32 pixel) {
  if (key == kInvalidIndex) return kInvalidIndex;
  if (t.wave == 0) return key & ~kSecondaryBit;
  u32 rem;
  const u32 w2 = static_cast<u32>(tb_divide(key, t.wave, t.wave_reciprocal, &rem));
  const u32 w = w2 >> 1;
  u32 r = rem;
  if (!tb_index_order(t, pixel, w)) {
    const u32 gp = rem >> t.lane_shift;
    const u32 shifted = gp >= t.add ? gp - t.add : gp + t.groups - t.add;
    u32 g;
    tb_divide(static_cast<u64>(shifted) * t.mul_inv, t.groups, t.group_reciprocal, &g);
    r = (g << t.lane_shift) | (rem & ((1u << t.lane_shift) - 1u));
  }
  return w * t.wave + r - tb_phase(t, pixel);
}

typedef uint4 PixelAssoc;

typedef uint4 VisEntry;

constexpr int kCountSlots = 3;
struct Counters {
  u32 surfel_count[kCountSlots];
  u32 merge_count;
  u32 new_surfel_count;
  u32 capacity_overflow;
  u32 scan_ticket;
  u32 pad;
};

struct DeviceState {
  float* surfels;
  size_t stride;
  u32 capacity;
  int width, height;
  PixelAssoc* assoc;
  float* first_depth;
  u8* supported;
  VisEntry* vis;
  u32* seg_count;
  u8* merge_flag;
  uint2* upd_list;
  u32* upd_count;
  u8* new_flag;
  u32* new_index;
  u32* new_list;
  unsigned long long* scan_state;
  Counters* counters;
  float4* gradient;
  float* smooth;
  float* smooth_next;
  int reg_t_prev;
  int reg_full_sweep;
  unsigned long long* timeline;
  u32 timeline_frames;
};

struct FrameParams {
  u32 frame_index;
  int count_slot;
  int skip;
  u32 op_epoch;
  TieBreak tb;
  int active_window;
  float fx, fy, cx, cy;
  float fx_inv, fy_inv, cx_inv, cy_inv;
  float sensor_noise_factor;
  float cos_normal_compatibility_threshold;
  float max_surfel_confidence;
  float depth_scaling;
  float inv_depth_scaling;
  float radius_factor_squared;
  int blend_radius;
  Mat3x4 local_T_global;
  Mat3x4 global_T_local;
  u16* depth; size_t depth_pitch;
  const u16* depth_pre; size_t depth_pre_pitch;
  const float2* normals; size_t normals_pitch;
  const float* radius; size_t radius_pitch;
  const uchar3* color; size_t color_pitch;
};

__device__ __forceinline__ void pdl_prologue() {
#if defined(__CUDA_ARCH__)
  asm volatile("griddepcontrol.launch_dependents;");
  asm volatile("griddepcontrol.wait;" ::: "memory");
#endif
}
__device__ __forceinline__ unsigned long long globaltimer_ns() {
  unsigned long long t;
  asm volatile("mov.u64 %0, %globaltimer;" : "=l"(t));
  return t;
}
struct TimelineScope {
  unsigned long long* slot;
  __device__ __forceinline__ explicit TimelineScope(unsigned long long* s) : slot(s) { begin(); }
  __device__ __forceinline__ TimelineScope(const DeviceState& d, u32 frame, int kernel_id)
      : slot(d.timeline ? d.timeline + (static_cast<size_t>(frame % d.timeline_frames) * KID_COUNT + kernel_id) * 2 : nullptr) {
    begin();
  }
  __device__ __forceinline__ void begin() {
    if (slot && threadIdx.x == 0 && blockIdx.x < 8 && blockIdx.y == 0) atomicMin(slot, globaltimer_ns());
  }
  __device__ __forceinline__ ~TimelineScope() {
    if (slot && threadIdx.x == 0) atomicMax(slot + 1, globaltimer_ns());
  }
};
inline unsigned long long* TimelineSlot(const DeviceState& d, u32 frame, int kernel_id) {
  return d.timeline ? d.timeline + (static_cast<size_t>(frame % d.timeline_frames) * KID_COUNT + kernel_id) * 2 : nullptr;
}

int PdlMode();
int ScaleGrid(int blocks);

template <typename... KArgs, typename... Args>
inline void LaunchKernelImpl(bool dependent, void (*kernel)(KArgs...), dim3 grid, dim3 block, size_t smem,
                             cudaStream_t stream, Args&&... args) {
  cudaLaunchConfig_t cfg = {};
  cfg.gridDim = grid;
  cfg.blockDim = block;
  cfg.dynamicSmemBytes = smem;
  cfg.stream = stream;
  cudaLaunchAttribute attr[1];
  attr[0].id = cudaLaunchAttributeProgrammaticStreamSerialization;
  attr[0].val.programmaticStreamSerializationAllowed = 1;
  cfg.attrs = attr;
  const int mode = PdlMode();
  cfg.numAttrs = (mode == 2 || (mode == 1 && dependent)) ? 1 : 0;
  cudaLaunchKernelEx(&cfg, kernel, static_cast<KArgs>(args)...);
}
template <typename... KArgs, typename... Args>
inline void LaunchKernel(void (*kernel)(KArgs...), dim3 grid, dim3 block, size_t smem, cudaStream_t stream,
                         Args&&... args) {
  LaunchKernelImpl(false, kernel, grid, block, smem, stream, static_cast<Args&&>(args)...);
}
template <typename... KArgs, typename... Args>
inline void LaunchDependent(void (*kernel)(KArgs...), dim3 grid, dim3 block, size_t smem, cudaStream_t stream,
                            Args&&... args) {
  LaunchKernelImpl(true, kernel, grid, block, smem, stream, static_cast<Args&&>(args)...);
}

struct KernelLaunch {
  const void* func;
  dim3 grid, block;
  size_t smem;
  int kernel_id;
  int arg_count;
  void* args[4];
  alignas(64) unsigned char storage[2304];
  size_t used;
  void Reset(const void* f, dim3 g, dim3 b, size_t shared, int id) {
    func = f; grid = g; block = b; smem = shared; kernel_id = id; arg_count = 0; used = 0;
  }
  template <typename T>
  void Arg(const T& v) {
    used = (used + alignof(T) - 1) / alignof(T) * alignof(T);
    static_assert(alignof(T) <= 64, "argument alignment");
    memcpy(storage + used, &v, sizeof(T));
    args[arg_count++] = storage + used;
    used += sizeof(T);
  }
};
void LaunchOnStream(cudaStream_t stream, const KernelLaunch& k, bool dependent);

struct LaunchPlan {
  int sm_count;
  int project, associate, merge, integrate, update_neighbors;
  int reg_accumulate, reg_step, reg_copy;
};
int ConfigurePreprocessKernels(int carveout_percent);
int ConfigureIntegrateKernels(int carveout_percent, LaunchPlan* plan);
int ConfigureRegularizeKernels(int carveout_percent, LaunchPlan* plan);

struct alignas(64) TensorMapStorage { unsigned char bytes[128]; };
int MakeDepthTensorMap(TensorMapStorage* out, const u16* base, size_t pitch_bytes, int width, int height);
int PreprocessFused(cudaStream_t stream, const sm_preprocess_params& p, int width, int height, float fx, float fy,
                    float cx, float cy, const u16* raw, size_t raw_pitch, const u16* const* other_depths,
                    const size_t* other_pitches, const float* others_TR_reference, u16* scratch_B,
                    size_t scratch_B_pitch, u16* out_depth, size_t out_depth_pitch, float2* out_normals,
                    size_t out_normals_pitch, float* out_radius, size_t out_radius_pitch, uint4* clear_assoc,
                    float* clear_first_depth, u8* clear_supported, u16* out_depth_copy = nullptr,
                    size_t out_depth_copy_pitch = 0, unsigned long long* timeline_bilateral = nullptr,
                    unsigned long long* timeline_tail = nullptr, const TensorMapStorage* scratch_B_map = nullptr);
int DescribePreprocess(KernelLaunch* bilateral, KernelLaunch* tail, bool skip, const sm_preprocess_params& p, int width,
                       int height, float fx, float fy, float cx, float cy, const u16* raw, size_t raw_pitch,
                       const u16* const* other_depths, const size_t* other_pitches, const float* others_TR_reference,
                       u16* scratch_B, size_t scratch_B_pitch, u16* out_depth, size_t out_depth_pitch,
                       float2* out_normals, size_t out_normals_pitch, float* out_radius, size_t out_radius_pitch,
                       uint4* clear_assoc, float* clear_first_depth, u8* clear_supported, u16* out_depth_copy,
                       size_t out_depth_copy_pitch, unsigned long long* timeline_bilateral,
                       unsigned long long* timeline_tail, const TensorMapStorage* scratch_B_map);
int StageBilateral(cudaStream_t stream, float sigma_xy, float sigma_value_factor, u16 value_to_ignore,
                   float radius_factor, u16 max_depth, float depth_valid_region_radius, int width, int height,
                   const u16* in, size_t in_pitch, u16* out, size_t out_pitch);
int StageOutlier(cudaStream_t stream, int other_count, int required_count, float tolerance, float fx, float fy,
                 float cx, float cy, int width, int height, const u16* in, size_t in_pitch,
                 const u16* const* other_depths, const size_t* other_pitches, const float* others_TR_reference,
                 u16* out, size_t out_pitch);
int StageErode(cudaStream_t stream, int radius, int width, int height, const u16* in, size_t in_pitch, u16* out,
               size_t out_pitch);
int StageMedianDensify(cudaStream_t stream, int iterations, int width, int height, const u16* in, size_t in_pitch,
                       u16* out, size_t out_pitch, u16* scratch, size_t scratch_pitch);
int StageDownscaleMedian(cudaStream_t stream, u16 value_to_ignore, int in_width, int in_height, const u16* in,
                         size_t in_pitch, int out_width, int out_height, u16* out, size_t out_pitch);
int StageColorPyramid(cudaStream_t stream, int levels, int width, int height, const u8* in, size_t in_pitch, u8* out,
                      size_t out_pitch);
int StageNormals(cudaStream_t stream, float observation_angle_threshold_deg, float depth_scaling, float fx, float fy,
                 float cx, float cy, int width, int height, const u16* in, size_t in_pitch, u16* out, size_t out_pitch,
                 float2* normals, size_t normals_pitch);
int StageRadii(cudaStream_t stream, float point_radius_extension_factor, float point_radius_clamp_factor,
               float depth_scaling, float fx, float fy, float cx, float cy, int width, int height, const u16* in,
               size_t in_pitch, float* radius, size_t radius_pitch, u16* out, size_t out_pitch);

struct IntegrateEvents {
  cudaEvent_t ev[14];
  bool enabled;
};
int IntegrateFrame(cudaStream_t stream, const DeviceState& d, const FrameParams& f, bool do_blending,
                   bool rasters_already_cleared, const LaunchPlan& plan, const IntegrateEvents* events);
enum FrameKernel { FK_PROJECT = 0, FK_ASSOCIATE, FK_MERGE, FK_BLEND, FK_INTEGRATE, FK_UPDATE_NEIGHBORS, FK_SCAN, FK_CREATE,
                   FK_PROJECT_MAIN, FK_PROJECT_TAIL, FK_COUNT };
int DescribeFrameKernel(FrameKernel which, const LaunchPlan& plan, const DeviceState& d, const FrameParams& f,
                        KernelLaunch* out);
int ClearAssociationRasters(cudaStream_t stream, const DeviceState& d);

struct PipelineCtx {
  cudaStream_t front;
  cudaStream_t crit;
  cudaStream_t side;
  cudaEvent_t ev_assoc, ev_merge, ev_blend, ev_integrate;
  cudaEvent_t ev_create[2], ev_update[2];
  cudaEvent_t ev_reg;
  bool have_frame;
};
struct RegularizeArgs {
  bool disable_denoising;
  int iterations;
  float radius_factor, regularizer_weight;
  int window;
};
int IntegrateFramePipelined(cudaStream_t stream, PipelineCtx* pc, int set, DeviceState& d, const FrameParams& f,
                            bool do_blending, const RegularizeArgs& reg, const LaunchPlan& plan);
int ExportVertices(cudaStream_t stream, const DeviceState& d, int count_slot, int sm_count, float* position_buffer,
                   u8* color_buffer);

inline void NoteRegStep(DeviceState& d, u32 frame_index, int window) {
  d.reg_t_prev = static_cast<int>(frame_index - static_cast<u32>(window));
  d.reg_full_sweep = 0;
}
inline void NoteIntegratedFrame(DeviceState& d, u32 frame_index) {
  if (static_cast<int>(frame_index) < d.reg_t_prev) d.reg_t_prev = static_cast<int>(frame_index);
}
int RebuildMetaRow(cudaStream_t stream, const DeviceState& d, u32 count, int sm_count);
int RegularizeSurfels(cudaStream_t stream, DeviceState& d, bool disable_denoising, u32 frame_index,
                      float radius_factor_for_regularization_neighbors, float regularizer_weight,
                      int regularization_frame_window_size, int count_slot, int remove_replaced_below_slot,
                      const LaunchPlan& plan);
int DescribeRegularize(KernelLaunch* first, KernelLaunch* second, bool skip, const LaunchPlan& plan,
                       const DeviceState& d, bool disable_denoising, u32 frame_index,
                       float radius_factor_for_regularization_neighbors, float regularizer_weight,
                       int regularization_frame_window_size, int count_slot, int remove_replaced_below_slot);

}
```

surfelmeshing_b200/csrc/transfer.cu:

```cuda

#include <algorithm>
#include <chrono>
#include <cstdio>
#include <cstdlib>
#include <cstring>
#include <exception>
#include <string>
#include <thread>

#include "sm_handle.cuh"

namespace smb {

namespace {

#define SM_CUDA(call)                                                                                   \
  do {                                                                                                  \
    const cudaError_t e_ = (call);                                                                      \
    if (e_ != cudaSuccess) return SetError(SM_ERR_CUDA, (std::string(#call) + ": " + cudaGetErrorString(e_)).c_str()); \
  } while (0)

#define SM_S(row, i) d.surfels[static_cast<size_t>(row) * d.stride + (i)]
#define SM_SU(row, i) reinterpret_cast<u32*>(d.surfels)[static_cast<size_t>(row) * d.stride + (i)]
#define SM_SMOOTH(axis, i) d.smooth[static_cast<size_t>(axis) * d.stride + (i)]

constexpr int kBlock = 256;

struct DeltaArgs {
  int count_slot;
  u32 count_at_token;
  int stamp_threshold;
  u32 epoch_at_token;
  u32 capacity;
  u32* cursor;
  u32* index;
  float* values;
};

__global__ void __launch_bounds__(kBlock) k_delta_select(DeviceState d, DeltaArgs a) {
  const u32 n = d.counters->surfel_count[a.count_slot];
  const int lane = threadIdx.x & 31;
  for (u32 base = blockIdx.x * blockDim.x; base < n; base += gridDim.x * blockDim.x) {
    const u32 i = base + threadIdx.x;
    bool changed = false;
    u32 stamp = 0;
    float radius_squared = 0.f;
    if (i < n) {
      stamp = SM_SU(SM_ROW_LAST_UPDATE_STAMP, i);
      radius_squared = SM_S(SM_ROW_RADIUS_SQUARED, i);
      changed = i >= a.count_at_token || static_cast<int>(stamp) >= a.stamp_threshold ||
                (radius_squared < 0.f && SM_SU(kRowMergeEpoch, i) > a.epoch_at_token);
    }
    const unsigned mask = __ballot_sync(0xffffffffu, changed);
    if (mask == 0) continue;
    u32 warp_base = 0;
    if (lane == 0) warp_base = atomicAdd(a.cursor, static_cast<u32>(__popc(mask)));
    warp_base = __shfl_sync(0xffffffffu, warp_base, 0);
    if (!changed) continue;
    const u32 k = warp_base + __popc(mask & ((1u << lane) - 1u));
    if (k >= a.capacity) continue;
    a.index[k] = i;
    float* v = a.values + k;
    const size_t c = a.capacity;
    v[0 * c] = SM_SMOOTH(0, i);
    v[1 * c] = SM_SMOOTH(1, i);
    v[2 * c] = SM_SMOOTH(2, i);
    v[3 * c] = radius_squared;
    v[4 * c] = SM_S(SM_ROW_NORMAL_X, i);
    v[5 * c] = SM_S(SM_ROW_NORMAL_Y, i);
    v[6 * c] = SM_S(SM_ROW_NORMAL_Z, i);
    v[7 * c] = __uint_as_float(stamp);
  }
}

struct VizArgs {
  int count_slot;
  u32 frame_index;
  int active_window;
  u32 latest_triangulated_frame_index, latest_mesh_surfel_count;
  u32 point_size_in_floats;
  int mode;
  float* vertex;
  u32* neighbor_index;
  float* normal_vertex;
};

__device__ __forceinline__ u32 pack_rgb(u32 r, u32 g, u32 b) { return (r & 0xFFu) | ((g & 0xFFu) << 8) | ((b & 0xFFu) << 16); }

__global__ void __launch_bounds__(kBlock) k_viz_buffers(DeviceState d, VizArgs a) {
  const u32 n = d.counters->surfel_count[a.count_slot];
  for (u32 i = blockIdx.x * blockDim.x + threadIdx.x; i < n; i += gridDim.x * blockDim.x) {
    const float sx = SM_SMOOTH(0, i), sy = SM_SMOOTH(1, i), sz = SM_SMOOTH(2, i);
    if (a.vertex) {
      const u32 creation_stamp = SM_SU(SM_ROW_CREATION_STAMP, i);
      const bool output_vertex = creation_stamp <= a.latest_triangulated_frame_index || i >= a.latest_mesh_surfel_count;
      float* v = a.vertex + static_cast<size_t>(i) * a.point_size_in_floats;
      v[0] = output_vertex ? sx : __int_as_float(0x7fffffff);
      v[1] = sy;
      v[2] = sz;
      u32 color;
      if (a.mode == 1 || a.mode == 2) {
        const u32 stamp = a.mode == 2 ? creation_stamp : SM_SU(SM_ROW_LAST_UPDATE_STAMP, i);
        const int age = static_cast<int>(a.frame_index - stamp);
        const int max_age = a.mode == 2 ? 3000 : a.active_window;
        if (age < 1) {
          color = pack_rgb(255, 80, 80);
        } else if (age > max_age) {
          color = pack_rgb(40, 40, 255);
        } else {
          const float blend = __saturatef(fmul(u2f(static_cast<u32>(age - 1)), frcp(u2f(static_cast<u32>(max_age - 1)))));
          const u32 intensity = 255u - (f2u_trunc(fmul(blend, 255.99f)) & 0xFFu);
          color = pack_rgb(intensity, intensity, intensity);
        }
      } else if (a.mode == 3) {
        const float radius = fsqrt_approx(SM_S(SM_ROW_RADIUS_SQUARED, i));
        const float blend = __saturatef(fmul(fadd(radius, -0.0005f), 105.26316070556640625f));
        const u32 red = f2u_trunc(fmul(blend, 255.99f)) & 0xFFu;
        color = pack_rgb(red, 255u - red, 80);
      } else if (a.mode == 4) {
        const u32 r8 = f2u_trunc(fmul(fadd(SM_S(SM_ROW_NORMAL_X, i), 1.0f), 127.99500274658203125f));
        const u32 g8 = f2u_trunc(fmul(fadd(SM_S(SM_ROW_NORMAL_Y, i), 1.0f), 127.99500274658203125f));
        const u32 b8 = f2u_trunc(fmul(fadd(SM_S(SM_ROW_NORMAL_Z, i), 1.0f), 127.99500274658203125f));
        color = pack_rgb(r8, g8, b8);
      } else {
        color = SM_SU(SM_ROW_COLOR, i);
      }
      v[3] = __uint_as_float(color);
    }
    if (a.neighbor_index) {
      uint4 lo, hi;
      const u32 n0 = SM_SU(SM_ROW_NEIGHBOR0 + 0, i), n1 = SM_SU(SM_ROW_NEIGHBOR0 + 1, i);
      const u32 n2 = SM_SU(SM_ROW_NEIGHBOR0 + 2, i), n3 = SM_SU(SM_ROW_NEIGHBOR0 + 3, i);
      lo = make_uint4(i, n0 == kInvalidIndex ? i : n0, i, n1 == kInvalidIndex ? i : n1);
      hi = make_uint4(i, n2 == kInvalidIndex ? i : n2, i, n3 == kInvalidIndex ? i : n3);
      uint4* out = reinterpret_cast<uint4*>(a.neighbor_index + static_cast<size_t>(i) * 8);
      out[0] = lo;
      out[1] = hi;
    }
    if (a.normal_vertex) {
      const float radius = fsqrt_approx(SM_S(SM_ROW_RADIUS_SQUARED, i));
      float* o = a.normal_vertex + static_cast<size_t>(i) * 6;
      o[0] = sx; o[1] = sy; o[2] = sz;
      o[3] = ffma(radius, SM_S(SM_ROW_NORMAL_X, i), sx);
      o[4] = ffma(radius, SM_S(SM_ROW_NORMAL_Y, i), sy);
      o[5] = ffma(radius, SM_S(SM_ROW_NORMAL_Z, i), sz);
    }
  }
}

int FullTransfer(sm_reconstruction* r, cudaStream_t stream, u32 n, float* const out[7], uint32_t* stamp) {
  const size_t bytes = sizeof(float) * n;
  const float* s = r->d.surfels;
  const size_t st = r->d.stride;
  const float* src[7] = {r->d.smooth + 0 * st, r->d.smooth + 1 * st, r->d.smooth + 2 * st,
                         s + SM_ROW_RADIUS_SQUARED * st, s + SM_ROW_NORMAL_X * st, s + SM_ROW_NORMAL_Y * st,
                         s + SM_ROW_NORMAL_Z * st};
  for (int k = 0; k < 7; ++k) SM_CUDA(cudaMemcpyAsync(out[k], src[k], bytes, cudaMemcpyDeviceToHost, stream));
  SM_CUDA(cudaMemcpyAsync(stamp, s + SM_ROW_LAST_UPDATE_STAMP * st, bytes, cudaMemcpyDeviceToHost, stream));
  return SM_OK;
}

}

int UpdateVisualizationBuffers(sm_reconstruction* r, cudaStream_t stream, const sm_visualization_params& p, float* vertex,
                               uint32_t* neighbor_index, float* normal_vertex) {
  if (p.point_size_in_floats < 4 && vertex) return SetError(SM_ERR_INVALID_ARGUMENT, "point_size_in_floats < 4");
  if (neighbor_index && (reinterpret_cast<uintptr_t>(neighbor_index) & 15)) return SetError(SM_ERR_INVALID_ARGUMENT, "neighbor index buffer must be 16-byte aligned");
  VizArgs a;
  a.count_slot = r->count_slot;
  a.frame_index = p.frame_index;
  a.active_window = p.surfel_integration_active_window_size;
  a.latest_triangulated_frame_index = p.latest_triangulated_frame_index;
  a.latest_mesh_surfel_count = p.latest_mesh_surfel_count;
  a.point_size_in_floats = p.point_size_in_floats;
  a.mode = p.visualize_last_update_timestamp ? 1 : p.visualize_creation_timestamp ? 2 : p.visualize_radii ? 3 : p.visualize_normals ? 4 : 0;
  a.vertex = vertex; a.neighbor_index = neighbor_index; a.normal_vertex = normal_vertex;
  r->last_stream = stream;
  { LaunchScope scope(stream, KID_VIZ_BUFFERS); LaunchKernel(k_viz_buffers, dim3(r->sm_count * 8), dim3(kBlock), 0, stream, r->d, a); }
  return CheckLaunch("visualization buffers");
}

void RecordOperation(sm_reconstruction* r, int stamp_threshold) {
  ++r->op_epoch;
  r->op_history.push_back({r->op_epoch, stamp_threshold});
  if (r->op_history.size() > 8192) r->op_history.erase(r->op_history.begin(), r->op_history.begin() + 4096);
}

void FreeTransferBuffers(sm_reconstruction* r) {
  cudaFree(r->delta_index); cudaFree(r->delta_values); cudaFree(r->delta_cursor);
  if (r->delta_host) cudaFreeHost(r->delta_host);
  r->delta_index = nullptr; r->delta_values = nullptr; r->delta_cursor = nullptr; r->delta_host = nullptr;
  r->delta_capacity = 0; r->delta_host_capacity = 0;
}

namespace {
bool DeltaTimingEnabled() {
  static const bool enabled = [] { const char* e = std::getenv("SM_B200_DELTA_TIMING"); return e && e[0] == '1'; }();
  return enabled;
}
}

int TransferDelta(sm_reconstruction* r, cudaStream_t stream, uint32_t frame_index, sm_transfer_token* token, float* x,
                  float* y, float* z, float* radius_squared, float* nx, float* ny, float* nz,
                  uint32_t* last_update_stamp, sm_transfer_stats* stats) {
  (void)frame_index;
  r->last_stream = stream;
  int status = FetchCounters(r, stream);
  if (status != SM_OK) return status;
  const u32 n = r->host_counters->surfel_count[r->count_slot];
  float* const out[7] = {x, y, z, radius_squared, nx, ny, nz};
  sm_transfer_stats st{};
  st.surfel_count = n;

  bool full = token->generation != r->state_generation || token->epoch > r->op_epoch || token->surfel_count > n;
  int threshold = 0x7FFFFFFF;
  if (!full) {
    if (!r->op_history.empty() && r->op_history.front().epoch > token->epoch + 1) full = true;
    for (const auto& op : r->op_history)
      if (op.epoch > token->epoch) threshold = std::min(threshold, op.stamp_threshold);
  }
  if (!full && threshold <= 0) full = true;
  if (!full && n > 0) {
    if (r->delta_capacity < n) {
      SM_CUDA(cudaStreamSynchronize(stream));
      cudaFree(r->delta_index); cudaFree(r->delta_values);
      r->delta_index = nullptr; r->delta_values = nullptr;
      const size_t cap = std::min<size_t>(r->d.stride, std::max<size_t>(2 * static_cast<size_t>(n), 1u << 20));
      SM_CUDA(cudaMalloc(&r->delta_index, sizeof(u32) * cap));
      SM_CUDA(cudaMalloc(&r->delta_values, sizeof(float) * 8 * cap));
      r->delta_capacity = static_cast<u32>(cap);
    }
    if (!r->delta_cursor) SM_CUDA(cudaMalloc(&r->delta_cursor, sizeof(u32)));
    SM_CUDA(cudaMemsetAsync(r->delta_cursor, 0, sizeof(u32), stream));
    DeltaArgs a;
    a.count_slot = r->count_slot;
    a.count_at_token = static_cast<u32>(token->surfel_count);
    a.stamp_threshold = threshold;
    a.epoch_at_token = static_cast<u32>(token->epoch);
    a.capacity = r->delta_capacity;
    a.cursor = r->delta_cursor;
    a.index = r->delta_index;
    a.values = r->delta_values;
    { LaunchScope scope(stream, KID_DELTA_SELECT); LaunchKernel(k_delta_select, dim3(r->sm_count * 8), dim3(kBlock), 0, stream, r->d, a); }
    status = CheckLaunch("delta select");
    if (status != SM_OK) return status;
    u32 changed = 0;
    SM_CUDA(cudaMemcpyAsync(&changed, r->delta_cursor, sizeof(u32), cudaMemcpyDeviceToHost, stream));
    SM_CUDA(cudaStreamSynchronize(stream));
    st.d2h_bytes += sizeof(u32);
    if (static_cast<size_t>(changed) * 9 > static_cast<size_t>(n) * 8) {
      full = true;
    } else if (changed > 0) {
      const size_t words = static_cast<size_t>(changed) * 9;
      if (r->delta_host_capacity < words) {
        if (r->delta_host) cudaFreeHost(r->delta_host);
        r->delta_host = nullptr;
        const size_t cap = std::max<size_t>(2 * words, 1u << 20);
        SM_CUDA(cudaMallocHost(&r->delta_host, sizeof(u32) * cap));
        r->delta_host_capacity = cap;
      }
      u32* host_index = r->delta_host;
      float* host_values = reinterpret_cast<float*>(r->delta_host + changed);
      SM_CUDA(cudaMemcpyAsync(host_index, r->delta_index, sizeof(u32) * changed, cudaMemcpyDeviceToHost, stream));
      SM_CUDA(cudaMemcpy2DAsync(host_values, sizeof(float) * changed, r->delta_values, sizeof(float) * r->delta_capacity,
                                sizeof(float) * changed, 8, cudaMemcpyDeviceToHost, stream));
      SM_CUDA(cudaStreamSynchronize(stream));
      st.d2h_bytes += sizeof(u32) * words;
      const auto t_scatter = std::chrono::steady_clock::now();
      u32* const dst_rows[8] = {reinterpret_cast<u32*>(x), reinterpret_cast<u32*>(y), reinterpret_cast<u32*>(z),
                                reinterpret_cast<u32*>(radius_squared), reinterpret_cast<u32*>(nx),
                                reinterpret_cast<u32*>(ny), reinterpret_cast<u32*>(nz), last_update_stamp};
      const u32* src_rows = reinterpret_cast<const u32*>(host_values);
      auto scatter_rows = [&](int first_row, int last_row) {
        for (int k = first_row; k < last_row; ++k) {
          const u32* v = src_rows + static_cast<size_t>(k) * changed;
          u32* dst = dst_rows[k];
          for (u32 j = 0; j < changed; ++j) dst[host_index[j]] = v[j];
        }
      };
      bool scattered = false;
      if (changed >= (1u << 16)) {
        std::thread workers[3];
        int started = 0;
        try {
          for (; started < 3; ++started) workers[started] = std::thread(scatter_rows, 2 * started + 2, 2 * started + 4);
        } catch (const std::exception&) {
        }
        scatter_rows(0, 2);
        for (int t = 0; t < started; ++t) workers[t].join();
        if (started < 3) scatter_rows(2 * started + 2, 8);
        scattered = true;
      }
      if (!scattered) scatter_rows(0, 8);
      if (DeltaTimingEnabled()) {
        const double ms = std::chrono::duration<double, std::milli>(std::chrono::steady_clock::now() - t_scatter).count();
        fprintf(stderr, "[surfel_b200] delta transfer: %u of %u slots, host scatter %.3f ms\n", changed, n, ms);
      }
    }
    st.changed_count = changed;
  }
  if (full) {
    if (n > 0) {
      status = FullTransfer(r, stream, n, out, last_update_stamp);
      if (status != SM_OK) return status;
      SM_CUDA(cudaStreamSynchronize(stream));
      st.d2h_bytes += static_cast<uint64_t>(n) * 8 * sizeof(float);
    }
// ... 12 lines not shown
```

Measured before the change: 8511.

## Pack smoothed positions and meta into float4 records for regularisation

Replaces the three SoA smooth-position rows plus the separate meta row with an AoS float4 record array (x,y,z,meta) that is double-buffered for regularisation. Neighbour gathers in the regularisation kernels become one 16-byte load per neighbour instead of four scattered 4-byte loads, and meta is read in the same transaction. Export paths must now run a mirror kernel to copy records back into the SoA rows, and state loading runs a pack kernel. This adds launches on transfer/export paths and extra write bandwidth for the w component in integrate updates.

```diff
diff --git a/surfelmeshing_b200/csrc/api.cu b/surfelmeshing_b200/csrc/api.cu
--- a/surfelmeshing_b200/csrc/api.cu
+++ b/surfelmeshing_b200/csrc/api.cu
@@ -144,7 +144,7 @@
       "k_normals", "k_radii", "k_project", "k_associate", "k_merge", "k_blend", "k_integrate", "k_update_neighbors",
       "k_new_surfel_scan", "k_create_surfels", "k_reg_accumulate", "k_reg_step", "k_reg_copy_only",
       "k_export_vertices", "k_median_densify", "k_delta_select", "k_viz_buffers", "k_project_tail",
-      "k_downscale_depth_median", "k_downscale_color"};
+      "k_downscale_depth_median", "k_downscale_color", "k_reg_mirror", "k_reg_pack"};
   return (id >= 0 && id < KID_COUNT) ? names[id] : "?";
 }
 
@@ -298,9 +298,9 @@
   const size_t scan_tiles = (P + kSegment - 1) / kSegment;
   SM_CUDA(cudaMalloc(&d.surfels, sizeof(float) * SM_ROW_COUNT * d.stride));
   SM_CUDA(cudaMalloc(&d.gradient, sizeof(float4) * d.stride));
-  SM_CUDA(cudaMalloc(&r->smooth_alt, sizeof(float) * 3 * d.stride));
-  d.smooth = d.surfels + static_cast<size_t>(SM_ROW_SMOOTH_X) * d.stride;
-  d.smooth_next = r->smooth_alt;
+  SM_CUDA(cudaMalloc(&r->reg_records, sizeof(float4) * 2 * d.stride));
+  d.smooth = r->reg_records;
+  d.smooth_next = r->reg_records + d.stride;
   SM_CUDA(cudaMemset(d.gradient, 0, sizeof(float4) * d.stride));
   for (int i = 0; i < kSets; ++i) {
     SM_CUDA(cudaMalloc(&r->assoc_set[i], sizeof(PixelAssoc) * P));
@@ -462,7 +462,7 @@
   cudaGetLastError();
   DestroyFrameGraph(r->graph);
   DeviceState& d = r->d;
-  cudaFree(d.surfels); cudaFree(d.gradient); cudaFree(r->smooth_alt); cudaFree(d.new_list);
+  cudaFree(d.surfels); cudaFree(d.gradient); cudaFree(r->reg_records); cudaFree(d.new_list);
   for (int i = 0; i < kSets; ++i) {
     cudaFree(r->vis_set[i]); cudaFree(r->seg_count_set[i]); cudaFree(r->merge_flag_set[i]);
     cudaFree(r->upd_list_set[i]); cudaFree(r->upd_count_set[i]);
@@ -625,9 +625,11 @@
   const size_t bytes = sizeof(float) * n;
   const float* s = r->d.surfels;
   const size_t st = r->d.stride;
-  SM_CUDA(cudaMemcpyAsync(x, r->d.smooth + 0 * st, bytes, cudaMemcpyDeviceToHost, stream));
-  SM_CUDA(cudaMemcpyAsync(y, r->d.smooth + 1 * st, bytes, cudaMemcpyDeviceToHost, stream));
-  SM_CUDA(cudaMemcpyAsync(z, r->d.smooth + 2 * st, bytes, cudaMemcpyDeviceToHost, stream));
+  const int mirrored = MirrorRegRecords(stream, r->d, n, r->sm_count);
+  if (mirrored != SM_OK) return mirrored;
+  SM_CUDA(cudaMemcpyAsync(x, s + SM_ROW_SMOOTH_X * st, bytes, cudaMemcpyDeviceToHost, stream));
+  SM_CUDA(cudaMemcpyAsync(y, s + SM_ROW_SMOOTH_Y * st, bytes, cudaMemcpyDeviceToHost, stream));
+  SM_CUDA(cudaMemcpyAsync(z, s + SM_ROW_SMOOTH_Z * st, bytes, cudaMemcpyDeviceToHost, stream));
   SM_CUDA(cudaMemcpyAsync(radius_squared, s + SM_ROW_RADIUS_SQUARED * st, bytes, cudaMemcpyDeviceToHost, stream));
   SM_CUDA(cudaMemcpyAsync(nx, s + SM_ROW_NORMAL_X * st, bytes, cudaMemcpyDeviceToHost, stream));
   SM_CUDA(cudaMemcpyAsync(ny, s + SM_ROW_NORMAL_Y * st, bytes, cudaMemcpyDeviceToHost, stream));
@@ -677,11 +679,10 @@
   if (merge_count) *merge_count = r->host_counters->merge_count;
   if (host_rows && n > host_row_stride_elems) return SetError(SM_ERR_INVALID_ARGUMENT, "sm_dump_state: host rows shorter than surfels_size()");
   if (host_rows && n > 0) {
+    const int mirrored = MirrorRegRecords(stream, r->d, n, r->sm_count);
+    if (mirrored != SM_OK) return mirrored;
     SM_CUDA(cudaMemcpy2DAsync(host_rows, host_row_stride_elems * sizeof(float), r->d.surfels,
                               r->d.stride * sizeof(float), n * sizeof(float), SM_ROW_COUNT, cudaMemcpyDeviceToHost,
-                              stream));
-    SM_CUDA(cudaMemcpy2DAsync(host_rows + SM_ROW_SMOOTH_X * host_row_stride_elems, host_row_stride_elems * sizeof(float),
-                              r->d.smooth, r->d.stride * sizeof(float), n * sizeof(float), 3, cudaMemcpyDeviceToHost,
                               stream));
     SM_CUDA(cudaStreamSynchronize(stream));
   }
@@ -692,8 +693,6 @@
                   uint32_t surfels_size, uint32_t merge_count) {
   cudaStream_t stream = static_cast<cudaStream_t>(stream_v);
   if (surfels_size > r->d.capacity) return SetError(SM_ERR_CAPACITY, "sm_load_state: state larger than the surfel cap");
-  r->d.smooth = r->d.surfels + static_cast<size_t>(SM_ROW_SMOOTH_X) * r->d.stride;
-  r->d.smooth_next = r->smooth_alt;
   r->d.reg_full_sweep = 1;
   if (surfels_size > 0) {
     SM_CUDA(cudaMemcpy2DAsync(r->d.surfels, r->d.stride * sizeof(float), host_rows,
@@ -705,7 +704,7 @@
       SM_CUDA(cudaMemsetAsync(r->d.surfels + row * r->d.stride, 0, surfels_size * sizeof(float), stream));
     }
     SM_CUDA(cudaMemsetAsync(r->d.surfels + kRowMergeEpoch * r->d.stride, 0, surfels_size * sizeof(float), stream));
-    const int status = RebuildMetaRow(stream, r->d, surfels_size, r->sm_count);
+    const int status = PackRegRecords(stream, r->d, surfels_size, r->sm_count);
     if (status != SM_OK) return status;
   }
   Counters c{};
diff --git a/surfelmeshing_b200/csrc/integrate.cu b/surfelmeshing_b200/csrc/integrate.cu
--- a/surfelmeshing_b200/csrc/integrate.cu
+++ b/surfelmeshing_b200/csrc/integrate.cu
@@ -15,8 +15,6 @@
 
 #define SM_S(row, i) d.surfels[static_cast<size_t>(row) * d.stride + (i)]
 #define SM_SU(row, i) reinterpret_cast<u32*>(d.surfels)[static_cast<size_t>(row) * d.stride + (i)]
-#define SM_SMOOTH(axis, i) d.smooth[static_cast<size_t>(axis) * d.stride + (i)]
-#define SM_SMOOTH_NEXT(axis, i) d.smooth_next[static_cast<size_t>(axis) * d.stride + (i)]
 
 constexpr int kBlock = 256;
 
@@ -833,10 +831,11 @@
       SM_SU(SM_ROW_LAST_UPDATE_STAMP, idx) = 0;
       SM_S(SM_ROW_RADIUS_SQUARED, idx) = -1.0f;
       reinterpret_cast<u8*>(&SM_SU(SM_ROW_COLOR, idx))[3] = 1;
-      SM_SU(kRowMeta, idx) = kMetaDetachBit;
       SM_SU(kRowMergeEpoch, idx) = f.op_epoch;
-      SM_SMOOTH_NEXT(0, idx) = SM_SMOOTH(0, idx); SM_SMOOTH_NEXT(1, idx) = SM_SMOOTH(1, idx);
-      SM_SMOOTH_NEXT(2, idx) = SM_SMOOTH(2, idx);
+      float4 record = d.smooth[idx];
+      record.w = __uint_as_float(kMetaDetachBit);
+      d.smooth[idx] = record;
+      d.smooth_next[idx] = record;
       return false;
     }
     if (!(e.x & kActiveBit)) return false;
@@ -875,11 +874,17 @@
       SM_SU(SM_ROW_COLOR, idx) = s.color;
       if (s.stamped) {
         SM_SU(SM_ROW_LAST_UPDATE_STAMP, idx) = f.frame_index;
-        SM_SU(kRowMeta, idx) = f.frame_index | (((s.color >> 24) & 1u) ? kMetaDetachBit : 0u);
+        const u32 meta = f.frame_index | (((s.color >> 24) & 1u) ? kMetaDetachBit : 0u);
+        if (s.replaced) {
+          const float4 record = make_float4(s.smooth_x, s.smooth_y, s.smooth_z, __uint_as_float(meta));
+          d.smooth[idx] = record;
+          d.smooth_next[idx] = record;
+        } else {
+          store_reg_meta(d.smooth, idx, meta);
+          store_reg_meta(d.smooth_next, idx, meta);
+        }
       }
       if (s.replaced) {
-        SM_SMOOTH(0, idx) = s.smooth_x; SM_SMOOTH(1, idx) = s.smooth_y; SM_SMOOTH(2, idx) = s.smooth_z;
-        SM_SMOOTH_NEXT(0, idx) = s.smooth_x; SM_SMOOTH_NEXT(1, idx) = s.smooth_y; SM_SMOOTH_NEXT(2, idx) = s.smooth_z;
         SM_SU(SM_ROW_CREATION_STAMP, idx) = f.frame_index;
 #pragma unroll
         for (int i = 0; i < 4; ++i) SM_SU(SM_ROW_NEIGHBOR0 + i, idx) = kInvalidIndex;
@@ -1156,9 +1161,10 @@
       const u32 q = neighbor_index[direction];
       if (q == kInvalidIndex) continue;
       ndist[direction] = squared_norm(fsub(SM_S(SM_ROW_X, q), g.x), fsub(SM_S(SM_ROW_Y, q), g.y), fsub(SM_S(SM_ROW_Z, q), g.z));
-      nsx[direction] = SM_SMOOTH(0, q);
-      nsy[direction] = SM_SMOOTH(1, q);
-      nsz[direction] = SM_SMOOTH(2, q);
+      const float4 record = d.smooth[q];
+      nsx[direction] = record.x;
+      nsy[direction] = record.y;
+      nsz[direction] = record.z;
     }
     float sum_x = 0.f, sum_y = 0.f, sum_z = 0.f;
     int existing_neighbor_count_plus_1 = 1;
@@ -1186,7 +1192,6 @@
     SM_S(SM_ROW_CONFIDENCE, idx) = 1.0f;
     SM_SU(SM_ROW_CREATION_STAMP, idx) = f.frame_index;
     SM_SU(SM_ROW_LAST_UPDATE_STAMP, idx) = f.frame_index;
-    SM_SU(kRowMeta, idx) = f.frame_index;
     SM_S(SM_ROW_RADIUS_SQUARED, idx) = radius_squared;
     SM_S(SM_ROW_GRADIENT_X, idx) = 0.f; SM_S(SM_ROW_GRADIENT_Y, idx) = 0.f; SM_S(SM_ROW_GRADIENT_Z, idx) = 0.f;
     SM_S(SM_ROW_GRADIENT_COUNT, idx) = 0.f;
@@ -1195,8 +1200,9 @@
     const float sx = fmul(fadd(g.x, sum_x), rcp_count);
     const float sy = fmul(fadd(g.y, sum_y), rcp_count);
     const float sz = fmul(fadd(g.z, sum_z), rcp_count);
-    SM_SMOOTH(0, idx) = sx; SM_SMOOTH(1, idx) = sy; SM_SMOOTH(2, idx) = sz;
-    SM_SMOOTH_NEXT(0, idx) = sx; SM_SMOOTH_NEXT(1, idx) = sy; SM_SMOOTH_NEXT(2, idx) = sz;
+    const float4 record = make_float4(sx, sy, sz, __uint_as_float(f.frame_index));
+    d.smooth[idx] = record;
+    d.smooth_next[idx] = record;
   }
 }
 
@@ -1207,9 +1213,10 @@
   for (u32 i = blockIdx.x * blockDim.x + threadIdx.x; i < n; i += gridDim.x * blockDim.x) {
     const bool merged = SM_S(SM_ROW_RADIUS_SQUARED, i) < 0.f;
     const float nan = __int_as_float(0x7fffffff);
-    position_buffer[3 * i + 0] = merged ? nan : SM_SMOOTH(0, i);
-    position_buffer[3 * i + 1] = merged ? nan : SM_SMOOTH(1, i);
-    position_buffer[3 * i + 2] = merged ? nan : SM_SMOOTH(2, i);
+    const float4 smooth = d.smooth[i];
+    position_buffer[3 * i + 0] = merged ? nan : smooth.x;
+    position_buffer[3 * i + 1] = merged ? nan : smooth.y;
+    position_buffer[3 * i + 2] = merged ? nan : smooth.z;
     const u32 c = SM_SU(SM_ROW_COLOR, i);
     color_buffer[3 * i + 0] = c & 0xFF;
     color_buffer[3 * i + 1] = (c >> 8) & 0xFF;
diff --git a/surfelmeshing_b200/csrc/knn.cu b/surfelmeshing_b200/csrc/knn.cu
--- a/surfelmeshing_b200/csrc/knn.cu
+++ b/surfelmeshing_b200/csrc/knn.cu
@@ -576,8 +576,11 @@
   if (status != SM_OK) return status;
   if (out_point_count) *out_point_count = n;
   const size_t st = r->d.stride;
-  return smb::KnnBuild(k, stream, n, r->d.smooth, r->d.smooth + st, r->d.smooth + 2 * st,
-                       r->d.surfels + SM_ROW_RADIUS_SQUARED * st, nullptr, cell_size);
+  const int mirrored = smb::MirrorRegRecords(stream, r->d, n, r->sm_count);
+  if (mirrored != SM_OK) return mirrored;
+  const float* s = r->d.surfels;
+  return smb::KnnBuild(k, stream, n, s + SM_ROW_SMOOTH_X * st, s + SM_ROW_SMOOTH_Y * st, s + SM_ROW_SMOOTH_Z * st,
+                       s + SM_ROW_RADIUS_SQUARED * st, nullptr, cell_size);
 }
 
 int sm_knn_query(sm_knn_index* k, void* stream, uint32_t query_count, const float* qx, const float* qy, const float* qz,
diff --git a/surfelmeshing_b200/csrc/pipeline.cu b/surfelmeshing_b200/csrc/pipeline.cu
--- a/surfelmeshing_b200/csrc/pipeline.cu
+++ b/surfelmeshing_b200/csrc/pipeline.cu
@@ -435,8 +435,8 @@
   int uploaded_until = c.first - half - 1;
   const int it0 = c.first - 2;
 
-  float* smooth = r->d.smooth;
-  float* smooth_next = r->d.smooth_next;
+  float4* smooth = r->d.smooth;
+  float4* smooth_next = r->d.smooth_next;
 
   auto active = [&](int frame) { return frame >= c.first && frame < c.last; };
   auto clamp_frame = [&](int frame) { return frame < c.first ? c.first : (frame >= c.last ? c.last - 1 : frame); };
@@ -485,7 +485,7 @@
                            c.ip->radius_factor_for_regularization_neighbors, c.ip->regularizer_weight,
                            c.ip->regularization_frame_window_size, new_slot, i == 0 ? old_slot : -1);
         if (!disable_denoising && active(crit)) {
-          float* const filled = smooth_next;
+          float4* const filled = smooth_next;
           smooth_next = smooth;
           smooth = filled;
           d.smooth = smooth; d.smooth_next = smooth_next;
diff --git a/surfelmeshing_b200/csrc/regularize.cu b/surfelmeshing_b200/csrc/regularize.cu
--- a/surfelmeshing_b200/csrc/regularize.cu
+++ b/surfelmeshing_b200/csrc/regularize.cu
@@ -10,8 +10,6 @@
 
 #define SM_S(row, i) d.surfels[static_cast<size_t>(row) * d.stride + (i)]
 #define SM_SU(row, i) reinterpret_cast<u32*>(d.surfels)[static_cast<size_t>(row) * d.stride + (i)]
-#define SM_SMOOTH(axis, i) d.smooth[static_cast<size_t>(axis) * d.stride + (i)]
-#define SM_SMOOTH_NEXT(axis, i) d.smooth_next[static_cast<size_t>(axis) * d.stride + (i)]
 
 constexpr int kBlock = 256;
 #ifndef SM_REG_ACCUMULATE_MIN_BLOCKS
@@ -60,13 +58,14 @@
     }
     if ((nbr[0] & nbr[1] & nbr[2] & nbr[3]) == kInvalidIndex) continue;
 
-    u32 meta[4];
+    float4 rec[4];
 #pragma unroll
     for (int k = 0; k < 4; ++k) {
       const u32 q = nbr[k] != kInvalidIndex ? nbr[k] : i;
-      meta[k] = SM_SU(kRowMeta, q);
-    }
-    const float sx = SM_SMOOTH(0, i), sy = SM_SMOOTH(1, i), sz = SM_SMOOTH(2, i);
+      rec[k] = d.smooth[q];
+    }
+    const float4 self = d.smooth[i];
+    const float sx = self.x, sy = self.y, sz = self.z;
     const float nx = SM_S(SM_ROW_NORMAL_X, i), ny = SM_S(SM_ROW_NORMAL_Y, i), nz = SM_S(SM_ROW_NORMAL_Z, i);
     const float radius_squared = SM_S(SM_ROW_RADIUS_SQUARED, i);
 
@@ -74,23 +73,16 @@
     int neighbor_count = 0;
 #pragma unroll
     for (int k = 0; k < 4; ++k) {
-      if (i < n_remove && nbr[k] != kInvalidIndex && (meta[k] & kMetaDetachBit)) {
+      const u32 meta = __float_as_uint(rec[k].w);
+      if (i < n_remove && nbr[k] != kInvalidIndex && (meta & kMetaDetachBit)) {
         nbr[k] = kInvalidIndex;
         SM_SU(SM_ROW_NEIGHBOR0 + k, i) = kInvalidIndex;
       }
-      use[k] = nbr[k] != kInvalidIndex && !outside_window(meta[k] & ~kMetaDetachBit, p);
+      use[k] = nbr[k] != kInvalidIndex && !outside_window(meta & ~kMetaDetachBit, p);
       neighbor_count += use[k] ? 1 : 0;
     }
     if (neighbor_count == 0) continue;
 
-    float qx[4], qy[4], qz[4];
-#pragma unroll
-    for (int k = 0; k < 4; ++k) {
-      const u32 q = use[k] ? nbr[k] : i;
-      qx[k] = SM_SMOOTH(0, q);
-      qy[k] = SM_SMOOTH(1, q);
-      qz[k] = SM_SMOOTH(2, q);
-    }
     const float max_distance_squared = fmul(radius_squared, p.radius_factor_squared);
     const float rcp_count = frcp(i2f(neighbor_count));
     const float factor = fmul(fadd(p.regularizer_weight, p.regularizer_weight), rcp_count);
@@ -99,9 +91,9 @@
     for (int k = 0; k < 4; ++k) {
       if (!use[k]) continue;
       const u32 q = nbr[k];
-      const float dx = fsub(qx[k], sx);
-      const float dy = fsub(qy[k], sy);
-      const float dz = fsub(qz[k], sz);
+      const float dx = fsub(rec[k].x, sx);
+      const float dy = fsub(rec[k].y, sy);
+      const float dz = fsub(rec[k].z, sz);
       const float f = fmul(factor, ffma(nz, dz, ffma(nx, dx, fmul(ny, dy))));
       atomicAdd(&d.gradient[q], make_float4(fmul(nx, f), fmul(ny, f), fmul(nz, f), weight_term));
       if (squared_norm(dx, dy, dz) > max_distance_squared) SM_SU(SM_ROW_NEIGHBOR0 + k, i) = kInvalidIndex;
@@ -122,15 +114,14 @@
     const u32 stamp = stamp_ahead;
     if (i + step < n) stamp_ahead = SM_SU(SM_ROW_LAST_UPDATE_STAMP, i + step);
     if (outside_window(stamp, p)) {
-      if (p.full_sweep || static_cast<int>(stamp) >= p.t_prev) {
-        SM_SMOOTH_NEXT(0, i) = SM_SMOOTH(0, i); SM_SMOOTH_NEXT(1, i) = SM_SMOOTH(1, i); SM_SMOOTH_NEXT(2, i) = SM_SMOOTH(2, i);
-      }
+      if (p.full_sweep || static_cast<int>(stamp) >= p.t_prev) d.smooth_next[i] = d.smooth[i];
       continue;
     }
     u32 nbr[4];
 #pragma unroll
     for (int k = 0; k < 4; ++k) nbr[k] = SM_SU(SM_ROW_NEIGHBOR0 + k, i);
-    const float sx = SM_SMOOTH(0, i), sy = SM_SMOOTH(1, i), sz = SM_SMOOTH(2, i);
+    const float4 self = d.smooth[i];
+    const float sx = self.x, sy = self.y, sz = self.z;
     const float nx = SM_S(SM_ROW_NORMAL_X, i), ny = SM_S(SM_ROW_NORMAL_Y, i), nz = SM_S(SM_ROW_NORMAL_Z, i);
     const float4 accumulated = d.gradient[i];
     float gx = ffma(fsub(sx, SM_S(SM_ROW_X, i)), 2.0f, accumulated.x);
@@ -138,21 +129,19 @@
     float gz = ffma(fsub(sz, SM_S(SM_ROW_Z, i)), 2.0f, accumulated.z);
     int neighbor_count = 0;
     float rx = 0.f, ry = 0.f, rz = 0.f;
-    float qx[4], qy[4], qz[4];
+    float4 rec[4];
 #pragma unroll
     for (int k = 0; k < 4; ++k) {
       const u32 q = nbr[k] != kInvalidIndex ? nbr[k] : i;
-      qx[k] = SM_SMOOTH(0, q);
-      qy[k] = SM_SMOOTH(1, q);
-      qz[k] = SM_SMOOTH(2, q);
+      rec[k] = d.smooth[q];
     }
 #pragma unroll
     for (int k = 0; k < 4; ++k) {
       if (nbr[k] == kInvalidIndex) continue;
       ++neighbor_count;
-      const float dx = fsub(qx[k], sx);
-      const float dy = fsub(qy[k], sy);
-      const float dz = fsub(qz[k], sz);
+      const float dx = fsub(rec[k].x, sx);
+      const float dy = fsub(rec[k].y, sy);
+      const float dz = fsub(rec[k].z, sz);
       const float normal_dot_difference = ffma(nz, dz, ffma(nx, dx, fmul(ny, dy)));
       rx = ffma(-nx, normal_dot_difference, rx);
       ry = ffma(-ny, normal_dot_difference, ry);
@@ -170,9 +159,7 @@
     const float max_step_length = fsqrt_approx(SM_S(SM_ROW_RADIUS_SQUARED, i));
     const float step_length = fmul(step_factor, gradient_length);
     if (step_length > max_step_length) step_factor = fmul(step_factor, fmul(max_step_length, frcp(step_length)));
-    SM_SMOOTH_NEXT(0, i) = ffma(step_factor, -gx, sx);
-    SM_SMOOTH_NEXT(1, i) = ffma(step_factor, -gy, sy);
-    SM_SMOOTH_NEXT(2, i) = ffma(step_factor, -gz, sz);
+    d.smooth_next[i] = make_float4(ffma(step_factor, -gx, sx), ffma(step_factor, -gy, sy), ffma(step_factor, -gz, sz), self.w);
     d.gradient[i] = make_float4(0.f, 0.f, 0.f, 0.f);
   }
 }
@@ -192,27 +179,49 @@
       }
     }
     if (outside_window(SM_SU(SM_ROW_LAST_UPDATE_STAMP, i), p)) continue;
-    const float x = SM_S(SM_ROW_X, i), y = SM_S(SM_ROW_Y, i), z = SM_S(SM_ROW_Z, i);
-    SM_SMOOTH(0, i) = x; SM_SMOOTH(1, i) = y; SM_SMOOTH(2, i) = z;
-    SM_SMOOTH_NEXT(0, i) = x; SM_SMOOTH_NEXT(1, i) = y; SM_SMOOTH_NEXT(2, i) = z;
+    const float4 record = make_float4(SM_S(SM_ROW_X, i), SM_S(SM_ROW_Y, i), SM_S(SM_ROW_Z, i), d.smooth[i].w);
+    d.smooth[i] = record;
+    d.smooth_next[i] = record;
   }
 }
 
 }
 
 namespace {
-__global__ void __launch_bounds__(kBlock) k_rebuild_meta(DeviceState d, u32 count) {
+__global__ void __launch_bounds__(kBlock) k_reg_pack(DeviceState d, u32 count) {
+  pdl_prologue();
   for (u32 i = blockIdx.x * blockDim.x + threadIdx.x; i < count; i += gridDim.x * blockDim.x) {
     const u32 flag = (SM_SU(SM_ROW_COLOR, i) >> 24) == 1u ? kMetaDetachBit : 0u;
-    SM_SU(kRowMeta, i) = (SM_SU(SM_ROW_LAST_UPDATE_STAMP, i) & ~kMetaDetachBit) | flag;
-  }
-}
-}
-
-int RebuildMetaRow(cudaStream_t stream, const DeviceState& d, u32 count, int sm_count) {
+    const u32 meta = (SM_SU(SM_ROW_LAST_UPDATE_STAMP, i) & ~kMetaDetachBit) | flag;
+    const float4 record = make_float4(SM_S(SM_ROW_SMOOTH_X, i), SM_S(SM_ROW_SMOOTH_Y, i), SM_S(SM_ROW_SMOOTH_Z, i),
+                                      __uint_as_float(meta));
+    d.smooth[i] = record;
+    d.smooth_next[i] = record;
+  }
+}
+
+__global__ void __launch_bounds__(kBlock) k_reg_mirror(DeviceState d, u32 count) {
+  pdl_prologue();
+  for (u32 i = blockIdx.x * blockDim.x + threadIdx.x; i < count; i += gridDim.x * blockDim.x) {
+    const float4 record = d.smooth[i];
+    SM_S(SM_ROW_SMOOTH_X, i) = record.x;
+    SM_S(SM_ROW_SMOOTH_Y, i) = record.y;
+    SM_S(SM_ROW_SMOOTH_Z, i) = record.z;
+    SM_SU(kRowMeta, i) = __float_as_uint(record.w);
+  }
+}
+}
+
+int PackRegRecords(cudaStream_t stream, const DeviceState& d, u32 count, int sm_count) {
   if (count == 0) return SM_OK;
-  k_rebuild_meta<<<sm_count * 4, kBlock, 0, stream>>>(d, count);
-  return CheckLaunch("rebuild meta row");
+  { LaunchScope scope(stream, KID_REG_PACK); LaunchKernel(k_reg_pack, dim3(sm_count * 4), dim3(kBlock), 0, stream, d, count); }
+  return CheckLaunch("pack regularisation records");
+}
+
+int MirrorRegRecords(cudaStream_t stream, const DeviceState& d, u32 count, int sm_count) {
+  if (count == 0) return SM_OK;
+  { LaunchScope scope(stream, KID_REG_MIRROR); LaunchKernel(k_reg_mirror, dim3(sm_count * 4), dim3(kBlock), 0, stream, d, count); }
+  return CheckLaunch("mirror regularisation records");
 }
 
 int DescribeRegularize(KernelLaunch* first, KernelLaunch* second, bool skip, const LaunchPlan& plan,
@@ -257,7 +266,7 @@
   LaunchOnStream(stream, first, false);
   if (n == 1) return CheckLaunch("regularize (copy only)");
   LaunchOnStream(stream, second, true);
-  float* const filled = d.smooth_next;
+  float4* const filled = d.smooth_next;
   d.smooth_next = d.smooth;
   d.smooth = filled;
   NoteRegStep(d, frame_index, regularization_frame_window_size);
diff --git a/surfelmeshing_b200/csrc/sm_handle.cuh b/surfelmeshing_b200/csrc/sm_handle.cuh
--- a/surfelmeshing_b200/csrc/sm_handle.cuh
+++ b/surfelmeshing_b200/csrc/sm_handle.cuh
@@ -65,7 +65,7 @@
   float2* run_normals[smb::kSets] = {}; size_t run_normals_pitch = 0;
   float* run_radius[smb::kSets] = {}; size_t run_radius_pitch = 0;
   smb::u16* run_depth_pre[smb::kSets] = {};
-  float* smooth_alt = nullptr;
+  float4* reg_records = nullptr;
   smb::PipelineCtx pipe{};
   cudaStream_t pre_stream = nullptr;
   cudaEvent_t pre_done[2] = {nullptr, nullptr}, int_done[2] = {nullptr, nullptr}, entry_event = nullptr;
diff --git a/surfelmeshing_b200/csrc/sm_kernels.cuh b/surfelmeshing_b200/csrc/sm_kernels.cuh
--- a/surfelmeshing_b200/csrc/sm_kernels.cuh
+++ b/surfelmeshing_b200/csrc/sm_kernels.cuh
@@ -19,7 +19,7 @@
   KID_NORMALS, KID_RADII, KID_PROJECT, KID_ASSOCIATE, KID_MERGE, KID_BLEND, KID_INTEGRATE, KID_UPDATE_NEIGHBORS,
   KID_NEW_SURFEL_SCAN, KID_CREATE_SURFELS, KID_REG_ACCUMULATE, KID_REG_STEP, KID_REG_COPY_ONLY,
   KID_EXPORT_VERTICES, KID_MEDIAN_DENSIFY, KID_DELTA_SELECT, KID_VIZ_BUFFERS, KID_PROJECT_TAIL, KID_DOWNSCALE_DEPTH,
-  KID_DOWNSCALE_COLOR, KID_COUNT
+  KID_DOWNSCALE_COLOR, KID_REG_MIRROR, KID_REG_PACK, KID_COUNT
 };
 const char* KernelName(int id);
 bool ProfilingEnabled();
@@ -46,6 +46,10 @@
 constexpr int kRowMergeEpoch = SM_ROW_ACCUM_X;
 constexpr int kRowMeta = SM_ROW_ACCUM_Y;
 constexpr u32 kMetaDetachBit = 0x80000000u;
+
+__device__ __forceinline__ void store_reg_meta(float4* records, u32 i, u32 meta) {
+  reinterpret_cast<u32*>(records + i)[3] = meta;
+}
 constexpr int kSegment = 1024;
 constexpr u32 kActiveBit = 0x80000000u;
 
@@ -154,8 +158,8 @@
   unsigned long long* scan_state;
   Counters* counters;
   float4* gradient;
-  float* smooth;
-  float* smooth_next;
+  float4* smooth;
+  float4* smooth_next;
   int reg_t_prev;
   int reg_full_sweep;
   unsigned long long* timeline;
@@ -357,7 +361,8 @@
 inline void NoteIntegratedFrame(DeviceState& d, u32 frame_index) {
   if (static_cast<int>(frame_index) < d.reg_t_prev) d.reg_t_prev = static_cast<int>(frame_index);
 }
-int RebuildMetaRow(cudaStream_t stream, const DeviceState& d, u32 count, int sm_count);
+int PackRegRecords(cudaStream_t stream, const DeviceState& d, u32 count, int sm_count);
+int MirrorRegRecords(cudaStream_t stream, const DeviceState& d, u32 count, int sm_count);
 int RegularizeSurfels(cudaStream_t stream, DeviceState& d, bool disable_denoising, u32 frame_index,
                       float radius_factor_for_regularization_neighbors, float regularizer_weight,
                       int regularization_frame_window_size, int count_slot, int remove_replaced_below_slot,
diff --git a/surfelmeshing_b200/csrc/transfer.cu b/surfelmeshing_b200/csrc/transfer.cu
--- a/surfelmeshing_b200/csrc/transfer.cu
+++ b/surfelmeshing_b200/csrc/transfer.cu
@@ -22,7 +22,6 @@
 
 #define SM_S(row, i) d.surfels[static_cast<size_t>(row) * d.stride + (i)]
 #define SM_SU(row, i) reinterpret_cast<u32*>(d.surfels)[static_cast<size_t>(row) * d.stride + (i)]
-#define SM_SMOOTH(axis, i) d.smooth[static_cast<size_t>(axis) * d.stride + (i)]
 
 constexpr int kBlock = 256;
 
@@ -62,9 +61,10 @@
     a.index[k] = i;
     float* v = a.values + k;
     const size_t c = a.capacity;
-    v[0 * c] = SM_SMOOTH(0, i);
-    v[1 * c] = SM_SMOOTH(1, i);
-    v[2 * c] = SM_SMOOTH(2, i);
+    const float4 smooth = d.smooth[i];
+    v[0 * c] = smooth.x;
+    v[1 * c] = smooth.y;
+    v[2 * c] = smooth.z;
     v[3 * c] = radius_squared;
     v[4 * c] = SM_S(SM_ROW_NORMAL_X, i);
     v[5 * c] = SM_S(SM_ROW_NORMAL_Y, i);
@@ -90,7 +90,8 @@
 __global__ void __launch_bounds__(kBlock) k_viz_buffers(DeviceState d, VizArgs a) {
   const u32 n = d.counters->surfel_count[a.count_slot];
   for (u32 i = blockIdx.x * blockDim.x + threadIdx.x; i < n; i += gridDim.x * blockDim.x) {
-    const float sx = SM_SMOOTH(0, i), sy = SM_SMOOTH(1, i), sz = SM_SMOOTH(2, i);
+    const float4 smooth = d.smooth[i];
+    const float sx = smooth.x, sy = smooth.y, sz = smooth.z;
     if (a.vertex) {
       const u32 creation_stamp = SM_SU(SM_ROW_CREATION_STAMP, i);
       const bool output_vertex = creation_stamp <= a.latest_triangulated_frame_index || i >= a.latest_mesh_surfel_count;
@@ -152,7 +153,9 @@
   const size_t bytes = sizeof(float) * n;
   const float* s = r->d.surfels;
   const size_t st = r->d.stride;
-  const float* src[7] = {r->d.smooth + 0 * st, r->d.smooth + 1 * st, r->d.smooth + 2 * st,
+  const int mirrored = MirrorRegRecords(stream, r->d, n, r->sm_count);
+  if (mirrored != SM_OK) return mirrored;
+  const float* src[7] = {s + SM_ROW_SMOOTH_X * st, s + SM_ROW_SMOOTH_Y * st, s + SM_ROW_SMOOTH_Z * st,
                          s + SM_ROW_RADIUS_SQUARED * st, s + SM_ROW_NORMAL_X * st, s + SM_ROW_NORMAL_Y * st,
                          s + SM_ROW_NORMAL_Z * st};
   for (int k = 0; k < 7; ++k) SM_CUDA(cudaMemcpyAsync(out[k], src[k], bytes, cudaMemcpyDeviceToHost, stream));
```

Result: faster. 9248 (median of 6 runs) (+8.7%).
